# pedroegsilva/gofindthem

Hardware: AMD Instinct MI355X
Metric: ProcessText throughput: documents/s (and input GB/s), 10000-term dictionary + 1000 expressions, 1000000 docs of ~4 KB sharded over 1 GPU(s) (higher is better)
Workload: dtype u8; 1 GPU; BASELINE.json configs[2]: 10000 terms + 1000 AND/OR/NOT expressions, 1000000 docs x ~4 KB on this GPU (SURVEY.md 8(d) generator), case-insensitive finder, inputs resident in HBM; alphabet=lower, keywords=10000, docs_total=1000000, docs_per_gpu=1000000, text_bytes_per_gpu=4100690990, parallelism=docs sharded x1, cu_margin=0

## Files before the change

### gofindthem_amd/_lib.py

```python
import ctypes as C
import os

HERE = os.path.dirname(os.path.abspath(__file__))
LIB_PATH = os.environ.get("GFT_LIBRARY") or os.path.join(HERE, "libgft.so")

GFT_OK, GFT_E_INVALID, GFT_E_NOT_BUILT, GFT_E_HIP, GFT_E_UNSUPPORTED, GFT_E_PARSE, GFT_E_ENGINE = 0, -1, -2, -3, -4, -5, -6
GFT_E_NOMEM, GFT_E_INTERNAL, GFT_W_NO_RCCL = -7, -8, 1
GFT_POS_START, GFT_POS_END = 0, 1
GFT_JSON_OK, GFT_JSON_SYNTAX, GFT_JSON_DEPTH, GFT_JSON_PATH, GFT_JSON_KEY, GFT_JSON_DUP, GFT_JSON_TEXT = range(7)
GFT_FOLD_ASCII = 1
GFT_STATS_ACCUMULATE = 1
GFT_SCORE_DISTINCT = 1
GFT_SCAN_UNIQUE = 2
GFT_POS_RUNES = 4
OP_UNIT, OP_AND, OP_OR, OP_NOT, OP_INORD = 1, 2, 3, 4, 5
INORD_FLAG = 1 << 27


class GftMatches(C.Structure):
    _fields_ = [("n_docs", C.c_uint64), ("n_matches", C.c_uint64), ("match_off", C.c_void_p),
                ("term_id", C.c_void_p), ("pos", C.c_void_p)]


class GftSparse(C.Structure):
# ... 62 lines not shown
    "gft_finder_literal": (_i, [_vp, _i, _u32, C.POINTER(_vp), C.POINTER(_u32)]),
    "gft_finder_expression": (_i, [_vp, _u32, C.POINTER(_vp), C.POINTER(_u32), C.POINTER(_vp), C.POINTER(_u32),
                                   C.POINTER(_vp), C.POINTER(_u32)]),
    "gft_finder_force_build": (_i, [_vp]),
    "gft_finder_process_text": (_i, [_vp, C.c_char_p, _u64, _vp, _u32, C.POINTER(_u32)]),
    "gft_finder_process_texts": (_i, [_vp, _vp, _vp, _u64, _vp]),
    "gft_finder_last_regex_docs": (_u64, [_vp]),
    "gft_finder_process_device": (_i, [_vp, _vp, _vp, _u64, _vp]),
    "gft_finder_process_device_begin": (_i, [_vp, _vp, _vp, _u64, _vp]),
    "gft_finder_process_device_end": (_i, [_vp]),
    "gft_finder_debug_add_literal": (_i, [_vp, _i, C.c_char_p, _u32]),
    "gft_finder_debug_set_updated": (_i, [_vp, _i, _i]),
    "gft_finder_debug_get_updated": (_i, [_vp, C.POINTER(_i), C.POINTER(_i)]),
    "gft_group_create": (_i, [C.POINTER(_vp), _vp]),
    "gft_group_destroy": (None, [_vp]),
    "gft_group_last_error": (C.c_char_p, [_vp]),
    "gft_group_add_rule": (_i, [_vp, C.c_char_p, _u64, C.c_char_p, _u64]),
    "gft_group_state": (_i, [_vp, _vp, _u64, C.POINTER(_u64)]),
    "gft_group_process_jsons": (_i, [_vp, _vp, _vp, _u64, C.c_char_p, _u64, C.c_char_p, _u64, _i, _vp, _u64, C.POINTER(_u64)]),
    "gft_group_last_result": (_i, [_vp, _vp, _u64, C.POINTER(_u64)]),
    "gft_group_evaluate": (_i, [_vp, C.c_char_p, _u64, _vp, _u64, C.POINTER(_u64)]),
    "gft_group_last_batch": (_i, [_vp, C.POINTER(_u64), C.POINTER(_u64)]),
    "gft_group_set_schema": (_i, [_vp, _vp, _vp, _u32, C.c_char_p, _u64, C.c_char_p, _u64]),
    "gft_group_n_rule_exprs": (_u32, [_vp]),
    "gft_group_rule_expr": (_i, [_vp, _u32, C.POINTER(_vp), C.POINTER(_u32), C.POINTER(_vp), C.POINTER(_u32)]),
    "gft_group_process_records_device": (_i, [_vp, _vp, _vp, _vp, _vp, _u64, _u64, _vp]),
    "gft_group_process_records": (_i, [_vp, _vp, _vp, _vp, _vp, _u64, _u64, _vp]),
    "gft_debug_eval_rules": (_i, [_vp, _vp, _u32, _vp, _vp, _u64, _u64, _vp]),
    "gft_debug_eval_rules_device": (_i, [_vp, _vp, _u32, _vp, _vp, _u64, _u64, _vp]),
    "gft_group_tag_records_device": (_i, [_vp, _vp, _vp, _vp, _vp, _u64, _u64, _vp, _vp, _vp, _vp, _u64, C.POINTER(_u64)]),
    "gft_group_tag_records": (_i, [_vp, _vp, _vp, _vp, _vp, _u64, _u64, _vp, _vp, _vp, _vp, _u64, C.POINTER(_u64)]),
    "gft_group_tag_jsons_device": (_i, [_vp, _vp, _vp, _u64, _vp, _vp, _vp, _vp, _vp, _u64, C.POINTER(_u64)]),
    "gft_group_tag_jsons_schema": (_i, [_vp, _vp, _vp, _u64, _vp, _u64, C.POINTER(_u64)]),
    "gft_group_tag_jsons_auto": (_i, [_vp, _vp, _vp, _u64, C.c_char_p, _u64, C.c_char_p, _u64, _vp, _u64, C.POINTER(_u64)]),
    "gft_debug_tag_entries": (_i, [_vp, _vp, _u32, _vp, _vp, _u64, _u64, _vp, _vp, _vp, _vp, _u64, C.POINTER(_u64)]),
    "gft_debug_tag_entries_device": (_i, [_vp, _vp, _u32, _vp, _vp, _u64, _u64, _vp, _vp, _vp, _vp, _u64, C.POINTER(_u64)]),
    "gft_group_rules_json_device": (_i, [_vp, _vp, _u64, _vp, _vp, _u64, _vp, C.POINTER(_u64)]),
    "gft_debug_rules_json": (_i, [_vp, _vp, _u64, _vp, _vp, _u64, _vp, C.POINTER(_u64)]),
    "gft_group_tags_json_device": (_i, [_vp, _vp, _vp, _vp, _u64, _u64, _vp, _vp, _u64, _vp, C.POINTER(_u64)]),
    "gft_debug_tags_json": (_i, [_vp, _vp, _u32, _vp, _vp, _u64, _u64, _vp, _vp, _u64, _vp, C.POINTER(_u64)]),
    "gft_group_json_leaves_device": (_i, [_vp, _vp, _vp, _u64, _vp, _vp, _vp, _vp, _u64, _vp, _u64, _vp]),
    "gft_group_process_jsons_device": (_i, [_vp, _vp, _vp, _u64, _vp, _vp]),
    "gft_group_process_jsons_schema": (_i, [_vp, _vp, _vp, _u64, _vp, _u64, C.POINTER(_u64)]),
    "gft_group_json_last": (_i, [_vp, C.POINTER(_u64), C.POINTER(_u64)]),
    "gft_group_json_paths_device": (_i, [_vp, _vp, _vp, _u64, _vp, _u64, _vp, _u64, _vp, C.POINTER(_u64), C.POINTER(_u64)]),
    "gft_group_process_jsons_auto": (_i, [_vp, _vp, _vp, _u64, C.c_char_p, _u64, C.c_char_p, _u64, _vp, _u64, C.POINTER(_u64)]),
    "gft_group_json_auto_last": (_i, [_vp, C.POINTER(_u64), C.POINTER(_u64), C.POINTER(_u64)]),
    "gft_debug_emulate_json_paths": (_i, [_vp, _vp, _vp, _u64, _vp, _u64, _vp, _u64, _vp, C.POINTER(_u64), C.POINTER(_u64), _vp, _u64, C.POINTER(_u64)]),
    "gft_debug_json_paths_ref": (_i, [_vp, _vp, _vp, _u64, _vp, _u64, _vp, _u64, _vp, C.POINTER(_u64)]),
    "gft_debug_json_leaves_ref": (_i, [_vp, _vp, _vp, _u64, _vp, _vp, _vp, _vp, _u64, _vp, _u64, _vp]),
    "gft_debug_emulate_json_leaves": (_i, [_vp, _vp, _vp, _u64, _vp, _vp, _vp, _vp, _u64, _vp, _u64, _vp]),
    "gft_debug_json_schema_find": (C.c_int64, [_vp, C.c_int64, C.c_char_p, _u32, C.POINTER(C.c_int64)]),
    "gft_group_dsl_parse": (_i, [C.c_char_p, _u64, _vp, _u64, C.POINTER(_u64)]),
    "gft_group_dsl_tokens": (_i, [C.c_char_p, _u64, _vp, _u64, C.POINTER(_u64)]),
    "gft_dsl_parse": (_i, [C.c_char_p, _u64, _i, _vp, _u64, C.POINTER(_u64)]),
    "gft_regex_required_literals": (_i, [C.c_char_p, _u64, _vp, _u64, C.POINTER(_u64)]),
    "gft_dsl_tokens": (_i, [C.c_char_p, _u64, _vp, _u64, C.POINTER(_u64)]),
    "gft_to_lower": (_i, [C.c_char_p, _u64, _vp, _u64, C.POINTER(_u64)]),
    "gft_to_lower_device": (_i, [_vp, _vp, _vp, _u64, _vp, _u64, _vp, C.POINTER(_u64)]),
    "gft_debug_lower_rune": (_u32, [_u32]),
    "gft_debug_emulate_to_lower": (_i, [_vp, _vp, _u64, _vp, _u64, _vp, C.POINTER(_u64)]),
    "gft_finder_lowered_batches": (_i, [_vp, C.POINTER(_u64), C.POINTER(_u64)]),
    "gft_split_lines_device": (_i, [_vp, _vp, _u64, _u32, _vp, _u64, C.POINTER(_u64)]),
    "gft_debug_split_lines": (_i, [_vp, _u64, _u32, _vp, _u64, C.POINTER(_u64)]),
    "gft_debug_split_shape": (None, [C.POINTER(_u32), C.POINTER(_u32)]),
    "gft_finder_split_lines_device": (_i, [_vp, _vp, _u64, _u32, _vp, _u64, C.POINTER(_u64)]),
    "gft_select_docs_device": (_i, [_vp, _vp, _vp, _u64, _vp, _u32, _vp, _u32, _vp, _vp, _u64, _vp, _vp, _u64, C.POINTER(_u64), C.POINTER(_u64)]),
    "gft_debug_select_docs": (_i, [_vp, _vp, _u64, _vp, _u32, _vp, _u32, _vp, _vp, _u64, _vp, _vp, _u64, C.POINTER(_u64), C.POINTER(_u64)]),
    "gft_debug_select_shape": (None, [C.POINTER(_u32), C.POINTER(_u32), C.POINTER(_u32)]),
    "gft_context_docs_device": (_i, [_vp, _vp, _vp, _u64, _vp, _u32, _vp, _u32, _vp, _u64, _u64, _vp, _vp, _u64, _vp, _vp, _vp, _u64, _vp, _u64,
                                     C.POINTER(_u64), C.POINTER(_u64), C.POINTER(_u64), C.POINTER(_u64)]),
    "gft_debug_context_docs": (_i, [_vp, _vp, _u64, _vp, _u32, _vp, _u32, _vp, _u64, _u64, _vp, _vp, _u64, _vp, _vp, _vp, _u64, _vp, _u64,
                                    C.POINTER(_u64), C.POINTER(_u64), C.POINTER(_u64), C.POINTER(_u64)]),
    "gft_debug_context_shape": (None, [C.POINTER(_u32), C.POINTER(_u32), C.POINTER(_u32)]),
    "gft_finder_context_docs_device": (_i, [_vp, _vp, _vp, _u64, _vp, _vp, _u32, _vp, _u64, _u64, _vp, _vp, _u64, _vp, _vp, _vp, _u64, _vp, _u64,
                                            C.POINTER(_u64), C.POINTER(_u64), C.POINTER(_u64), C.POINTER(_u64)]),
    "gft_finder_select_docs_device": (_i, [_vp, _vp, _vp, _u64, _vp, _vp, _u32, _vp, _vp, _u64, _vp, _vp, _u64, C.POINTER(_u64), C.POINTER(_u64)]),
    "gft_route_docs_device": (_i, [_vp, _vp, _vp, _u64, _vp, _u32, _vp, _u32, _u32, _u32, _vp, _vp, _u64, _vp, _vp, _u64, _vp, _vp]),
    "gft_debug_route_docs": (_i, [_vp, _vp, _u64, _vp, _u32, _vp, _u32, _u32, _u32, _vp, _vp, _u64, _vp, _vp, _u64, _vp, _vp]),
    "gft_debug_route_shape": (None, [C.POINTER(_u32)]),
    "gft_finder_route_docs_device": (_i, [_vp, _vp, _vp, _u64, _vp, _vp, _u32, _u32, _u32, _vp, _vp, _u64, _vp, _vp, _u64, _vp, _vp]),
    "gft_hit_spans_device": (_i, [_vp, _vp, _vp, _u64, _u32, _vp, _vp, _vp, _vp, _vp, _vp, _vp, _u64, C.POINTER(_u64)]),
    "gft_redact_spans_device": (_i, [_vp, _vp, _vp, _u64, _vp, _vp, _vp, _u32]),
    "gft_debug_witness_terms": (_i, [_vp, _vp, _u32, _u32, _u32, _vp, _vp, _u64, C.POINTER(_u64)]),
    "gft_debug_hit_spans": (_i, [_vp, _vp, _vp, _u64, _vp, _u32, _vp, _vp, _vp, _u32, _vp, _vp, _vp, _vp, _vp, _vp, _u64, C.POINTER(_u64)]),
    "gft_debug_redact_spans": (_i, [_vp, _vp, _u64, _vp, _vp, _vp, _u32]),
    "gft_debug_spans_shape": (None, [C.POINTER(_u32), C.POINTER(_u32)]),
    "gft_finder_hit_spans_device": (_i, [_vp, _vp, _vp, _u64, _vp, _vp, _vp, _vp, _vp, _vp, _vp, _u64, C.POINTER(_u64), C.POINTER(_i)]),
    "gft_finder_hit_spans_source_device": (_i, [_vp, _vp, _vp, _u64, _vp, _vp, _vp, _vp, _vp, _vp, _vp, _u64, C.POINTER(_u64), C.POINTER(_i)]),
    "gft_map_spans_to_source_device": (_i, [_vp, _vp, _vp, _u64, _vp, _vp, _vp]),
    "gft_debug_map_spans_to_source": (_i, [_vp, _vp, _u64, _vp, _vp, _vp]),
    "gft_excerpt_spans_device": (_i, [_vp, _vp, _vp, _u64, _vp, _vp, _vp, _u32, _u32, _u32, _vp, _u64, _vp, _vp, _vp, _vp, _u64, _vp, _vp,
                                     C.POINTER(_u64), C.POINTER(_u64)]),
    "gft_debug_excerpt_spans": (_i, [_vp, _vp, _u64, _vp, _vp, _vp, _u32, _u32, _u32, _vp, _u64, _vp, _vp, _vp, _vp, _u64, _vp, _vp,
                                    C.POINTER(_u64), C.POINTER(_u64)]),
    "gft_debug_excerpt_shape": (None, [C.POINTER(_u32), C.POINTER(_u32)]),
    "gft_finder_excerpts_device": (_i, [_vp, _vp, _vp, _u64, _vp, _vp, _vp, _i, _i, _u32, _u32, _u32, _vp, _u64, _vp, _vp, _vp, _vp, _u64, _vp, _vp,
                                       C.POINTER(_u64), C.POINTER(_u64), C.POINTER(_i)]),
    "gft_excerpt_spans_snap_device": (_i, [_vp, _vp, _vp, _u64, _vp, _vp, _vp, _u32, _u32, _u32, _u32, _vp, _u64, _vp, _vp, _vp, _vp, _u64, _vp,
                                          _vp, C.POINTER(_u64), C.POINTER(_u64)]),
    "gft_debug_excerpt_spans_snap": (_i, [_vp, _vp, _u64, _vp, _vp, _vp, _u32, _u32, _u32, _u32, _vp, _u64, _vp, _vp, _vp, _vp, _u64, _vp, _vp,
                                         C.POINTER(_u64), C.POINTER(_u64)]),
    "gft_debug_excerpt_snap_edges": (_i, [_vp, _u64, _u64, _u64, _u32, _u32, C.POINTER(_u64), C.POINTER(_u64)]),
    "gft_finder_excerpts_snap_device": (_i, [_vp, _vp, _vp, _u64, _vp, _vp, _vp, _i, _i, _u32, _u32, _u32, _u32, _vp, _u64, _vp, _vp, _vp, _vp, _u64,
                                            _vp, _vp, C.POINTER(_u64), C.POINTER(_u64), C.POINTER(_i)]),
    "gft_mark_spans_device": (_i, [_vp, _vp, _vp, _u64, _vp, _vp, _vp, _vp, _u32, _vp, _u32, _u32, _vp, _u64, _vp, _vp, _vp, C.POINTER(_u64),
                                  C.POINTER(_u64)]),
    "gft_debug_mark_spans": (_i, [_vp, _vp, _u64, _vp, _vp, _vp, _vp, _u32, _vp, _u32, _u32, _vp, _u64, _vp, _vp, _vp, C.POINTER(_u64),
                                 C.POINTER(_u64)]),
    "gft_debug_mark_shape": (None, [C.POINTER(_u32), C.POINTER(_u32), C.POINTER(_u32), C.POINTER(_u32)]),
    "gft_finder_mark_device": (_i, [_vp, _vp, _vp, _u64, _vp, _vp, _vp, _i, _i, _vp, _u32, _vp, _u32, _u32, _vp, _u64, _vp, _vp, _vp,
                                   C.POINTER(_u64), C.POINTER(_u64), C.POINTER(_i)]),
    "gft_replace_spans_device": (_i, [_vp, _vp, _vp, _u64, _vp, _vp, _vp, _vp, _vp, _u32, _vp, _vp, _u32, _u32, _vp, _u64, _vp, _vp, _vp, _vp, _vp,
                                     _u64, C.POINTER(_u64), C.POINTER(_u64)]),
    "gft_debug_replace_spans": (_i, [_vp, _vp, _u64, _vp, _vp, _vp, _vp, _vp, _u32, _vp, _vp, _u32, _u32, _vp, _u64, _vp, _vp, _vp, _vp, _vp,
                                    _u64, C.POINTER(_u64), C.POINTER(_u64)]),
    "gft_debug_replace_shape": (None, [C.POINTER(_u32)] * 6),
    "gft_finder_replace_device": (_i, [_vp, _vp, _vp, _u64, _vp, _vp, _vp, _i, _i, _vp, _vp, _vp, _vp, _u32, _u32, _vp, _u64, _vp, _vp, _vp, _vp,
                                      _vp, _u64, C.POINTER(_u64), C.POINTER(_u64), C.POINTER(_i)]),
    "gft_term_stats_device": (_i, [_vp, _vp, _vp, _u64, _u32, _u32, _u64, _vp, _vp, _vp]),
    "gft_count_columns_device": (_i, [_vp, _vp, _u64, _u32, _vp, _u32, _vp]),
    "gft_batch_term_stats_device": (_i, [_vp, _vp, _vp, _u64, _u32, _vp, _vp, _u32, _u64, _vp, _vp, _vp, C.POINTER(_i)]),
    "gft_debug_term_stats": (_i, [_vp, _vp, _u64, _u32, _u32, _u64, _vp, _vp, _vp]),
    "gft_debug_count_columns": (_i, [_vp, _u64, _u32, _vp, _u32, _vp]),
    "gft_debug_stats_shape": (None, [C.POINTER(_u32)] * 8),
    "gft_finder_term_stats_device": (_i, [_vp, _vp, _vp, _u64, _vp, _vp, _u32, _u64, _vp, _vp, _vp, C.POINTER(_i)]),
    "gft_score_docs_device": (_i, [_vp, _vp, _vp, _u64, _u32, _vp, _u32, _vp, C.POINTER(_u64)]),
    "gft_top_docs_device": (_i, [_vp, _vp, _u64, _u32, _u64, _vp, _vp, C.POINTER(_u64)]),
    "gft_gather_docs_device": (_i, [_vp, _vp, _vp, _u64, _vp, _u64, _u64, _vp, _u64, _vp, C.POINTER(_u64)]),
    "gft_batch_top_docs_device": (_i, [_vp, _vp, _vp, _u64, _u32, _vp, _vp, _vp, _u32, _u32, _u64, _vp, _vp, _vp, C.POINTER(_u64), C.POINTER(_i)]),
    "gft_batch_top_docs_words_device": (_i, [_vp, _vp, _vp, _u64, _u32, _vp, _vp, _vp, _u32, _u32, _u64, _vp, _vp, _vp, C.POINTER(_u64),
                                            C.POINTER(_i)]),
    "gft_debug_score_docs": (_i, [_vp, _vp, _u64, _u32, _vp, _u32, _vp, C.POINTER(_u64)]),
    "gft_debug_top_docs": (_i, [_vp, _u64, _u32, _u64, _vp, _vp, C.POINTER(_u64)]),
    "gft_debug_gather_docs": (_i, [_vp, _vp, _u64, _vp, _u64, _u64, _vp, _u64, _vp, C.POINTER(_u64)]),
    "gft_debug_rank_shape": (None, [C.POINTER(_u32)] * 10),
    "gft_finder_top_docs_device": (_i, [_vp, _vp, _vp, _u64, _vp, _vp, _vp, _u32, _u32, _u64, _vp, _vp, _vp, C.POINTER(_u64), C.POINTER(_i)]),
    "gft_filter_word_matches_device": (_i, [_vp, _vp, _vp, _u64, _vp, _vp, _vp, _vp, _vp, _u32, _u32, _vp, _vp, _vp, _vp, _u64, C.POINTER(_u64)]),
    "gft_debug_filter_word_matches": (_i, [_vp, _vp, _u64, _vp, _vp, _vp, _vp, _vp, _u32, _u32, _vp, _vp, _vp, _vp, _u64, C.POINTER(_u64)]),
    "gft_debug_word_rune": (_u32, [_u32]),
    "gft_debug_words_shape": (None, [C.POINTER(_u32)] * 3),
    "gft_scan_words_device": (_i, [_vp, _vp, _vp, _u64, _u32, _vp]),
    "gft_process_words_device": (_i, [_vp, _vp, _vp, _u64, _u32, _vp]),
    "gft_process_words": (_i, [_vp, _vp, _vp, _u64, _u32, _vp]),
    "gft_hit_spans_words_device": (_i, [_vp, _vp, _vp, _u64, _u32, _vp, _vp, _vp, _vp, _vp, _vp, _vp, _u64, C.POINTER(_u64)]),
    "gft_batch_term_stats_words_device": (_i, [_vp, _vp, _vp, _u64, _u32, _vp, _vp, _u32, _u64, _vp, _vp, _vp, C.POINTER(_i)]),
    "gft_finder_set_whole_words": (_i, [_vp, _i]),
    "gft_finder_whole_words": (_i, [_vp]),
    "gft_debug_lowermap_shape": (None, [C.POINTER(_u32), C.POINTER(_u32), C.POINTER(_u32), C.POINTER(_u32)]),
    "gft_group_process_json_lines": (_i, [_vp, _vp, _u64, C.c_char_p, _u64, C.c_char_p, _u64, _vp, _u64, C.POINTER(_u64)]),
    "gft_debug_emulate_scan": (_i, [_vp, _vp, _u32, _vp, _u32, _u32, _u32, _u32, _vp, _vp, _u64, C.POINTER(_u64)]),
    "gft_debug_tables": (_i, [_vp, _vp, _u32, _vp, _u64, _u64, C.c_char_p, C.POINTER(C.c_char_p), _vp, _u64, C.POINTER(_u64), _vp, _u64]),
    "gft_debug_learned_unit": (_i, [_vp, C.POINTER(_u32), C.POINTER(_u32)]),
    "gft_debug_last_unit_route": (_i, [_vp, C.POINTER(C.c_char_p)]),
    "gft_debug_last_fold_bits": (_i, [_vp, C.POINTER(_u32)]),
    "gft_debug_scan_plan": (_i, [_vp, _vp, _u32, _u64, C.c_char_p, C.POINTER(C.c_char_p), _vp]),
    "gft_debug_pool_entries": (_i, [_vp, C.POINTER(_u64)]),
    "gft_debug_last_solve_pf": (_i, [_vp, C.POINTER(_u32), C.POINTER(_u32)]),
    "gft_debug_judge_batch": (_i, [_vp, _i, _u32, _u64, _u64, _u64, _u64, C.POINTER(_i), C.POINTER(_u64), _vp, _vp, _u64]),
    "gft_debug_learn": (_i, [C.c_char_p, _u32, _i, _u64, _u64, _u64, C.POINTER(_u32), C.POINTER(C.c_double)]),
    "gft_debug_eval_programs": (_i, [_vp, _vp, _u32, _u32, _vp, _vp, _vp]),
    "gft_debug_program_shape": (_i, [_vp, _vp, _u32, _u32, _vp, _u32]),
    "gft_debug_plan_solve": (_i, [_u32, _u32, _u32, _i, _u32, _u64, _u32, _u64, _i, _i, _u32, _vp]),
    "gft_debug_plan_solve_pf": (_i, [_u32, _u32, _u32, _i, _u32, _u32, _u64, _u32, _u64, _i, _i, _u32, _u32, _vp]),
    "gft_debug_host_solve": (_i, [_vp, _u64, _vp, _vp, _vp, _u32, C.POINTER(_i)]),
    "gft_profile_enable": (_i, [_vp, _i]),
    "gft_profile_read": (_i, [_vp, C.c_char_p, C.POINTER(C.c_double), C.POINTER(_u64)]),
    "gft_profile_reset": (_i, [_vp]),
}

EMIT_FN = C.CFUNCTYPE(None, _vp, _vp, _u32, C.c_int64)
BUILD_FN = C.CFUNCTYPE(_i, _vp, _vp, _vp, _u32, _i, _vp, _u32)
FIND_FN = C.CFUNCTYPE(_i, _vp, _vp, _u64, EMIT_FN, _vp, _vp, _u32)

_LIB = None


def _mapped_hip_runtimes():
    try:
        with open("/proc/self/maps") as f:
            return sorted({ln.split()[-1] for ln in f if "libamdhip64.so" in ln})
    except OSError:
        return []


def _hip_runtime_first():
    import sys
    if "torch" in sys.modules or os.environ.get("GFT_NO_TORCH_PRELOAD"):
        return
    import importlib.util
    if importlib.util.find_spec("torch") is not None:
        import torch


def _check_one_hip_runtime():
    libs = _mapped_hip_runtimes()
    if len(libs) > 1:
        import warnings
        warnings.warn("two HIP runtimes are mapped into this process (%s): device pointers of one are not valid in the "
                      "other -- import torch before gofindthem_amd loads libgft.so" % ", ".join(libs), RuntimeWarning)


def load():
    global _LIB
    if _LIB is None:
        if not os.path.exists(LIB_PATH):
            raise RuntimeError("libgft.so is not built (run `python -m gofindthem_amd.build`); "
                               "gofindthem_amd has no CPU fallback for the hot path")
        _hip_runtime_first()
        L = C.CDLL(LIB_PATH)
        _check_one_hip_runtime()
        for name, (res, args) in SYMBOLS.items():
            f = getattr(L, name)
            f.restype, f.argtypes = res, args
        _LIB = L
    return _LIB
```

### gofindthem_amd/csrc/batch_verdict.hpp

```cpp
#pragma once
#include <algorithm>
#include <cstddef>
#include <cstdint>

#include "table_set.hpp"

namespace gft {

constexpr size_t kCtlBytes = 64, kCtlWords = 7;
constexpr size_t kCtlBad = 0, kCtlCursor = 8, kCtlTotal = 16, kCtlNonascii = 24, kCtlUnits = 32;
constexpr size_t kCtlBatchClear = 32;
constexpr size_t kCtlRetryClear = 16;
constexpr size_t kCtlScanRead = 24;

struct CtlBlock {
    uint32_t bad = 0;
    uint64_t cursor = 0, total = 0;
    uint32_t nonascii_bits = 0;
    uint32_t miss_epoch = 0;
    uint64_t n_units = 0, text_lo = 0, text_hi = 0;
};
CtlBlock decode_ctl(const uint64_t words[kCtlWords]);

struct BatchVerdict {
    bool nonascii = false;
    uint32_t nonascii_bits = 0;
    uint64_t text_lo = 0, text_hi = 0;
    uint64_t n_units = 0, total = 0;
};

struct ScanLaunch {
    bool deferred = false;
    bool single = false;
    uint32_t epoch = 0;
    bool ordered = false;
    uint64_t n_docs = 0, unit_cap = 0, pool_cap = 0;
    uint64_t static_slabs = 0;
};

inline bool single_miss(const CtlBlock& c, const ScanLaunch& L) { return L.single && c.miss_epoch == L.epoch; }

struct Judgement {
    enum Kind { accept, again_general, again_grow, invalid } kind = accept;
    uint64_t pool_need = 0;
    const char* err = "";
    BatchVerdict verdict;
};
Judgement judge_deferred(const CtlBlock& c, const ScanLaunch& L);

struct Learned {
    int single_streak = 0;
    uint32_t unit_max = kScan2UnitMax;
    double scan4_density = 0.06;
    uint32_t unit_entries = 0;
};
constexpr int kSingleMissStreak = -8;
inline void count_streak(Learned& s, uint64_t n_units, uint64_t n_docs) {
    s.single_streak = n_units == n_docs ? s.single_streak + 1 : std::min(s.single_streak, 0);
}
void learn(Learned& s, ScanKernel kernel, uint32_t fifo_cap, bool ordered, uint64_t total, uint64_t text_lo, uint64_t text_hi);

}
```

### gofindthem_amd/csrc/gft_api.cpp

```cpp
#include "gft_engine.hpp"

#include <cstdio>
#include <cstdlib>

using namespace gft;
using namespace gft::api;

namespace {

long env_num(const char* name, long dflt) { const char* v = getenv(name); return v ? atol(v) : dflt; }

void refresh_options(gft_engine* e) {
    const auto num = env_num;
    e->opt_scan_dbg = (uint32_t)num("GFT_SCAN_DEBUG", 0);
    e->opt_scan_prio = num("GFT_SCAN_PRIO", 1) ? 1u : 0u;
    e->opt_scan_ordered = getenv("GFT_SCAN_ORDERED") ? 1u : 0u;
    e->opt_scan4_chunk = (uint32_t)num("GFT_SCAN4_CHUNK", 0);
    e->opt_scan4_round = (uint32_t)num("GFT_SCAN4_ROUND", 0);
    e->opt_solve.dbg = (uint32_t)num("GFT_SOLVE_DEBUG", 0);
    e->opt_solve.forced_group = (int)num("GFT_SOLVE_GROUP_DOCS", -1);
    e->opt_solve.prog_lds = num("GFT_SOLVE_PROG_LDS", 1) ? 1u : 0u;
    const long pf = num("GFT_SOLVE_PF_TERMS", 0);
    e->opt_solve.forced_pf = pf == 6 || pf == 12 ? (uint32_t)pf : 0u;
}

}

namespace gft::api {

ScanOptions scan_options() {
    const auto num = env_num;
    ScanOptions o;
    o.forced = parse_forced(getenv("GFT_SCAN_KERNEL"));
    o.scan5_groups = (uint32_t)num("GFT_SCAN5_GROUPS", 0);
    o.scan5_large = num("GFT_SCAN5_LARGE", 1) ? 1u : 0u;
    o.scan5_bloom_kb = (uint32_t)std::min<long>(std::max<long>(num("GFT_SCAN5_BLOOM_KB", 32), 0), 64);
    o.scan5_fifo = (uint32_t)std::min<long>(std::max<long>(num("GFT_SCAN5_FIFO", 0), 0), 4096) & ~63u;
    return o;
}

bool pend_settled(const gft_engine* e) {
    for (unsigned i = 0; i < e->pend_count; i++)
        if (!e->pend[(e->pend_head + i) % 2].done) return false;
    return true;
}

int check_ready(const gft_engine* e, unsigned need, const char* who) {
    if ((need & kNeedDevice) && e->device < 0) return fail(e, GFT_E_HIP, "no HIP device available");
    if ((need & kNeedBuilt) && !e->built) return fail(e, GFT_E_NOT_BUILT, "gft_build has not been called");
    if ((need & kNeedPrograms) && !e->have_programs) return fail(e, GFT_E_NOT_BUILT, "gft_set_programs has not been called");
    if ((need & kNeedSettled) && !pend_settled(e))
        return fail(e, GFT_E_INVALID, (who ? std::string(who) + ": " : std::string()) +
                                          "batches of gft_process_device_begin are in flight: gft_process_device_end (or _complete) first");
    return GFT_OK;
}

}

extern "C" {

int gft_engine_create(gft_engine** out, int device) try {
    if (!out) return GFT_E_INVALID;
    *out = nullptr;
    std::unique_ptr<gft_engine> owner(new gft_engine());
    gft_engine* e = owner.get();
    int count = 0;
    hipError_t h = hipGetDeviceCount(&count);
    if (h != hipSuccess || count == 0) {
        e->device = -1;
        e->err = std::string("no HIP device available: ") + (h != hipSuccess ? hipGetErrorString(h) : "device count is 0");
        *out = owner.release();
        return GFT_E_HIP;
    }
    if (device < 0) { if (hipGetDevice(&device) != hipSuccess) device = 0; }
    e->device = device;
    DeviceGuard g(device);
    hipDeviceProp_t prop;
    if (hipGetDeviceProperties(&prop, device) == hipSuccess) {
        e->n_cus_hw = prop.multiProcessorCount > 0 ? (unsigned)prop.multiProcessorCount : 256;
        if (const char* m = getenv("GFT_CU_MARGIN")) { const int v = atoi(m); if (v > 0) e->cu_margin = (unsigned)v; }
        e->n_cus = e->n_cus_hw > e->cu_margin ? e->n_cus_hw - e->cu_margin : 1;
        int optin = 0;
        if (hipDeviceGetAttribute(&optin, hipDeviceAttributeSharedMemPerBlockOptin, device) != hipSuccess) optin = 0;
        e->lds_max = std::max<size_t>(prop.sharedMemPerBlock, (size_t)std::max(optin, 0));
        if (std::string(prop.gcnArchName).find("gfx950") != std::string::npos) e->lds_max = std::max<size_t>(e->lds_max, 160 * 1024);
    }
    if (hipStreamCreateWithFlags(&e->stream, hipStreamDefault) == hipSuccess) e->own_stream = true;
    else e->stream = nullptr;
    refresh_options(e);
    *out = owner.release();
    return GFT_OK;
} GFT_CATCH(nullptr)

void gft_engine_destroy(gft_engine* e) {
    if (!e) return;
    if (e->device < 0) {
        destroy_multi(e);
        delete e;
        return;
    }
    DeviceGuard g(e->device);
    if (e->stream) (void)hipStreamSynchronize(e->stream);
    for (auto& kv : e->prof)
        for (auto& p : kv.second.ev) { e->prof_pool.push_back(p.first); e->prof_pool.push_back(p.second); }
    for (hipEvent_t ev : e->prof_pool) (void)hipEventDestroy(ev);
    for (int k = 0; k < 2; k++) {
        if (e->staging.pin[k]) (void)hipHostFree(e->staging.pin[k]);
        if (k == 0 && e->pin_rb) (void)hipHostFree(e->pin_rb);
        if (e->staging.pin_ev[k]) (void)hipEventDestroy(e->staging.pin_ev[k]);
        if (e->pend[k].rb) (void)hipHostFree(e->pend[k].rb);
        if (e->pend[k].ev) (void)hipEventDestroy(e->pend[k].ev);
    }
    if (e->d_excerpt.pin) (void)hipHostFree(e->d_excerpt.pin);
    destroy_multi(e);
    hipStream_t own = e->own_stream ? e->stream : nullptr;
    delete e;
    if (own) (void)hipStreamDestroy(own);
}

const char* gft_last_error(const gft_engine* e) { return e ? e->err.c_str() : "null engine"; }

int gft_set_stream(gft_engine* e, void* hip_stream) try {
    if (!e) return GFT_E_INVALID;
    GFT_LOCK(e);
    if (int rc = check_ready(e, kNeedDevice)) return rc;
    DeviceGuard g(e->device);
    if (e->own_stream && e->stream) { (void)hipStreamSynchronize(e->stream); (void)hipStreamDestroy(e->stream); }
    e->own_stream = false;
    e->stream = (hipStream_t)hip_stream;
    if (!hip_stream) {
        HIP_TRY(hipStreamCreateWithFlags(&e->stream, hipStreamDefault), "stream create");
        e->own_stream = true;
    }
    return GFT_OK;
} GFT_CATCH((e ? &e->err : nullptr))


int gft_set_cu_margin(gft_engine* e, uint32_t margin) try {
    if (!e) return GFT_E_INVALID;
    GFT_LOCK(e);
    if (int rc = check_ready(e, kNeedDevice)) return rc;
    if (e->pend_count) return fail(e, GFT_E_INVALID, "batches are in flight (gft_process_device_end first)");
    e->cu_margin = margin;
    e->n_cus = e->n_cus_hw > margin ? e->n_cus_hw - margin : 1;
    return GFT_OK;
} GFT_CATCH((e ? &e->err : nullptr))

}

namespace gft::api {

static int upload_scan3_short_tables(gft_engine* e, const Scan3Tables& s3) {
    const std::vector<uint8_t> none(16, 0), g1(s3.cls, s3.cls + 256), g2(s3.cls_fold, s3.cls_fold + 256);
    SyncOnExit drained(e);
    auto& d = e->d_tabs.s3;
    int rc;
    if ((rc = upload(e, d.short3, s3.short3.empty() ? none : s3.short3, "table upload"))) return rc;
    if ((rc = upload(e, d.srec, s3.srec, "table upload"))) return rc;
    if (!s3.short3_big.empty() && (rc = upload(e, d.short3_big, s3.short3_big, "table upload"))) return rc;
    if ((rc = upload(e, d.srec_big, s3.srec_big, "table upload"))) return rc;
    if ((rc = upload(e, d.cls, g1, "table upload"))) return rc;
    if ((rc = upload(e, d.cls_fold, g2, "table upload"))) return rc;
    return GFT_OK;
}

int install_tables(gft_engine* e, TableSet&& set, uint32_t flags) {
    const AcTables& tab = set.tab;
    const Scan2Tables& s2 = set.s2;
    const Scan3Tables& s3 = set.s3;
    ScanPlan plan;
// ... 258 lines not shown
```

### gofindthem_amd/csrc/gft_debug.cpp

```cpp
#include "gft_engine.hpp"

#include <unordered_set>

#include "host_solve.hpp"

using namespace gft;
using namespace gft::api;

extern "C" {

int gft_debug_emulate_scan(const uint8_t* terms_blob, const uint64_t* term_off, uint32_t n_terms, const uint8_t* text,
                           uint32_t len, uint32_t lo, uint32_t flags, uint32_t scan_flags, uint32_t* out_term,
                           uint32_t* out_pos, uint64_t cap, uint64_t* needed) try {
    if ((n_terms && (!terms_blob || !term_off)) || (len && !text) || lo > len || !needed) return GFT_E_INVALID;
    std::vector<std::string> terms;
    for (uint32_t i = 0; i < n_terms; i++) terms.emplace_back((const char*)terms_blob + term_off[i], (size_t)(term_off[i + 1] - term_off[i]));
    AcTables tab;
    build_ac_tables(std::move(terms), tab);
    Scan3Tables t;
    build_scan3_tables(tab, t);
    if (!t.supported) return GFT_E_UNSUPPORTED;
    std::vector<Scan3Hit> hits;
    scan3_emulate(t, text, len, lo, (scan_flags & GFT_FOLD_ASCII) != 0, (flags & GFT_POS_END) != 0, hits);
    *needed = hits.size();
// ... 13 lines not shown
    Scan2Tables s2;
    build_scan2_tables(tab, s2);
    if (!s2.long_ok) return GFT_E_UNSUPPORTED;
    Scan5Tables s5;
    build_scan5_tables(tab, s2, std::min<uint32_t>(groups && groups < s2.kp ? groups : s2.kp, 32u), s5);
    if (groups_used) *groups_used = s5.G;
    const bool fold = (scan_flags & GFT_FOLD_ASCII) != 0;
    const uint8_t* cls = fold ? s2.cls_fold : s2.cls;
    const uint8_t* grp = fold ? s5.grp_fold : s5.grp;
    const uint32_t kp = s2.kp, G = s5.G;
    auto cl = [&](int64_t i) { return i < 0 ? s2.pad_class : (uint32_t)cls[text[i]]; };
    auto gr = [&](int64_t i) { return i < 0 ? s5.pad_group : (uint32_t)grp[text[i]]; };
    std::unordered_set<uint32_t> keys;
    for (const Scan2Slot& sl : s2.slots) if (sl.key != kScan2EmptyKey) keys.insert(sl.key);
    std::vector<std::vector<uint32_t>> shorts;
    for (const auto& term : tab.terms)
        if (!term.empty() && term.size() < 4) {
            std::vector<uint32_t> v;
            for (unsigned char ch : term) v.push_back(tab.byte_class[ch]);
            shorts.push_back(v);
        }
    for (uint32_t i = 0; i < len; i++) {
        const uint32_t key = (uint32_t)((((uint64_t)cl((int64_t)i - 3) * kp + cl((int64_t)i - 2)) * kp + cl((int64_t)i - 1)) * kp + cl(i));
        bool f = keys.count(key) != 0;
        for (size_t k = 0; k < shorts.size() && !f; k++) {
            const auto& v = shorts[k];
            bool eq = true;
            for (size_t j = 0; j < v.size() && eq; j++) eq = cl((int64_t)i - (int64_t)(v.size() - 1 - j)) == v[j];
            f = eq;
        }
        out_exact[i] = f ? 1 : 0;
        out_dual[i] = 0;
    }
    for (int64_t j = (int64_t)(lane_start & 1u); j < (int64_t)len; j += 2) {
        const uint64_t ent = s5.filter[((size_t)gr(j - 2) * G + gr(j - 1)) * G + gr(j)];
        out_dual[j] = (uint8_t)(ent >> gr(j - 3) & 1);
        if (j + 1 < (int64_t)len) out_dual[j + 1] = (uint8_t)(ent >> (32 + gr(j + 1)) & 1);
    }
    if (lane_start & 1u) {
        const uint64_t ent = s5.filter[((size_t)gr(-3) * G + gr(-2)) * G + gr(-1)];
        if (len) out_dual[0] = (uint8_t)(ent >> (32 + gr(0)) & 1);
    }
    return GFT_OK;
} GFT_CATCH(nullptr)

int gft_debug_program_shape(const uint32_t* prog_words, const uint64_t* prog_off, uint32_t n_exprs, uint32_t n_slots, uint32_t* out_shape,
                            uint32_t shape_cap) try {
    if (!prog_words || !prog_off || !out_shape || n_slots > (1u << kDwFieldBits)) return GFT_E_INVALID;
    ProgramSet ps;
    std::string err;
    const int rc = compile_programs(prog_words, prog_off, n_exprs, n_slots, ps, err);
    if (rc) return rc;
    if (shape_cap < 3 + ps.blk_class.size()) return GFT_E_INVALID;
    out_shape[0] = ps.fprog_words; out_shape[1] = ps.n_rare_words > 0; out_shape[2] = ps.wide_pairs;
    std::copy(ps.blk_class.begin(), ps.blk_class.end(), out_shape + 3);
    return GFT_OK;
} GFT_CATCH(nullptr)

int gft_debug_eval_programs(const uint32_t* prog_words, const uint64_t* prog_off, uint32_t n_exprs, uint32_t n_slots,
                            const uint8_t* present, uint8_t* out_hit, uint32_t* out_depth) try {
    if (!prog_words || !prog_off || !out_hit || (n_slots && !present) || n_slots > (1u << kDwFieldBits)) return GFT_E_INVALID;
    ProgramSet ps;
    std::string err;
    const int rc = compile_programs(prog_words, prog_off, n_exprs, n_slots, ps, err);
    if (rc) return rc;
    std::vector<uint8_t> elsewhere(n_exprs, 0);
    for (uint32_t x : ps.host_only) elsewhere[x] = 1;
    for (uint32_t k = 0; k < ps.n_wide; k++) elsewhere[ps.wide_list[3 * k]] = 1;
    for (uint32_t i = 0; i < n_exprs; i++) {
        const uint32_t ex = ps.order[i], b = i / 64, lane = i % 64;
        if (elsewhere[ex]) return GFT_E_UNSUPPORTED;
        const uint32_t depth = ps.fdepth[ex];
        if (out_depth) out_depth[ex] = depth;
        bool acc = false;
        std::vector<bool> stack;
        size_t reached = 0;
        for (uint64_t pc = 0; pc < ps.fprog_off[ex + 1] - ps.fprog_off[ex]; pc++) {
            const uint32_t w = ps.fprog_t[ps.fblk_off[b] + ((pc / 4) * 64 + lane) * 4 + pc % 4];
            if (w & kDwRare) {
                if (!(w & kDwNeg)) return GFT_E_UNSUPPORTED;
                acc = !acc;
                continue;
            }
            const bool v = (present[(w & kDwFieldMask) >> kDwFieldShift] != 0) != ((w & kDwNeg) != 0);
            if ((w & kDwPop) && stack.empty()) return GFT_E_INVALID;
            const bool x = (w & kDwPop) ? (bool)stack.back() : v;
            const bool A = (w & kDwSel) ? x : (w & kDwOnes) != 0, B = (w & kDwOr) ? x : false;
            const bool before = acc;
            acc = (acc && A) || B;
            if (w & kDwPop) stack.pop_back();
            if (w & kDwPush) stack.push_back(before);
            if (stack.size() > depth) return GFT_E_INVALID;
            reached = std::max(reached, stack.size());
        }
        if (!stack.empty()) return GFT_E_INVALID;
        if (reached > (ps.blk_class[b] == 0 ? 0u : ps.blk_class[b] == 1 ? kSolveRegStack : kMaxBoolDepth)) return GFT_E_INTERNAL;
        out_hit[ex] = acc ? 1 : 0;
    }
    return GFT_OK;
} GFT_CATCH(nullptr)

static int debug_tables_and_plan(const uint8_t* terms_blob, const uint64_t* term_off, uint32_t n_terms, const uint8_t* blob, uint64_t blob_len,
                                 uint64_t lds_max, const char* forced_kernel, TableSet& set, uint32_t& flags, ScanPlan& plan, std::string& err) {
    if (blob) {
        if (int rc = read_tables(blob, blob_len, set, flags, err)) return rc;
    } else {
        std::vector<std::string> terms;
        for (uint32_t i = 0; i < n_terms; i++) terms.emplace_back((const char*)terms_blob + term_off[i], (size_t)(term_off[i + 1] - term_off[i]));
        compile_tables(std::move(terms), set);
    }
    ScanOptions opt = scan_options();
    if (forced_kernel) opt.forced = parse_forced(forced_kernel);
    return plan_scan(set, opt, lds_max, kExtraKernels, plan, err);
}

int gft_debug_tables(const uint8_t* terms_blob, const uint64_t* term_off, uint32_t n_terms, const uint8_t* blob, uint64_t blob_len,
                     uint64_t lds_max, const char* forced_kernel, const char** kernel, uint8_t* out, uint64_t cap, uint64_t* needed,
                     char* err_out, uint64_t err_cap) try {
    if (!kernel || !needed || (!blob && n_terms && (!terms_blob || !term_off))) return GFT_E_INVALID;
    *kernel = "";
    *needed = 0;
    std::string err;
    auto done = [&](int rc) {
        if (err_out && err_cap) { const size_t n = std::min<size_t>(err.size(), err_cap - 1); memcpy(err_out, err.data(), n); err_out[n] = 0; }
        return rc;
    };
    TableSet set;
    uint32_t flags = 0;
    int rc;
    ScanPlan plan;
    if ((rc = debug_tables_and_plan(terms_blob, term_off, n_terms, blob, blob_len, lds_max, forced_kernel, set, flags, plan, err))) return done(rc);
    *kernel = kScanKernelName[(int)plan.kernel];
    if (plan.kernel == ScanKernel::scan5) {
        Scan5Tables s5;
        std::vector<uint32_t> bloom;
        derive_scan5(set, plan, s5, bloom);
    }
    std::vector<uint8_t> b;
    write_tables(set, flags, b);
    *needed = b.size();
    if (!out) return done(GFT_OK);
    if (cap < b.size()) return done(GFT_E_INVALID);
    memcpy(out, b.data(), b.size());
    return done(GFT_OK);
} GFT_CATCH(nullptr)

int gft_debug_learned_unit(const gft_engine* e, uint32_t* unit_max, uint32_t* fifo_cap) {
    if (!e || !unit_max) return GFT_E_INVALID;
    *unit_max = e->learned.unit_max;
    if (fifo_cap) *fifo_cap = e->plan.kernel == ScanKernel::scan5 ? e->plan.s5plan.fifo_cap : kScan2FifoCap;
    return GFT_OK;
}

int gft_debug_last_unit_route(const gft_engine* e, const char** name) {
    if (!e || !name) return GFT_E_INVALID;
    *name = e->last_unit_route;
    return GFT_OK;
}

int gft_debug_last_fold_bits(const gft_engine* e, uint32_t* bits) {
    if (!e || !bits) return GFT_E_INVALID;
    *bits = e->reported.nonascii_bits;
    return GFT_OK;
}

int gft_debug_scan_plan(const uint8_t* terms_blob, const uint64_t* term_off, uint32_t n_terms, uint64_t lds_max, const char* forced_kernel,
                        const char** kernel, uint32_t* plan_out) try {
    if (!kernel || !plan_out || (n_terms && (!terms_blob || !term_off))) return GFT_E_INVALID;
    *kernel = "";
    TableSet set;
    uint32_t flags = 0;
    ScanPlan plan;
    std::string err;
    if (int rc = debug_tables_and_plan(terms_blob, term_off, n_terms, nullptr, 0, lds_max, forced_kernel, set, flags, plan, err)) return rc;
    *kernel = kScanKernelName[(int)plan.kernel];
    const bool s5 = plan.kernel == ScanKernel::scan5;
    plan_out[0] = set.tab.max_term_len;
    plan_out[1] = s5 ? plan.s5_term_bits : 0u;
    plan_out[2] = s5 ? plan.s5_pos_bias : 0u;
    plan_out[3] = s5 ? plan.s5plan.fifo_cap : kScan2FifoCap;
    return GFT_OK;
} GFT_CATCH(nullptr)

int gft_debug_pool_entries(const gft_engine* e, uint64_t* entries) {
    if (!e || !entries) return GFT_E_INVALID;
    *entries = e->pool.total;
    return GFT_OK;
}

int gft_debug_last_solve_pf(const gft_engine* e, uint32_t* pf_terms, uint32_t* unit_entries) {
    if (!e || !pf_terms) return GFT_E_INVALID;
    *pf_terms = e->last_pf_terms;
    if (unit_entries) *unit_entries = e->learned.unit_entries;
    return GFT_OK;
}

int gft_debug_host_solve(const uint32_t* words, uint64_t len, const uint32_t* slots, const uint64_t* list_off,
                         const int64_t* positions, uint32_t n_lists, int* out) try {
    if (!words || !out || (n_lists && (!slots || !list_off))) return GFT_E_INVALID;
    uint32_t n_slots = 0;
    for (uint64_t i = 0; i < len; i++)
        if ((words[i] >> 28) == GFT_OP_UNIT) n_slots = std::max(n_slots, (words[i] & GFT_SLOT_MASK) + 1);
    ProgramTraits tr;
    std::string err;
    const int rc = check_program(words, len, n_slots, 0, tr, err);
    if (rc) return rc;
    SlotLists m;
    for (uint32_t k = 0; k < n_lists; k++) {
        std::vector<int64_t>& v = m[slots[k]];
        for (uint64_t i = list_off[k]; i < list_off[k + 1]; i++) v.push_back(positions[i]);
    }
    *out = host_solve(words, len, m) ? 1 : 0;
    return GFT_OK;
} GFT_CATCH(nullptr)

}
```

### gofindthem_amd/csrc/gft_engine.hpp

```cpp
#pragma once
#include "../../include/gft.h"

#include <hip/hip_runtime.h>

#include <algorithm>
#include <cstring>
#include <map>
#include <memory>
#include <mutex>
#include <string>
#include <utility>
#include <vector>

#include "batch_verdict.hpp"
#include "copy_pool.hpp"
#include "gft_guard.hpp"
#include "gft_kernels.hpp"
#include "program_set.hpp"
#include "solve_plan.hpp"
#include "table_set.hpp"

namespace gft::api {

struct DevBuf {
    void* p = nullptr;
    size_t cap = 0;
    DevBuf() = default;
    DevBuf(const DevBuf&) = delete;
    DevBuf& operator=(const DevBuf&) = delete;
    DevBuf(DevBuf&& o) noexcept : p(o.p), cap(o.cap) { o.p = nullptr; o.cap = 0; }
    DevBuf& operator=(DevBuf&& o) noexcept {
        if (this != &o) { release(); p = o.p; cap = o.cap; o.p = nullptr; o.cap = 0; }
        return *this;
    }
    ~DevBuf() { release(); }
    hipError_t ensure(size_t bytes) {
        if (bytes <= cap) return hipSuccess;
        if (p) { hipError_t e = hipFree(p); p = nullptr; cap = 0; if (e != hipSuccess) return e; }
        size_t want = bytes + bytes / 8 + 256;
        hipError_t e = hipMalloc(&p, want);
        if (e == hipSuccess) cap = want;
        return e;
    }
    void release() { if (p) (void)hipFree(p); p = nullptr; cap = 0; }
    template <class T> T* as() const { return reinterpret_cast<T*>(p); }
};

struct ProfCat {
    std::vector<std::pair<hipEvent_t, hipEvent_t>> ev;
};

struct PoolState {
    uint64_t n_units = 0, total = 0;
    uint64_t valid_docs = ~0ull;
    bool csr_valid = false;
};

}

struct gft_engine {
    using DevBuf = gft::api::DevBuf;
    int device = 0;
    hipStream_t stream = nullptr;
    struct Staging {
        void* pin[2] = {nullptr, nullptr};
        hipEvent_t pin_ev[2] = {nullptr, nullptr};
        std::unique_ptr<gft::CopyPool> copy_pool;
    } staging;
    uint64_t* pin_rb = nullptr;
    bool own_stream = false;
    unsigned n_cus = 256;
    unsigned n_cus_hw = 256, cu_margin = 0;
    size_t lds_max = 65536;
    mutable std::string err;

    gft::TableSet tables;
    gft::ScanPlan plan;
    gft::Scan5Tables s5;
    bool built = false;
    uint32_t build_flags = 0;
    struct TableBufs {
        struct { DevBuf byte_class, delta, out_term, out_link, term_len; } dfa;
        struct { DevBuf filter, slots, more, cls, cls_fold, term_blob, term_off, short3, shorts_packed, short3_big, fpt; } s2;
        struct { DevBuf filter, short3, srec, short3_big, srec_big, bloom, slots, more, cls, cls_fold, term_blob, term_off; } s3;
        struct { DevBuf grp, grp_fold, filter, bloom; } s5;
    } d_tabs;
    DevBuf d_ctl, d_dbg;
    gft::Learned learned;
    gft::BatchVerdict reported;
    gft::api::PoolState pool;
    uint32_t opt_scan_dbg = 0;
    uint32_t opt_scan_prio = 1;
    uint32_t opt_scan_ordered = 0;
    uint32_t opt_scan4_round = 0;
    uint32_t opt_scan4_chunk = 0;
    gft::SolveOptions opt_solve;
    mutable std::recursive_mutex mu;
    std::vector<gft_engine*> peers;
    std::vector<uint64_t> shard_cut;
    bool in_multi = false;
    std::vector<void*> comms;
    bool rccl_self = false;
    void* rccl_lib = nullptr;

    bool have_programs = false;
    uint32_t n_exprs = 0, n_extra = 0;
    gft::ProgramSet progs;
    struct ProgramBufs {
        DevBuf prog, prog_off;
        DevBuf fprog, fprog_off, groups;
        DevBuf order, blk_class, wave_blk;
        DevBuf fprog_t, fblk_off;
        DevBuf wide_list;
    } d_progs;
    DevBuf d_patch;
    DevBuf d_wide_slot, d_wide_theta;
    DevBuf d_solve_dbg;
    uint32_t ctl_epoch = 1;
    uint32_t solve_unit_entries = 0;
    uint32_t last_pf_terms = 0;
    const char* last_unit_route = "";
    struct Pending {
        bool done = false;
        int rc = 0;
        const uint8_t* d_text = nullptr; const uint64_t* d_doc_off = nullptr; uint64_t n_docs = 0; uint32_t flags = 0;
        uint32_t* d_bitmap = nullptr;
        gft::ScanLaunch launch;
        uint64_t* rb = nullptr; hipEvent_t ev = nullptr;
        gft::BatchVerdict verdict;
    };
    Pending pend[2];
    unsigned pend_head = 0, pend_count = 0;
    DevBuf d_pscratch;

    DevBuf d_unit_cnt, d_unit_base, d_units, d_partial, d_pool_term, d_pool_pos, d_unit_start,
        d_unit_count, d_unit_out, d_term, d_pos, d_match_off;
    uint64_t pool_cap = 0;
    DevBuf d_text, d_doc_off, d_bitmap, d_xoff, d_xslot, d_xpos;
    struct UniqueBufs { DevBuf first, cnt, off, term; } d_uq;
    struct RuneBufs { DevBuf cnt, base, starts, prefix; } d_rn;
    std::vector<uint64_t> h_match_off;
    std::vector<uint32_t> h_term, h_pos;
    bool have_labels = false;
    std::vector<uint32_t> h_labels;
    DevBuf d_labels;
    struct SparseBufs {
        DevBuf cnt, partial, row_off, idx, label;
        std::vector<uint64_t> h_row_off;
        std::vector<uint32_t> h_expr_idx, h_label, h_bitmap;
    } sparse;
    struct LowerBufs {
        bool table_up = false;
        DevBuf page, delta, doc_units, unit_base, units, partial, unit_cnt, unit_out, ctl, text, off;
    } d_lw;

    struct SplitBufs { DevBuf sums, carry, cnt, base, partial; } d_split;

    struct SelectBufs { DevBuf want, len, sel, pos, rank, partial, ctl, c_off, c_src; } d_select;

    struct ContextBufs { DevBuf want, sel, len, keep, word_sel, word_fence, sum, carry, part, pos, rank, grank, partial, ctl, c_off, c_src; } d_context;

    struct RouteBufs { DevBuf masks, member, len, cnt, tile_bytes, base, partial, ctl, ent_len, c_off, c_src; } d_route;

    struct SpanBufs {
        bool wit_ready = false;
        DevBuf wit_off, wit_expr, want, keep, rank, partial, dst, ctl;
    } d_spans;

    struct LowerMapBufs { DevBuf tab, off, mapped, ctl; } d_lmap;

    struct ExcerptBufs {
        DevBuf ws, we, sdoc, smin, head, share, tmin, carry, rank, pos, partial, ctl, c_off, c_src;
        uint64_t* pin = nullptr;
    } d_excerpt;

    struct MarkBufs { DevBuf q, marks; } d_mark;

    struct ReplaceBufs { DevBuf rid, pl, ppos, key_rep, rep_off, tab, at, delta, len, roff; } d_replace;

    struct StatsBufs { DevBuf ctl, rows; } d_stats;

    struct KeptBufs { DevBuf off, start, term; } d_kept;

    struct RankBufs {
        DevBuf ctl, weights, rows, hist, tile_gt, tile_eq, gt_pos, eq_pos, partial, cand_score, cand_idx, len, c_off, c_src, score;
    } d_rank;

    struct WordBufs {
        bool table_up = false;
        DevBuf tab_row, tab_bits, ctl, keep, rank, partial, off, pos, term, span_off, span_start, span_len, span_term;
    } d_words;

    struct RuleBufs {
        uint64_t serial = 0;
        uint32_t n_fields = 0, n_tags = 0, n_exprs = 0, n_rules = 0, n_units = 0, max_depth = 0, field_words = 0;
        DevBuf expr_tag, masks, units, prog, prog_off, leaf_bitmap, tag_rows, flags, stage[6];
        DevBuf valid;
    } d_rules;

    struct TagBufs {
        DevBuf cnt, leaf_ent_off, partial, flags, row_off, ent_field, ent_expr;
    } d_tags;

    struct ResultBufs {
        uint64_t serial = 0;
        uint32_t n_exprs = 0;
        DevBuf rule_first, name_off, name_len, expr_off, expr_len, blob, cnt, scan, partial, flags, hole_len, out_off, text;
    } d_result;

    struct TagDocBufs {
        uint64_t slot_serial = 0, field_serial = 0;
        uint32_t n_exprs = 0, SW = 0, n_tags = 0, n_fields = 0;
        DevBuf src_off, src_expr, slot_off, slot_len, tag_word, tag_words, tag_off, tag_len, slot_blob;
        DevBuf field_rank, field_off, field_len, valid, field_blob;
        DevBuf slot_rows, leaf_field, rec_off, cnt, scan, partial, flags, hole_len, out_off, text;
        bool staged = false;
        uint64_t staged_records = 0, staged_leaves = 0;
    } d_tagdoc;

    struct JsonBufs {
        uint64_t serial = 0;
        uint32_t n_nodes = 0, table_mask = 0, max_key_len = 0;
        DevBuf nodes, keys, table, cnt_leaves, cnt_text, text_off, partial, flags, rec_off, leaf_field, leaf_off, text, blob, doc_off, status, rows;
        DevBuf paths;
    } d_json;

    int profiling = 0;
    std::vector<hipEvent_t> prof_pool;
    std::map<std::string, gft::api::ProfCat> prof;
};

#define GFT_LOCK(e) std::lock_guard<std::recursive_mutex> _gft_lock((e)->mu)

#define HIP_TRY(expr, what)                                             \
    do {                                                                \
        hipError_t _h = (expr);                                         \
        if (_h != hipSuccess) return gft::api::fail_hip(e, _h, what);   \
    } while (0)

namespace gft::api {

inline int fail(const gft_engine* e, int code, const std::string& msg) {
    e->err = msg;
    return code;
}
inline int fail_hip(const gft_engine* e, hipError_t h, const char* what) {
    e->err = std::string(what) + ": " + hipGetErrorString(h);
// ... 98 lines not shown
```

### gofindthem_amd/csrc/gft_kernels.hip

```cpp
#include <hip/hip_runtime.h>

#include "gft_kernels.hpp"
#include "gft_wave_dev.hpp"

namespace gft {

namespace {

constexpr uint32_t kLane = 64;

__device__ __forceinline__ uint32_t wave_incl_scan_shfl(uint32_t v) {
    const uint32_t l = lane_id();
#pragma unroll
    for (int s = 1; s < 64; s <<= 1) {
        uint32_t o = __shfl_up(v, s, 64);
        if ((int)l >= s) v += o;
    }
    return v;
}

__global__ void __launch_bounds__(256) k_unit_count(const uint64_t* __restrict__ doc_off, uint64_t n_docs,
                                                    uint32_t unit_max, uint32_t* __restrict__ cnt,
                                                    uint32_t* __restrict__ bad) {
    uint64_t d = (uint64_t)blockIdx.x * blockDim.x + threadIdx.x;
    if (d >= n_docs) return;
    uint64_t n = doc_off[d + 1] - doc_off[d];
    if (n > 0xFFFFFFFFull) { atomicOr(bad, 1u); n = 0; }
    cnt[d] = n <= unit_max ? 1u : (uint32_t)((n + unit_max - 1) / unit_max);
}

__global__ void k_pack_ctl(const uint64_t* __restrict__ unit_base, const uint64_t* __restrict__ doc_off, uint64_t n_docs,
                           uint64_t* __restrict__ out) {
    out[0] = unit_base[n_docs];
    out[1] = doc_off[0];
    out[2] = doc_off[n_docs];
}

__global__ void __launch_bounds__(256) k_unit_fill(const uint64_t* __restrict__ doc_off, uint64_t n_docs,
                                                   const uint64_t* __restrict__ unit_base, Unit* __restrict__ units,
                                                   uint64_t max_units, uint32_t unit_max) {
    uint64_t d = (uint64_t)blockIdx.x * blockDim.x + threadIdx.x;
    if (d >= n_docs) return;
    uint64_t n = doc_off[d + 1] - doc_off[d];
    if (n > 0xFFFFFFFFull) n = 0;
    uint64_t b = unit_base[d];
    uint32_t k = (uint32_t)(unit_base[d + 1] - b);
    if (k == 0) return;
    for (uint32_t i = 0; i < k; i++)
        if (b + i < max_units) units[b + i] = unit_slice((uint32_t)d, n, k, i, unit_max);
}

__global__ void __launch_bounds__(256) k_units_single(const uint64_t* __restrict__ doc_off, uint64_t n_docs, uint32_t unit_max,
                                                      Unit* __restrict__ units, uint64_t* __restrict__ unit_base,
                                                      uint32_t* __restrict__ ctl32, uint32_t epoch) {
    const uint64_t d = (uint64_t)blockIdx.x * blockDim.x + threadIdx.x;
    if (d == 0) {
        uint64_t* ctl64 = reinterpret_cast<uint64_t*>(ctl32);
        unit_base[n_docs] = n_docs;
        ctl32[1] = 0; ctl64[1] = 0; ctl64[2] = 0; ctl32[6] = 0;
        ctl64[4] = n_docs; ctl64[5] = doc_off[0]; ctl64[6] = doc_off[n_docs];
    }
    if (d >= n_docs) return;
    uint64_t n = doc_off[d + 1] - doc_off[d];
    if (n > 0xFFFFFFFFull) { atomicMax(ctl32, epoch); n = 0; }
    if (n > unit_max) { atomicMax(ctl32 + 7, epoch); n = unit_max; }
    units[d] = Unit{(uint32_t)d, 0u, (uint32_t)n};
    unit_base[d] = d;
}

__global__ void __launch_bounds__(256) k_patch_words(uint32_t* __restrict__ words, const uint64_t* __restrict__ idx,
                                                     const uint32_t* __restrict__ clr, const uint32_t* __restrict__ set, uint64_t n) {
    const uint64_t i = (uint64_t)blockIdx.x * blockDim.x + threadIdx.x;
    if (i >= n) return;
    if (clr[i]) atomicAnd(&words[idx[i]], ~clr[i]);
    if (set[i]) atomicOr(&words[idx[i]], set[i]);
}

__global__ void __launch_bounds__(256) k_clamp_u64(uint64_t* __restrict__ v, uint64_t n, uint64_t cap) {
    const uint64_t i = (uint64_t)blockIdx.x * blockDim.x + threadIdx.x;
    if (i < n && v[i] > cap) v[i] = cap;
}

constexpr uint32_t kScanItems = 16, kScanBlock = 256, kScanTile = kScanItems * kScanBlock;

__device__ __forceinline__ uint64_t block_excl_scan_u64(uint64_t v, uint64_t* total) {
    __shared__ uint64_t wsum[kScanBlock / 64];
    const uint32_t l = lane_id(), w = threadIdx.x >> 6;
    uint64_t incl = v;
#pragma unroll
    for (int s = 1; s < 64; s <<= 1) {
        uint64_t o = __shfl_up(incl, s, 64);
        if ((int)l >= s) incl += o;
    }
    if (l == 63) wsum[w] = incl;
    __syncthreads();
    uint64_t off = 0, tot = 0;
#pragma unroll
    for (uint32_t i = 0; i < kScanBlock / 64; i++) {
        if (i < w) off += wsum[i];
        tot += wsum[i];
    }
    __syncthreads();
    *total = tot;
    return off + incl - v;
}

__global__ void __launch_bounds__(kScanBlock) k_scan_partials(const uint32_t* __restrict__ in, uint64_t n,
                                                              uint64_t* __restrict__ partial) {
    uint64_t base = (uint64_t)blockIdx.x * kScanTile + (uint64_t)threadIdx.x * kScanItems;
    uint64_t s = 0;
#pragma unroll
    for (uint32_t i = 0; i < kScanItems; i++)
        if (base + i < n) s += in[base + i];
    uint64_t tot;
    block_excl_scan_u64(s, &tot);
    if (threadIdx.x == 0) partial[blockIdx.x] = tot;
}

__global__ void __launch_bounds__(kScanBlock) k_scan_spine(uint64_t* __restrict__ partial, uint64_t n_part) {
    uint64_t carry = 0;
    for (uint64_t b = 0; b < n_part; b += kScanBlock) {
        uint64_t i = b + threadIdx.x;
        uint64_t v = i < n_part ? partial[i] : 0, tot;
        uint64_t ex = block_excl_scan_u64(v, &tot);
        if (i < n_part) partial[i] = carry + ex;
        carry += tot;
    }
    if (threadIdx.x == 0) partial[n_part] = carry;
}

__global__ void __launch_bounds__(kScanBlock) k_scan_final(const uint32_t* __restrict__ in, uint64_t n,
                                                           const uint64_t* __restrict__ partial, uint64_t n_part,
                                                           uint64_t* __restrict__ out) {
    uint64_t base = (uint64_t)blockIdx.x * kScanTile + (uint64_t)threadIdx.x * kScanItems;
    uint32_t v[kScanItems];
    uint64_t s = 0;
#pragma unroll
    for (uint32_t i = 0; i < kScanItems; i++) {
        v[i] = base + i < n ? in[base + i] : 0;
        s += v[i];
    }
    uint64_t tot;
    uint64_t ex = block_excl_scan_u64(s, &tot) + partial[blockIdx.x];
#pragma unroll
    for (uint32_t i = 0; i < kScanItems; i++) {
        if (base + i < n) out[base + i] = ex;
        ex += v[i];
    }
    if (blockIdx.x == 0 && threadIdx.x == 0) out[n] = partial[n_part];
}

template <bool WRITE>
__device__ __forceinline__ uint32_t walk_chunk(const ScanParams& P, const uint8_t* __restrict__ buf,
                                               const uint8_t* __restrict__ cls_lds,
                                               const uint32_t* __restrict__ delta_lds, uint32_t seg_lo,
                                               uint32_t walk_from, uint32_t my_lo, uint32_t my_hi, uint64_t out_idx) {
    uint32_t state = 0, cnt = 0;
    const uint32_t ncls = P.n_classes;
    for (uint32_t p = walk_from; p < my_hi; p++) {
        const uint32_t c = cls_lds[buf[p - seg_lo]];
        const uint32_t e = state < P.n_lds_states ? delta_lds[state * ncls + c] : P.delta[(size_t)state * ncls + c];
        state = e & 0x7FFFFFFFu;
        if ((e >> 31) && p >= my_lo) {
            uint32_t s = state;
            do {
                const uint32_t t = P.out_term[s];
                if (t != 0xFFFFFFFFu) {
                    if (WRITE) {
                        P.pool_term[out_idx + cnt] = t;
                        P.pool_pos[out_idx + cnt] = P.pos_end ? p : p + 1 - P.term_len[t];
                    }
                    cnt++;
                }
                s = P.out_link[s];
            } while (s != 0);
        }
    }
    return cnt;
}

__global__ void __launch_bounds__(kScanBlockThreads) k_scan_units(const ScanParams P) {
    extern __shared__ __align__(16) uint8_t smem[];
    uint8_t* cls_lds = smem;
    uint32_t* delta_lds = reinterpret_cast<uint32_t*>(smem + 256);
    const uint32_t tier_words = P.n_lds_states * P.n_classes;
    uint8_t* text_lds = smem + 256 + (((size_t)tier_words * 4 + 15) & ~(size_t)15);

    for (uint32_t i = threadIdx.x; i < 256; i += blockDim.x) cls_lds[i] = P.byte_class[i];
    for (uint32_t i = threadIdx.x; i < tier_words; i += blockDim.x) delta_lds[i] = P.delta[i];
    __syncthreads();

    const uint32_t lane = lane_id(), wave = threadIdx.x >> 6, wpb = blockDim.x >> 6;
    uint8_t* buf = text_lds + (size_t)wave * kTextBuf;
    const uint32_t warm = P.max_term_len > 0 ? P.max_term_len - 1 : 0;
    bool told_nonascii = false;

    for (uint64_t u = (uint64_t)blockIdx.x * wpb + wave; u < P.n_units; u += (uint64_t)gridDim.x * wpb) {
        const Unit un = P.units[u];
        const uint64_t dstart = P.doc_off[un.doc];
        const uint32_t seg_lo = un.lo > warm ? un.lo - warm : 0;
        const uint32_t nbytes = un.hi - seg_lo;
        const uint8_t* src = P.text + dstart + seg_lo;
        uint32_t hib = 0;
        for (uint32_t i = lane; i < nbytes; i += kLane) {
            uint8_t b = src[i];
            hib |= b;
            if (P.fold && b >= 'A' && b <= 'Z') b += 32;
            buf[i] = b;
        }
        if (P.fold && P.nonascii && !told_nonascii && __any((hib & 0x80u) != 0)) { told_nonascii = true; if (lane == 0) atomicOr(P.nonascii, 1u); }
        __builtin_amdgcn_wave_barrier();
        __builtin_amdgcn_fence(__ATOMIC_ACQ_REL, "wavefront");
// ... 440 lines not shown
```

### gofindthem_amd/csrc/gft_kernels.hpp

```cpp
#pragma once
#include <hip/hip_runtime.h>
#include <stdint.h>

#include "solve_plan.hpp"

namespace gft {

constexpr uint32_t kScanBlockThreads = 512;
constexpr uint32_t kTextBuf = 8448;
constexpr uint32_t kSolveBlockThreads = 1024;
constexpr uint32_t kMaxPairs = 64;
constexpr uint32_t kMaxPairDepth = 32;
constexpr uint32_t kMaxBoolDepth = 128;
constexpr uint32_t kMaxPairsWide = 8192;
constexpr uint32_t kMaxPairDepthWide = 64;

#define GFT_K_INORD_FLAG (1u << 27)
#define GFT_K_SLOT_MASK ((1u << 27) - 1u)

struct Unit { uint32_t doc, lo, hi; };
__host__ __device__ inline Unit unit_slice(uint32_t doc, uint64_t n, uint64_t k, uint64_t i, uint32_t unit_max) {
    uint64_t per = (n + k - 1) / k;
    if (per > unit_max) per = unit_max;
    const uint64_t lo = i * per < n ? i * per : n, hi = lo + per < n ? lo + per : n;
// ... 71 lines not shown
    const uint32_t* unit_count;
    const uint32_t* term;
    const uint32_t* pos;
    const uint64_t* x_off;
    const uint32_t* x_slot;
    const uint32_t* x_pos;
    uint64_t n_docs;
    const uint32_t* fprog;
    const uint64_t* fprog_off;
    const uint32_t* gprog;
    const uint32_t* groups;
    const uint32_t* order;
    const Unit* units;
    uint32_t has_rare;
    uint32_t pos_back;
    const uint32_t* blk_class;
    const uint32_t* wave_blk;
    const uint32_t* fprog_t;
    const uint32_t* fblk_off;
    uint32_t n_exprs, n_slots, tile_words;
    uint32_t fprog_words;
    uint32_t dbg;
    unsigned long long* dbg_out;
    uint64_t* p_scratch;
    uint32_t* wide_slot;
    long long* wide_theta;
    uint32_t wide_cap;
    const uint32_t* wide_list;
    uint32_t n_wide;
    uint32_t* bitmap;
};

#if defined(__HIPCC__)
#define GFT_HD __host__ __device__
#else
#define GFT_HD
#endif

constexpr uint32_t kScan2Threads = 1024;
constexpr uint32_t kScan2StageCap = 6;
constexpr uint32_t kScan2FifoCap = 256;
constexpr uint32_t kScan2CandCapMin = 512;
constexpr uint32_t kScan2Slab = 4096;
constexpr uint32_t kScan2UnitMax = 8192;
constexpr uint32_t kGoldDev = 0x9E3779B1u;

constexpr uint32_t kScan2EmptyKey = 0xFFFFFFFFu;
constexpr uint32_t kScan2Multi = 0x80000000u;
constexpr uint32_t kScan2InlineLen = 24;
constexpr uint32_t kScan2MaxOff = 4;
constexpr uint32_t kScan2LenMask = 0x00FFFFFFu;
struct __attribute__((aligned(32))) Scan2Slot {
    uint32_t key;
    uint32_t info;
    uint32_t len;
    uint32_t front[5];
};
struct Scan2Short {
    uint32_t n;
    uint32_t term[3];
    uint32_t len[3];
    uint32_t pad;
};
constexpr uint32_t kScan2Short3Max = 32768;
constexpr uint32_t kScan2FptSize = 20480;
constexpr uint32_t kScan2FptLdsItems = 11000;
constexpr uint32_t kScan2FptAmbiguous = 0xFF;
template <uint32_t C>
GFT_HD inline uint32_t scan2_mul24c(uint32_t a) {
#if defined(__HIP_DEVICE_COMPILE__)
    uint32_t d;
    asm("v_mul_u32_u24 %0, %1, %2" : "=v"(d) : "n"(C), "v"(a));
    return d;
#else
    return (uint32_t)((uint64_t)(a & 0xFFFFFFu) * (uint64_t)(C & 0xFFFFFFu));
#endif
}
GFT_HD inline uint32_t scan2_slot_hash(uint32_t x, int which, uint32_t shift, uint32_t seed) {
    const uint32_t xf = (x ^ (x >> 20)) + seed;
    return (which ? scan2_mul24c<0x85EBCBu>(xf) : scan2_mul24c<0x9E3779u>(xf)) >> shift;
}
GFT_HD inline uint32_t scan2_pair_slot(uint32_t x, int which, uint32_t shift, uint32_t seed) {
    const uint32_t xf = (x ^ (x >> 20)) + seed;
    return ((scan2_mul24c<0x9E3779u>(xf) >> shift) & ~1u) | (uint32_t)which;
}
GFT_HD inline uint32_t scan2_fpt_index(uint32_t h, uint32_t fpt_lg) {
    return fpt_lg ? h >> (32 - fpt_lg) : scan2_mul24c<kScan2FptSize>(h >> 16) >> 16;
}
GFT_HD inline uint32_t scan2_fpt_xcell(uint32_t x, uint32_t fpt_lg) { return scan2_fpt_index(scan2_mul24c<0x3779B1u>(x), fpt_lg); }
GFT_HD inline uint32_t scan2_fpt_gcell(uint32_t x, uint32_t b1n, int which, uint32_t fpt_lg) {
    return scan2_fpt_index(which ? scan2_mul24c<0xB2AE35u>(x) + scan2_mul24c<0x9E4F2Du>(b1n)
                                 : scan2_mul24c<0xC2B2AFu>(x) + scan2_mul24c<0x27D4EBu>(b1n), fpt_lg);
}
GFT_HD inline uint32_t scan2_fpt_xmix(uint32_t x) { return scan2_mul24c<0xD4EB2Fu>(x); }
GFT_HD inline uint32_t scan2_fpt_xbyte(uint32_t xmix) { return 1u + (xmix >> 25); }
GFT_HD inline bool scan2_fpt_pass(uint32_t cx, uint32_t cg0, uint32_t cg1, uint32_t xmix, uint32_t tw) {
    (void)tw;
    const uint32_t tag = scan2_fpt_xbyte(xmix);
    const bool amb = (cx == kScan2FptAmbiguous) | (cg0 == kScan2FptAmbiguous) | (cg1 == kScan2FptAmbiguous);
    return (cx == tag) | (cg0 == tag) | (cg1 == tag) | amb;
}

struct Scan2Params {
    const uint8_t* text;
    const uint64_t* doc_off;
    const Unit* units;
    uint64_t n_units;
    const uint32_t* filter;
    uint32_t filter_words, hashed, hash_shift;
    const uint8_t* short3;
    uint32_t short3_bytes;
    const uint32_t* shorts_packed;
    uint32_t shorts_words;
    const uint32_t* short3_big;
    uint32_t cand_cap;
    const uint8_t* fpt;
    uint32_t fpt_lg;
    const Scan2Slot* slots;
    uint32_t slot_shift, slot_seed;
    const Scan2Slot* more;
    const uint8_t* cls;
    const uint8_t* term_blob;
    const uint32_t* term_off;
    uint32_t kp, pad_class, fold, pos_end;
    uint64_t* cursor;
    uint64_t pool_cap;
    uint32_t* pool_term;
    uint32_t* pool_pos;
    uint64_t* unit_start;
    uint32_t* unit_count;
    uint64_t* n_matches;
    uint32_t slab;
    uint32_t ordered;
    uint64_t text_bytes;
    uint32_t prio;
    uint32_t want_pos;
    uint32_t dbg;
    uint32_t* nonascii;
    uint64_t* dbg_counters;
    uint32_t chunk_units;
    uint32_t bound_q16, bound_add;
    uint32_t round_c;
    const uint8_t* s5_grp;
    uint32_t s5_G, s5_pad_g;
    const uint64_t* s5_filter;
    uint32_t s5_dual;
    uint32_t s5_fifo_cap;
    const uint8_t* s5_sgrp;
    uint32_t s5_sG;
    const uint32_t* s5_srec_big;
    uint32_t s5_term_bits, s5_pos_bias;
    const uint32_t* s5_bloom;
    uint32_t s5_bloom_lg;
};
GFT_HD inline uint32_t scan5_bloom_g(uint32_t x, uint32_t b1n, uint32_t lg) {
    return (scan2_mul24c<0xC2B2AFu>(x ^ (x >> 20)) + scan2_mul24c<0x27D4EBu>(b1n + 1)) >> (32 - lg);
}
GFT_HD inline uint32_t scan5_bloom_x(uint32_t x, uint32_t lg) { return scan2_mul24c<0x3779B1u>(x ^ (x >> 20)) >> (32 - lg); }
bool scan2_plan(uint32_t filter_words, uint32_t short3_bytes, uint32_t shorts_words, uint32_t fpt_lds_bytes, size_t lds_max,
                uint32_t* waves, uint32_t* cand_cap);
hipError_t launch_scan2(const Scan2Params& P, uint32_t waves, unsigned n_cus, hipStream_t st);
constexpr uint32_t kScan4ChunkUnits = 8;
constexpr uint32_t kScan4UnitMax = 8176;
bool scan4_plan(uint32_t filter_words, uint32_t short3_bytes, uint32_t shorts_words, uint32_t fpt_lds_bytes, size_t lds_max, bool want_pos,
                uint32_t* waves, uint32_t* fifo_cap);
hipError_t launch_scan4(const Scan2Params& P, uint32_t waves, unsigned n_cus, hipStream_t st);
constexpr uint32_t kScan5Waves = 16;
constexpr uint32_t kScan5MaxGroups = 27;
constexpr uint32_t kScan5SurvX = 64;
constexpr uint32_t kScan5SeenWords = 8;
constexpr uint32_t kScan5CandCapMin = 384;
struct Scan5Plan { uint32_t G, dual_entries, cand_cap, fifo_cap; };
bool scan5_plan(uint32_t kp, uint32_t short3_bytes, uint32_t shorts_words, uint32_t fpt_lds_bytes, size_t lds_max, uint32_t fifo_cap, Scan5Plan* out);
hipError_t launch_scan5(const Scan2Params& P, unsigned n_cus, hipStream_t st);


constexpr uint32_t kScan3Groups = 27;
constexpr uint32_t kScan3Threads = 1024;
constexpr uint32_t kScan3UnitMax = 8192;
constexpr uint32_t kScan3RecWords = 6;
constexpr uint32_t kScan3RecLds = 254;
constexpr uint32_t kScan3BloomLdsLg = 13;
constexpr uint32_t kScan3SurvCap = 128;
constexpr uint32_t kScan3MinRoom = 512;
constexpr uint32_t kScan3CandCapMin = 256;
constexpr uint32_t kScan3BloomMul1 = 0x9E3779B1u, kScan3BloomMul2 = 0x85EBCA6Bu;
GFT_HD inline uint32_t scan3_bloom_cell(uint32_t key5, uint32_t lg) { return (key5 * kScan3BloomMul1) >> (32 - lg); }
GFT_HD inline uint32_t scan3_bloom_bits(uint32_t key5) {
    const uint32_t h = key5 * kScan3BloomMul2;
    return 1u << (h >> 27) | 1u << ((h >> 22) & 31);
}

struct Scan3Params {
    const uint8_t* text;
    const uint64_t* doc_off;
    const Unit* units;
    uint64_t n_units;
    uint64_t text_bytes;
    const uint8_t* cls;
    const uint32_t* filter;
    uint32_t filter_words;
    const uint8_t* short3;
    uint32_t short3_bytes;
    const uint32_t* srec;
    uint32_t srec_words;
    const uint32_t* short3_big;
    const uint32_t* srec_big;
    const uint32_t* bloom;
    uint32_t bloom_lg, bloom_lds;
    const Scan2Slot* slots;
    uint32_t slot_shift, slot_seed;
    const Scan2Slot* more;
    const uint8_t* term_blob;
    const uint32_t* term_off;
    uint32_t G, fold, pos_end, want_pos, grouped, prio;
    uint32_t cand_cap;
    uint32_t dbg;
    uint32_t* nonascii;
    uint64_t* cursor;
    uint64_t pool_cap;
    uint32_t* pool_term;
    uint32_t* pool_pos;
    uint64_t* unit_start;
    uint32_t* unit_count;
    uint64_t* n_matches;
    uint32_t slab;
};
bool scan3_plan(uint32_t filter_words, uint32_t short3_bytes, uint32_t srec_words, uint32_t bloom_lds_bytes, size_t lds_max,
                uint32_t* waves, uint32_t* cand_cap);
hipError_t launch_scan3(const Scan3Params& P, uint32_t waves, unsigned n_cus, hipStream_t st);

hipError_t launch_unit_count(const uint64_t* d_doc_off, uint64_t n_docs, uint32_t unit_max, uint32_t* d_cnt,
                             uint32_t* d_bad, hipStream_t st);
hipError_t launch_pack_ctl(const uint64_t* d_unit_base, const uint64_t* d_doc_off, uint64_t n_docs, uint64_t* d_out, hipStream_t st);
hipError_t launch_unit_fill(const uint64_t* d_doc_off, uint64_t n_docs, const uint64_t* d_unit_base, Unit* d_units,
                            uint32_t unit_max, hipStream_t st, uint64_t max_units = ~0ull);
hipError_t launch_units_single(const uint64_t* d_doc_off, uint64_t n_docs, uint32_t unit_max, Unit* d_units, uint64_t* d_unit_base,
                               uint32_t* d_ctl32, uint32_t epoch, hipStream_t st);
hipError_t launch_patch_words(uint32_t* d_words, const uint64_t* d_idx, const uint32_t* d_clr, const uint32_t* d_set, uint64_t n, hipStream_t st);
hipError_t launch_clamp_u64(uint64_t* d_v, uint64_t n, uint64_t cap, hipStream_t st);
uint64_t scan_partials_needed(uint64_t n);
hipError_t launch_exclusive_scan(const uint32_t* d_in, uint64_t n, uint64_t* d_out, uint64_t* d_partial,
                                 hipStream_t st);
hipError_t launch_compact_count(const uint32_t* d_bitmap, uint64_t n_docs, uint32_t n_exprs, uint32_t* d_cnt, unsigned n_cus,
                                hipStream_t st);
hipError_t launch_compact_fill(const uint32_t* d_bitmap, uint64_t n_docs, uint32_t n_exprs, const uint64_t* d_row_off,
                               uint32_t* d_expr_idx, uint32_t* d_label, const uint32_t* d_expr_label, uint64_t cap, unsigned n_cus,
                               hipStream_t st);
size_t scan_units_lds_bytes(uint32_t n_lds_states, uint32_t n_classes);
hipError_t launch_scan_units(const ScanParams& P, unsigned n_cus, hipStream_t st);
hipError_t launch_gather(const uint64_t* d_unit_start, const uint32_t* d_unit_count, const uint64_t* d_unit_out,
                         uint64_t n_units, const uint32_t* d_pool_term, const uint32_t* d_pool_pos, uint32_t* d_term,
                         uint32_t* d_pos, const uint64_t* d_unit_base, uint64_t n_docs, uint64_t* d_match_off,
                         unsigned n_cus, hipStream_t st, const Unit* d_units_to_sort = nullptr,
                         const uint32_t* d_term_len = nullptr, uint32_t pos_end = 0);
hipError_t launch_fold_safe(const uint8_t* d_text, uint64_t lo, uint64_t hi, const uint64_t* d_doc_off, uint64_t n_docs, uint32_t* d_flag, hipStream_t st);
hipError_t launch_unique_terms(bool write, const uint64_t* d_match_off, const uint32_t* d_term, uint64_t n_docs, uint32_t n_terms,
                               uint32_t* d_first, unsigned grid, uint32_t* d_cnt, const uint64_t* d_out_off, uint32_t* d_out_term,
                               hipStream_t st);
hipError_t launch_rune_doc_blocks(const uint64_t* d_doc_off, uint64_t n_docs, uint32_t* d_cnt, hipStream_t st);
hipError_t launch_rune_block_starts(const uint8_t* d_text, const uint64_t* d_doc_off, const uint64_t* d_blk_base, uint64_t n_docs,
                                    uint64_t n_blocks, uint32_t* d_starts, hipStream_t st);
hipError_t launch_pos_to_rune(const uint8_t* d_text, const uint64_t* d_doc_off, const uint64_t* d_blk_base, const uint64_t* d_blk_prefix,
                              const uint64_t* d_match_off, uint64_t n_docs, uint64_t n_matches, uint32_t* d_pos, hipStream_t st);
hipError_t launch_solve(const SolveParams& S, const SolvePlan& plan, hipStream_t st);

}
```

### gofindthem_amd/csrc/gft_pipeline.cpp

```cpp
#include "gft_engine.hpp"

#include <cstdio>

#include "host_solve.hpp"

#ifndef GFT_EXTRA_KERNELS
namespace gft {
bool scan2_plan(uint32_t, uint32_t, uint32_t, uint32_t, size_t, uint32_t*, uint32_t*) { return false; }
hipError_t launch_scan2(const Scan2Params&, uint32_t, unsigned, hipStream_t) { return hipErrorNotSupported; }
bool scan4_plan(uint32_t, uint32_t, uint32_t, uint32_t, size_t, bool, uint32_t*, uint32_t*) { return false; }
hipError_t launch_scan4(const Scan2Params&, uint32_t, unsigned, hipStream_t) { return hipErrorNotSupported; }
}
namespace gft::api { const bool kExtraKernels = false; }
#else
namespace gft::api { const bool kExtraKernels = true; }
#endif

namespace gft::api {

static int ensure_pool(gft_engine* e, uint64_t entries) {
    if (entries <= e->pool_cap) return GFT_OK;
    HIP_TRY(e->d_pool_term.ensure(entries * 4), "pool alloc");
    HIP_TRY(e->d_pool_pos.ensure(entries * 4), "pool alloc");
    e->pool_cap = std::min(e->d_pool_term.cap, e->d_pool_pos.cap) / 4;
    return GFT_OK;
}

static int csr_from_pool(gft_engine* e, uint64_t n_docs) {
    hipStream_t st = e->stream;
    const uint64_t n_units = e->pool.n_units, total = e->pool.total;
    HIP_TRY(e->d_term.ensure(std::max<uint64_t>(total, 1) * 4), "result alloc");
    HIP_TRY(e->d_pos.ensure(std::max<uint64_t>(total, 1) * 4), "result alloc");
    HIP_TRY(e->d_unit_out.ensure((n_units + 1) * 8), "unit alloc");
    HIP_TRY(e->d_partial.ensure(scan_partials_needed(std::max(n_units, n_docs)) * 8), "unit alloc");
    ProfScope ps(e, "aux");
    HIP_TRY(launch_exclusive_scan(e->d_unit_count.as<uint32_t>(), n_units, e->d_unit_out.as<uint64_t>(),
                                  e->d_partial.as<uint64_t>(), st), "unit_out scan");
    const bool sort_units = counts_slabs(e->plan.kernel);
    HIP_TRY(launch_gather(e->d_unit_start.as<uint64_t>(), e->d_unit_count.as<uint32_t>(),
                          e->d_unit_out.as<uint64_t>(), n_units, e->d_pool_term.as<uint32_t>(),
                          e->d_pool_pos.as<uint32_t>(), e->d_term.as<uint32_t>(), e->d_pos.as<uint32_t>(),
                          e->d_unit_base.as<uint64_t>(), n_docs, e->d_match_off.as<uint64_t>(), e->n_cus, st,
                          sort_units ? e->d_units.as<Unit>() : nullptr,
                          e->d_tabs.dfa.term_len.as<uint32_t>(), (e->build_flags & GFT_POS_END) ? 1u : 0u),
            "gather");
    e->pool.csr_valid = true;
    return GFT_OK;
}

struct ScanBatch {
    const uint8_t* d_text; const uint64_t* d_doc_off;
    uint64_t n_docs, n_units, text_hi;
    uint32_t flags, unit_max;
    bool need_csr;
};

template <class T>
T* ctl_at(const gft_engine* e, size_t byte_off) { return reinterpret_cast<T*>(e->d_ctl.as<uint8_t>() + byte_off); }

template <class Params>
void fill_common(const gft_engine* e, const ScanBatch& b, Params& P) {
    P.text = b.d_text; P.doc_off = b.d_doc_off; P.units = e->d_units.as<Unit>(); P.n_units = b.n_units;
    P.pos_end = (e->build_flags & GFT_POS_END) ? 1 : 0;
    P.fold = (b.flags & GFT_FOLD_ASCII) ? 1 : 0;
    P.nonascii = ctl_at<uint32_t>(e, kCtlNonascii);
    P.cursor = ctl_at<uint64_t>(e, kCtlCursor); P.pool_cap = e->pool_cap;
    P.pool_term = e->d_pool_term.as<uint32_t>(); P.pool_pos = e->d_pool_pos.as<uint32_t>();
    P.unit_start = e->d_unit_start.as<uint64_t>(); P.unit_count = e->d_unit_count.as<uint32_t>();
}
template <class Params>
void fill_window(const gft_engine* e, const ScanBatch& b, Params& P) {
    fill_common(e, b, P);
    P.text_bytes = b.text_hi;
    P.n_matches = ctl_at<uint64_t>(e, kCtlTotal);
    P.want_pos = (b.need_csr || e->progs.n_inord_groups > 0) ? 1 : 0;
    P.prio = e->opt_scan_prio;
    P.dbg = e->opt_scan_dbg;
}

static uint64_t grid_waves(const gft_engine* e, uint64_t work) {
    const uint64_t wpw = e->plan.scan_waves;
    return std::min<uint64_t>(std::max<uint64_t>((work + wpw - 1) / wpw, 1), e->n_cus) * wpw;
}
constexpr uint64_t slab_floor(ScanKernel k) { return k == ScanKernel::scan3 ? 2 * kScan3MinRoom : 64; }
static uint32_t slab_size(const gft_engine* e) {
    const uint64_t n_waves = (uint64_t)e->n_cus * e->plan.scan_waves;
    return (uint32_t)std::min<uint64_t>(kScan2Slab, std::max<uint64_t>(slab_floor(e->plan.kernel), e->pool_cap / (2 * n_waves)));
}

static ScanParams dfa_params(const gft_engine* e, const ScanBatch& b) {
    ScanParams P;
    fill_common(e, b, P);
    const AcTables& tab = e->tables.tab;
    const auto& d = e->d_tabs.dfa;
    P.byte_class = d.byte_class.as<uint8_t>(); P.delta = d.delta.as<uint32_t>();
    P.out_term = d.out_term.as<uint32_t>(); P.out_link = d.out_link.as<uint32_t>();
    P.term_len = d.term_len.as<uint32_t>();
    P.n_classes = tab.n_classes; P.n_states = tab.n_states; P.n_lds_states = e->plan.n_lds_states;
    P.max_term_len = tab.max_term_len;
    return P;
}

static Scan3Params scan3_params(const gft_engine* e, const ScanBatch& b) {
    Scan3Params P;
    fill_window(e, b, P);
    const Scan3Tables& s3 = e->tables.s3;
    const auto& d = e->d_tabs.s3;
    P.cls = P.fold ? d.cls_fold.as<uint8_t>() : d.cls.as<uint8_t>();
    P.filter = d.filter.as<uint32_t>(); P.filter_words = (uint32_t)s3.filter.size();
    P.short3 = d.short3.as<uint8_t>(); P.short3_bytes = (uint32_t)s3.short3.size();
    P.srec = d.srec.as<uint32_t>(); P.srec_words = (uint32_t)s3.srec.size();
    P.short3_big = s3.short3_big.empty() ? nullptr : d.short3_big.as<uint32_t>();
    P.srec_big = d.srec_big.as<uint32_t>();
    P.bloom = d.bloom.as<uint32_t>(); P.bloom_lg = s3.bloom_lg; P.bloom_lds = s3.bloom_lg <= kScan3BloomLdsLg ? 1 : 0;
    P.slots = d.slots.as<Scan2Slot>(); P.slot_shift = s3.slot_shift; P.slot_seed = s3.slot_seed;
    P.more = d.more.as<Scan2Slot>();
    P.term_blob = d.term_blob.as<uint8_t>(); P.term_off = d.term_off.as<uint32_t>();
    P.G = s3.G; P.grouped = s3.grouped ? 1 : 0;
    P.cand_cap = e->plan.scan3_cand_cap;
    P.slab = slab_size(e);
    return P;
}

static Scan2Params scan2_params(const gft_engine* e, const ScanBatch& b) {
    Scan2Params P;
    fill_window(e, b, P);
    const Scan2Tables& s2 = e->tables.s2;
    const Scan3Tables& s3 = e->tables.s3;
    const gft_engine::TableBufs& d = e->d_tabs;
    P.filter = d.s2.filter.as<uint32_t>(); P.filter_words = (uint32_t)s2.filter.size();
    P.hashed = s2.hashed ? 1 : 0; P.hash_shift = s2.hash_shift;
    P.short3 = d.s2.short3.as<uint8_t>(); P.short3_bytes = (uint32_t)s2.short3.size();
    P.fpt = d.s2.fpt.as<uint8_t>(); P.fpt_lg = s2.fpt_lg;
    P.shorts_packed = d.s2.shorts_packed.as<uint32_t>(); P.shorts_words = (uint32_t)std::min<size_t>(s2.shorts_packed.size(), 255 * 3);
    P.short3_big = s2.short3_big.empty() ? nullptr : d.s2.short3_big.as<uint32_t>();
    P.cand_cap = e->plan.scan2_cand_cap;
    P.slots = d.s2.slots.as<Scan2Slot>(); P.slot_shift = s2.slot_shift; P.slot_seed = s2.slot_seed;
    P.more = d.s2.more.as<Scan2Slot>();
    P.cls = P.fold ? d.s2.cls_fold.as<uint8_t>() : d.s2.cls.as<uint8_t>();
    P.term_blob = d.s2.term_blob.as<uint8_t>(); P.term_off = d.s2.term_off.as<uint32_t>();
    P.kp = s2.kp; P.pad_class = s2.pad_class;
    P.ordered = (b.need_csr && e->opt_scan_ordered) ? 1 : 0;
    P.dbg_counters = (P.dbg & (2 | 64)) ? e->d_dbg.as<uint64_t>() : nullptr;
    P.slab = slab_size(e);
    if (e->plan.kernel == ScanKernel::scan4) {
        const uint64_t n_waves = (uint64_t)e->n_cus * e->plan.scan_waves;
        P.chunk_units = (uint32_t)std::min<uint64_t>(kScan4ChunkUnits, std::max<uint64_t>(1, b.n_docs / (n_waves * 4)));
        if (e->opt_scan4_chunk) P.chunk_units = std::min<uint32_t>(e->opt_scan4_chunk, kScan4ChunkUnits);
        P.cand_cap = e->plan.scan4_fifo[P.want_pos ? 1 : 0];
        P.bound_q16 = (uint32_t)std::min<double>(e->learned.scan4_density * 1.6 * 65536.0 + 1.0, 4.0e9);
        P.bound_add = 48;
        P.round_c = e->opt_scan4_round ? std::min<uint32_t>(64, std::max<uint32_t>(16, e->opt_scan4_round & ~15u)) : 64;
        const uint64_t chunk_need = (uint64_t)P.chunk_units * (((uint64_t)b.unit_max * P.bound_q16 >> 16) + P.bound_add);
        P.slab = (uint32_t)std::min<uint64_t>(std::max<uint64_t>(kScan2Slab, 4 * chunk_need), std::max<uint64_t>(chunk_need, e->pool_cap / (2 * n_waves)));
    } else if (e->plan.kernel == ScanKernel::scan5) {
        P.s5_filter = d.s5.filter.as<uint64_t>(); P.s5_dual = (uint32_t)e->s5.filter.size();
        P.s5_grp = P.fold ? d.s5.grp_fold.as<uint8_t>() : d.s5.grp.as<uint8_t>();
        P.s5_G = e->s5.G; P.s5_pad_g = e->s5.pad_group;
        P.s5_fifo_cap = e->plan.s5plan.fifo_cap; P.cand_cap = e->plan.s5plan.cand_cap;
        P.s5_sG = 0; P.s5_sgrp = nullptr; P.s5_srec_big = nullptr;
        if (e->plan.s5_short_groups) {
            P.short3 = d.s3.short3.as<uint8_t>(); P.short3_bytes = (uint32_t)s3.short3.size();
            P.shorts_packed = d.s3.srec.as<uint32_t>(); P.shorts_words = (uint32_t)s3.srec.size();
            P.short3_big = s3.short3_big.empty() ? nullptr : d.s3.short3_big.as<uint32_t>();
            P.s5_srec_big = d.s3.srec_big.as<uint32_t>();
            P.s5_sgrp = P.fold ? d.s3.cls_fold.as<uint8_t>() : d.s3.cls.as<uint8_t>();
            P.s5_sG = s3.G;
        }
        P.s5_term_bits = e->plan.s5_term_bits; P.s5_pos_bias = e->plan.s5_pos_bias;
        P.s5_bloom = e->plan.s5_bloom_lg ? d.s5.bloom.as<uint32_t>() : nullptr; P.s5_bloom_lg = e->plan.s5_bloom_lg;
    }
    return P;
}

static int enqueue_scan(gft_engine* e, const ScanBatch& b, ScanLaunch& L) {
    hipStream_t st = e->stream;
    const ScanKernel k = e->plan.kernel;
    ScanParams Pd; Scan3Params P3; Scan2Params P2;
    uint64_t work = b.n_units, slab = 0;
    L.ordered = false;
    if (k == ScanKernel::dfa) Pd = dfa_params(e, b);
    else if (k == ScanKernel::scan3) { P3 = scan3_params(e, b); slab = P3.slab; }
    else {
        if (e->opt_scan_dbg & (2 | 64)) {
            HIP_TRY(e->d_dbg.ensure(128), "debug alloc");
            HIP_TRY(hipMemsetAsync(e->d_dbg.p, 0, 128, st), "memset");
        }
        P2 = scan2_params(e, b); slab = P2.slab;
        L.ordered = P2.ordered != 0;
        if (k == ScanKernel::scan4) work = (b.n_units + P2.chunk_units - 1) / P2.chunk_units;
    }
    L.static_slabs = counts_slabs(k) ? grid_waves(e, work) * slab : 0;
    {
        ProfScope ps(e, "scan");
        HIP_TRY(k == ScanKernel::dfa     ? launch_scan_units(Pd, e->n_cus, st)
                : k == ScanKernel::scan2 ? launch_scan2(P2, e->plan.scan_waves, e->n_cus, st)
                : k == ScanKernel::scan3 ? launch_scan3(P3, e->plan.scan_waves, e->n_cus, st)
                : k == ScanKernel::scan4 ? launch_scan4(P2, e->plan.scan_waves, e->n_cus, st)
                                         : launch_scan5(P2, e->n_cus, st), "scan kernel launch");
    }
    if (on_scan2_tables(k) && (e->opt_scan_dbg & 64)) {
        const uint64_t n_units = b.n_units;
        uint64_t t[16];
        HIP_TRY(hipMemcpyAsync(t, e->d_dbg.p, sizeof t, hipMemcpyDeviceToHost, st), "debug read-back");
        HIP_TRY(hipStreamSynchronize(st), "debug read-back");
        if (k == ScanKernel::scan5) fprintf(stderr, "[gft scan debug] scan5 (G=%u, list %u):\n", e->s5.G, e->plan.s5plan.cand_cap);
        if (k == ScanKernel::scan4)
            fprintf(stderr, "[gft scan debug] scan4 wave cycles per unit: chunk set-up %.0f, filter %.0f, queue push %.0f, stage A issue %.0f, stage A %.0f, stage B %.0f, flush %.0f, unit records %.0f\n",
                    (double)t[4] / n_units, (double)t[5] / n_units, (double)t[6] / n_units, (double)t[7] / n_units, (double)t[8] / n_units,
                    (double)t[9] / n_units, (double)t[10] / n_units, (double)t[11] / n_units);
        else
            fprintf(stderr, "[gft scan debug] wave cycles per unit: first bytes %.0f, filter %.0f, list %.0f, stage A %.0f (scan5: trips %.0f + stage-B issue and short-term trips %.0f), stage B %.0f, flush %.0f, unit record %.0f\n",
                (double)t[4] / n_units, (double)t[5] / n_units, (double)t[6] / n_units, (double)(t[7] + t[10]) / n_units, (double)t[10] / n_units, (double)t[7] / n_units,
                (double)t[8] / n_units, (double)t[9] / n_units, (double)t[11] / n_units);
        double sum = 0;
        for (int ph = 4; ph < 12; ph++) sum += (double)t[ph];
        if (t[13]) fprintf(stderr, "[gft scan debug] %llu waves: mean %.0f cycles in all, the slowest %.0f (+%.1f %%)\n", (unsigned long long)t[13],
                           sum / (double)t[13], (double)t[12], 100.0 * ((double)t[12] * (double)t[13] / sum - 1.0));
    }
    return GFT_OK;
}

static void learn_from_batch(gft_engine* e, const ScanLaunch& L, const BatchVerdict& v) {
    const ScanKernel k = e->plan.kernel;
    learn(e->learned, k, k == ScanKernel::scan5 ? e->plan.s5plan.fifo_cap : kScan2FifoCap, L.ordered, v.total, v.text_lo, v.text_hi);
    e->learned.unit_entries = v.n_units ? (uint32_t)std::min<uint64_t>((v.total + v.n_units - 1) / v.n_units, 0xFFFFFFFFu) : 0u;
}

enum class UnitRoute {
    host,
    single,
    deferred,
    counted,
};
constexpr const char* kUnitRouteName[] = {"host", "single", "deferred", "counted"};
constexpr uint64_t kHostUnitDocs = 1024;

struct UnitTable {
    gft_engine* e;
    uint64_t n_units = 0, text_lo = 0, text_hi = 0;
    std::vector<uint64_t> h_base;
    std::vector<Unit> h_units;
    bool drain = false;
    explicit UnitTable(gft_engine* e_) : e(e_) {}
    ~UnitTable() { if (drain && e->stream) (void)hipStreamSynchronize(e->stream); }
};

static int build_unit_table(gft_engine* e, UnitRoute route, const uint64_t* d_doc_off, const uint64_t* h_doc_off, uint64_t n_docs,
                            uint32_t unit_max, uint64_t cap_units, ScanLaunch& L, UnitTable& t) {
    hipStream_t st = e->stream;
    HIP_TRY(e->d_ctl.ensure(kCtlBytes), "control alloc");
    HIP_TRY(e->d_unit_cnt.ensure(n_docs * 4), "unit alloc");
    HIP_TRY(e->d_unit_base.ensure((n_docs + 1) * 8), "unit alloc");
    HIP_TRY(e->d_partial.ensure(scan_partials_needed(n_docs) * 8), "unit alloc");
    if (route != UnitRoute::single) HIP_TRY(hipMemsetAsync(e->d_ctl.p, 0, kCtlBatchClear, st), "memset");
    auto room = [&]() -> int {
        HIP_TRY(e->d_units.ensure(t.n_units * sizeof(Unit)), "unit alloc");
        HIP_TRY(e->d_unit_start.ensure(t.n_units * 8), "unit alloc");
        HIP_TRY(e->d_unit_count.ensure(t.n_units * 4), "unit alloc");
        HIP_TRY(e->d_unit_out.ensure((t.n_units + 1) * 8), "unit alloc");
        HIP_TRY(e->d_partial.ensure(scan_partials_needed(std::max(t.n_units, n_docs)) * 8), "unit alloc");
        return GFT_OK;
    };
    auto count = [&]() -> int {
        ProfScope ps(e, "aux");
        HIP_TRY(launch_unit_count(d_doc_off, n_docs, unit_max, e->d_unit_cnt.as<uint32_t>(), ctl_at<uint32_t>(e, kCtlBad), st), "unit_count");
        HIP_TRY(launch_exclusive_scan(e->d_unit_cnt.as<uint32_t>(), n_docs, e->d_unit_base.as<uint64_t>(),
                                      e->d_partial.as<uint64_t>(), st), "unit scan");
        HIP_TRY(launch_pack_ctl(e->d_unit_base.as<uint64_t>(), d_doc_off, n_docs, ctl_at<uint64_t>(e, kCtlUnits), st), "unit scan");
        return GFT_OK;
    };
    int rc;
    switch (route) {
    case UnitRoute::host: {
        t.drain = true;
        t.h_base.assign(n_docs + 1, 0);
        for (uint64_t d = 0; d < n_docs; d++) {
            if (h_doc_off[d + 1] < h_doc_off[d]) return fail(e, GFT_E_INVALID, "doc_off is not ascending");
            const uint64_t n = h_doc_off[d + 1] - h_doc_off[d];
            if (n > 0xFFFFFFFFull) return fail(e, GFT_E_UNSUPPORTED, "a document is longer than 4 GiB - 1 bytes (positions are 32-bit)");
            const uint64_t k = n <= unit_max ? 1 : (n + unit_max - 1) / unit_max;
            t.h_base[d + 1] = t.h_base[d] + k;
            for (uint64_t i = 0; i < k; i++) t.h_units.push_back(unit_slice((uint32_t)d, n, k, i, unit_max));
        }
        t.n_units = t.h_base[n_docs]; t.text_lo = h_doc_off[0]; t.text_hi = h_doc_off[n_docs];
        HIP_TRY(hipMemcpyAsync(e->d_unit_base.p, t.h_base.data(), (n_docs + 1) * 8, hipMemcpyHostToDevice, st), "unit upload");
        if ((rc = room())) return rc;
        ProfScope ps(e, "aux");
        if (t.n_units) HIP_TRY(hipMemcpyAsync(e->d_units.p, t.h_units.data(), t.n_units * sizeof(Unit), hipMemcpyHostToDevice, st), "unit upload");
        return GFT_OK;
    }
    case UnitRoute::single: {
        {
            ProfScope ps(e, "aux");
            HIP_TRY(launch_units_single(d_doc_off, n_docs, unit_max, e->d_units.as<Unit>(), e->d_unit_base.as<uint64_t>(),
                                        ctl_at<uint32_t>(e, kCtlBad), e->ctl_epoch, st), "unit table");
        }
        t.n_units = n_docs; t.text_lo = 0; t.text_hi = ~0ull;
        L.deferred = L.single = true; L.epoch = e->ctl_epoch;
        L.unit_cap = L.n_docs = n_docs;
        if ((rc = room())) return rc;
        ProfScope ps(e, "aux");
        return GFT_OK;
    }
    case UnitRoute::deferred: {
        if ((rc = count())) return rc;
        L.deferred = true;
        t.n_units = cap_units; t.text_lo = 0; t.text_hi = ~0ull;
        L.unit_cap = cap_units; L.n_docs = n_docs;
        if ((rc = room())) return rc;
        ProfScope ps(e, "aux");
        HIP_TRY(hipMemsetAsync(e->d_units.p, 0, t.n_units * sizeof(Unit), st), "memset");
        HIP_TRY(launch_unit_fill(d_doc_off, n_docs, e->d_unit_base.as<uint64_t>(), e->d_units.as<Unit>(), unit_max, st, t.n_units), "unit_fill");
        HIP_TRY(launch_clamp_u64(e->d_unit_base.as<uint64_t>(), n_docs + 1, t.n_units, st), "unit clamp");
        return GFT_OK;
    }
    case UnitRoute::counted: {
        if ((rc = count())) return rc;
        uint64_t raw[kCtlWords] = {};
        HIP_TRY(hipMemcpyAsync(raw, e->d_ctl.p, sizeof raw, hipMemcpyDeviceToHost, st), "readback");
        HIP_TRY(hipStreamSynchronize(st), "sync");
        const CtlBlock c = decode_ctl(raw);
        t.n_units = c.n_units; t.text_lo = c.text_lo; t.text_hi = c.text_hi;
        count_streak(e->learned, t.n_units, n_docs);
        if (t.text_hi < t.text_lo) return fail(e, GFT_E_INVALID, "doc_off is not ascending");
        if (c.bad) return fail(e, GFT_E_INVALID, "doc_off is not ascending, or a document is longer than 4 GiB - 1 bytes (positions are 32-bit)");
        if ((rc = room())) return rc;
        ProfScope ps(e, "aux");
        HIP_TRY(launch_unit_fill(d_doc_off, n_docs, e->d_unit_base.as<uint64_t>(), e->d_units.as<Unit>(), unit_max, st), "unit_fill");
        return GFT_OK;
    }
    }
    return GFT_E_INTERNAL;
}

int scan_pipeline(gft_engine* e, const uint8_t* d_text, const uint64_t* d_doc_off, uint64_t n_docs, uint32_t flags,
                  bool need_csr, BatchVerdict& v, const uint64_t* h_doc_off, ScanLaunch* defer) {
    hipStream_t st = e->stream;
    v = BatchVerdict();
    ScanLaunch L;
    if (defer) *defer = L;
    e->pool = PoolState();
    e->solve_unit_entries = e->learned.unit_entries;
// ... 303 lines not shown
```

### gofindthem_amd/csrc/gft_scan5.hip

```cpp
#include <hip/hip_runtime.h>

#include <cstdlib>
#include <type_traits>

#include "gft_kernels.hpp"
#include "gft_wave_dev.hpp"

namespace gft {


namespace {

#include "gft_scan2_dev.hpp"
#include "gft_foldsafe_dev.hpp"

constexpr int kWays5 = 2;

struct Ctx5 {
    uint32_t* fifo;
    uint32_t fifo_cap;
    uint32_t nf;
    uint32_t npend;
    bool lost;
    bool direct;
    uint64_t dbase;
    uint32_t term_bits, pos_base;
};
typedef __attribute__((address_space(3))) uint32_t lds_w32;
__device__ __forceinline__ lds_w32* scan5_seen(const Ctx5& o) { return (lds_w32*)(o.fifo + o.fifo_cap + kScan5SurvX); }

template <bool POS>
__device__ __forceinline__ void out_append(Ctx5& o, bool em, uint32_t term, uint32_t pos) {
    const uint64_t mask = __ballot(em);
    if (em) {
        const uint32_t idx = o.nf + wave_rank(mask);
        if (!o.direct) {
            if (idx < o.fifo_cap - o.npend) o.fifo[idx] = POS ? term | (pos - o.pos_base) << o.term_bits : term;
        } else {
            KARG(pool_term)[o.dbase + idx] = term;
            if (POS) KARG(pool_pos)[o.dbase + idx] = pos;
        }
    }
    o.nf += (uint32_t)__popcll(mask);
    if (!o.direct && o.nf + o.npend > o.fifo_cap) o.lost = true;
}

template <bool POS>
__device__ __forceinline__ void short_trip(const Ctx& c, Ctx5& o, uint32_t ubase, uint32_t n) {
    const uint32_t lane = lane_id();
    const bool on = lane < n;
    const uint32_t job = o.fifo[o.fifo_cap - 1 - (o.npend - n) - (on ? lane : 0)];
    o.npend -= n;
    const uint32_t p = ubase + (job & 0xFFFFu);
    uint32_t sid = on ? job >> 16 : 0;
    if (!POS && sid && p >= 3) {
        const uint32_t bit = 1u << (sid & 31);
        if (__hip_atomic_fetch_or(scan5_seen(o) + (sid >> 5), bit, __ATOMIC_RELAXED, __HIP_MEMORY_SCOPE_WAVEFRONT) & bit) sid = 0;
    }
    uint32_t r[3] = {0, 0, 0};
    if (sid) {
        const uint32_t* src = c.lrec + 3 * sid;
        r[0] = src[0]; r[1] = src[1]; r[2] = src[2];
    }
#pragma unroll
    for (uint32_t j = 0; j < 3; j++) {
        if (j && !__any(r[j] != 0)) break;
        const uint32_t L = r[j] >> 28;
        out_append<POS>(o, r[j] != 0 && L <= p + 1, r[j] & 0x0FFFFFFFu, POS ? (c.P.pos_end ? p : p + 1 - L) : 0u);
    }
}
template <bool POS>
__device__ __forceinline__ void park_short(const Ctx& c, Ctx5& o, uint32_t ubase, uint32_t rel, uint32_t sid, uint32_t x3) {
    if (!__any(sid != 0)) return;
    if (__builtin_expect(__any(sid == 255) && KARG(short3_big) != nullptr, 0)) {
        uint32_t r[3] = {0, 0, 0};
        const uint32_t p = ubase + rel;
        if (sid) short_record(c, sid, x3, r);
#pragma unroll
        for (uint32_t j = 0; j < 3; j++) {
            const uint32_t L = r[j] >> 28;
            out_append<POS>(o, r[j] != 0 && L <= p + 1, r[j] & 0x0FFFFFFFu, POS ? (c.P.pos_end ? p : p + 1 - L) : 0u);
        }
        return;
    }
    const uint64_t m = __ballot(sid != 0);
    const uint32_t n = (uint32_t)__popcll(m);
    if (o.npend + n > o.fifo_cap / 2) {
        wave_lds_fence();
        while (o.npend) short_trip<POS>(c, o, ubase, o.npend < 64 ? o.npend : 64);
        wave_lds_fence();
    }
    if (!o.direct && o.nf + o.npend + n > o.fifo_cap) o.lost = true;
    if (sid) o.fifo[o.fifo_cap - 1 - o.npend - wave_rank(m)] = rel | sid << 16;
    o.npend += n;
}

template <bool POS>
__device__ __forceinline__ void short_trip_g(const Ctx& c, Ctx5& o, lds_u8* lsg, uint32_t ubase, uint32_t n) {
    const Scan2Params& P = c.P;
    const uint32_t lane = lane_id();
    const bool on = lane < n;
    const uint32_t job = o.fifo[o.fifo_cap - 1 - (o.npend - n) - (on ? lane : 0)];
    o.npend -= n;
    const uint32_t p = ubase + (job & 0xFFFFu);
    uint32_t sid = on ? job >> 16 : 0;
    const Text8 t8 = cand_load(c, p);
    const uint32_t W = P.fold ? fold4(t8.w) : t8.w;
    if (__builtin_expect(__any(sid == 255), 0)) {
        const uint32_t G = P.s5_sG;
        const uint32_t x3 = (lsg[(t8.w >> 8) & 0xFF] * G + lsg[(t8.w >> 16) & 0xFF]) * G + lsg[t8.w >> 24];
        const bool b = sid == 255;
        uint32_t cnt = 0;
        const uint32_t* g = nullptr;
        if (b) { g = KARG(s5_srec_big) + KARG(short3_big)[x3]; cnt = g[0]; }
        for (uint32_t j = 0; __any(j < cnt); j++) {
            uint32_t w0 = 0, w1 = 0;
            if (j < cnt) { w0 = g[1 + 2 * j]; w1 = g[2 + 2 * j]; }
            const uint32_t L = w0 >> 28;
            const bool ok = w0 != 0 && L <= p + 1 && ((W ^ w1) >> ((32 - 8 * L) & 31)) == 0;
            out_append<POS>(o, ok, w0 & 0x0FFFFFFFu, POS ? (P.pos_end ? p : p + 1 - L) : 0u);
        }
        if (b) sid = 0;
    }
    if (!__any(sid != 0)) return;
    const uint32_t* r = c.lrec + sid * kScan3RecWords;
#pragma unroll
    for (uint32_t j = 0; j < 3; j++) {
        const uint32_t w0 = sid ? r[2 * j] : 0;
        if (j && !__any(w0 != 0)) break;
        const uint32_t L = w0 >> 28;
        const bool ok = w0 != 0 && L <= p + 1 && ((W ^ r[2 * j + 1]) >> ((32 - 8 * L) & 31)) == 0;
        out_append<POS>(o, ok, w0 & 0x0FFFFFFFu, POS ? (P.pos_end ? p : p + 1 - L) : 0u);
    }
}
template <bool POS>
__device__ __forceinline__ void park_short_g(const Ctx& c, Ctx5& o, lds_u8* lsg, uint32_t ubase, uint32_t rel, uint32_t sid) {
    if (!__any(sid != 0)) return;
    const uint64_t m = __ballot(sid != 0);
    const uint32_t n = (uint32_t)__popcll(m);
    if (o.npend + n > o.fifo_cap / 2) {
        wave_lds_fence();
        while (o.npend) short_trip_g<POS>(c, o, lsg, ubase, o.npend < 64 ? o.npend : 64);
        wave_lds_fence();
    }
    if (!o.direct && o.nf + o.npend + n > o.fifo_cap) o.lost = true;
    if (sid) o.fifo[o.fifo_cap - 1 - o.npend - wave_rank(m)] = rel | sid << 16;
    o.npend += n;
}

template <bool POS>
__device__ __forceinline__ void finish_long5(const Ctx& c, Ctx5& o, bool on, uint32_t rel, const Cand& k, const Slot& s0, const Slot& s1,
                                             Front t, uint32_t tl, Deferred& d) {
    const Scan2Params& P = c.P;
    Slot e;
    const bool have = slot_pick(k.x, s0, s1, e) && on;
    if (!__any(have)) return;
    const bool multi = have && (e.a.y & kScan2Multi);
    uint32_t folded = 0;
    {
        const bool act = have && !multi;
        const uint32_t kmax = wave_kmax(act ? e.a.z & kScan2LenMask : 0);
        if (P.fold) front_fold_upto(t, folded, kmax);
        const bool ok = act && entry_ok(c, k.p, t, tl, e, kmax);
        out_append<POS>(o, ok, e.a.y, POS ? match_pos(P, k.p, e.a.z) : 0u);
    }
    if (!__any(multi)) return;
    const uint32_t n_ent = multi ? e.a.z : 0, more_at = e.a.y & ~kScan2Multi;
    const uint32_t tot = lane_value(wave_incl_scan(n_ent), 63);
    if (tot <= d.cap - d.n) {
        for (uint32_t j = 0; __any(j < n_ent); j++) {
            const uint64_t m = __ballot(j < n_ent);
            if (j < n_ent)
                d.list[d.n + wave_rank(m)] = make_uint2(rel, more_at + j);
            d.n += (uint32_t)__popcll(m);
        }
        return;
    }
    Slot cur = e;
    if (multi) cur = slot_load(&KARG(more)[more_at]);
    for (uint32_t j = 0; __any(j < n_ent); j++) {
        const bool act = j < n_ent;
        Slot nxt = cur;
        if (j + 1 < n_ent) nxt = slot_load(&KARG(more)[more_at + j + 1]);
        const uint32_t kmax = wave_kmax(act ? cur.a.z & kScan2LenMask : 0);
        if (P.fold) front_fold_upto(t, folded, kmax);
        const bool ok = act && entry_ok(c, k.p, t, tl, cur, kmax);
        out_append<POS>(o, ok, cur.a.y, POS ? match_pos(P, k.p, cur.a.z) : 0u);
        cur = nxt;
    }
}


template <bool POS>
__device__ __forceinline__ void drain_deferred5(const Ctx& c, Ctx5& o, uint32_t ubase, Deferred& d) {
    const Scan2Params& P = c.P;
    const uint32_t lane = lane_id();
    wave_lds_fence();
    const Scan2Slot* more = KARG(more);
    for (uint32_t i0 = 0; i0 < d.n; i0 += 64) {
        const bool on = i0 + lane < d.n;
        const uint2 it = d.list[on ? i0 + lane : 0];
        const uint32_t p = ubase + it.x;
        const Slot e = slot_load(&more[it.y]);
        const Text8 t8 = cand_load(c, p);
        Front t = front_load(c, p, t8.tw);
        const uint32_t tl = tail_load(c, p);
        const uint32_t kmax = wave_kmax(on ? e.a.z & kScan2LenMask : 0);
        uint32_t folded = 0;
        if (P.fold) front_fold_upto(t, folded, kmax);
        const bool ok = on && entry_ok(c, p, t, tl, e, kmax);
        out_append<POS>(o, ok, e.a.y, POS ? match_pos(P, p, e.a.z) : 0u);
    }
    d.n = 0;
    __builtin_amdgcn_wave_barrier();
}

template <bool FPT_LDS, bool DBG, bool SG, bool POS>
__global__ void __launch_bounds__(kScan2Threads) k_scan5(const Scan2Params P) {
    extern __shared__ __align__(16) uint8_t smem[];
    uint8_t* grp = smem;
    uint8_t* cls = smem + 256;
    uint8_t* sgrp = smem + 512;
    uint64_t* dual = reinterpret_cast<uint64_t*>(smem + 768);
    uint8_t* short3 = reinterpret_cast<uint8_t*>(dual + P.s5_dual);
    uint8_t* fpt = short3 + P.short3_bytes;
    const uint32_t bloom_lg = FPT_LDS ? 0u : __builtin_amdgcn_readfirstlane(P.s5_bloom_lg);
    const uint32_t bloom_bytes = bloom_lg ? (1u << bloom_lg) / 8 : 0u;
    uint32_t* lrec = reinterpret_cast<uint32_t*>(fpt + (FPT_LDS ? kScan2FptSize : bloom_bytes));
    uint32_t* wg_next = reinterpret_cast<uint32_t*>(smem + (((size_t)(reinterpret_cast<uint8_t*>(lrec) - smem) + P.shorts_words * 4 + 15) & ~(size_t)15));
    uint8_t* wave_lds_all = reinterpret_cast<uint8_t*>(wg_next) + 16;

    for (uint32_t i = threadIdx.x; i < 256; i += blockDim.x) { grp[i] = P.s5_grp[i]; cls[i] = P.cls[i]; sgrp[i] = SG ? P.s5_sgrp[i] : 0; }
    for (uint32_t i = threadIdx.x; i < P.s5_dual; i += blockDim.x) dual[i] = P.s5_filter[i];
    for (uint32_t i = threadIdx.x; i < P.short3_bytes / 4; i += blockDim.x)
        reinterpret_cast<uint32_t*>(short3)[i] = reinterpret_cast<const uint32_t*>(P.short3)[i];
    for (uint32_t i = threadIdx.x; FPT_LDS && i < kScan2FptSize / 4; i += blockDim.x)
        reinterpret_cast<uint32_t*>(fpt)[i] = reinterpret_cast<const uint32_t*>(P.fpt)[i];
    for (uint32_t i = threadIdx.x; !FPT_LDS && i < bloom_bytes / 4; i += blockDim.x) reinterpret_cast<uint32_t*>(fpt)[i] = P.s5_bloom[i];
    for (uint32_t i = threadIdx.x; i < P.shorts_words; i += blockDim.x) lrec[i] = P.shorts_packed[i];
    if (threadIdx.x == 0) { wg_next[0] = kScan5Waves; wg_next[1] = wg_next[2] = wg_next[3] = 0; }
    __syncthreads();
    if (DBG && (P.dbg & 128)) return;

    const uint32_t lane = lane_id(), wave = __builtin_amdgcn_readfirstlane(threadIdx.x >> 6);
    uint8_t* wave_lds = wave_lds_all + (size_t)wave * (P.s5_fifo_cap * 4 + kScan5SurvX * 4 + kScan5SeenWords * 4 + ((P.cand_cap * 2 + 15) & ~15u));
    uint32_t* fifo = reinterpret_cast<uint32_t*>(wave_lds);
    uint32_t* survx = fifo + P.s5_fifo_cap;
    uint16_t* cand = reinterpret_cast<uint16_t*>(survx + kScan5SurvX + kScan5SeenWords);
    const uint32_t G = __builtin_amdgcn_readfirstlane(P.s5_G);
    const uint32_t kp = __builtin_amdgcn_readfirstlane(P.kp), kp2 = __builtin_amdgcn_readfirstlane(kp * kp);
    lds_u8* lgrp = (lds_u8*)0;
    typedef uint32_t u32x2 __attribute__((ext_vector_type(2)));
    typedef __attribute__((address_space(3))) const u32x2 lds_u64;
    lds_u64* ldual = (lds_u64*)768;
    lds_u8* lsg = (lds_u8*)512;
    if ((uint32_t)(uintptr_t)(lds_u8*)smem != 0) __builtin_trap();

    unsigned long long tl[8] = {0, 0, 0, 0, 0, 0, 0, 0}, tprev = DBG ? clock64() : 0;
    auto mark = [&](int ph) {
        if (DBG && (P.dbg & 64)) { const unsigned long long now = clock64(); tl[ph] += now - tprev; tprev = now; }
    };
    auto static_slabs = [&]() { return (uint64_t)gridDim.x * kScan5Waves * KARG(slab); };
    uint64_t slab_next = ((uint64_t)blockIdx.x * kScan5Waves + wave) * KARG(slab);
    uint32_t wave_matches = 0;
    bool told_nonascii = !(P.fold && P.nonascii);
    uint32_t slab_left = KARG(slab);

    constexpr uint32_t wg_waves = kScan5Waves;
    const uint32_t round_units = gridDim.x * wg_waves, wg_first = blockIdx.x * wg_waves;
    auto unit_of = [&](uint32_t item) -> uint64_t { return (uint64_t)(item / wg_waves) * round_units + (wg_first + item % wg_waves); };
    uint64_t u = unit_of(wave), nu = 0;
    Unit un_n;
    uint64_t abs_n, end_n;
    auto request_unit = [&](uint64_t k) {
        un_n = P.units[k < P.n_units ? k : P.n_units - 1];
        abs_n = P.doc_off[un_n.doc]; end_n = P.doc_off[un_n.doc + 1];
    };
    auto units_arrived = [&]() { asm volatile("" : : "v"(un_n.doc), "v"(un_n.lo), "v"(un_n.hi), "v"(abs_n), "v"(end_n)); };
    request_unit(u);
    units_arrived();
    const uint8_t* text_n = KARG(text);
    for (; u < P.n_units; u = nu) {
        const Unit un{(uint32_t)__builtin_amdgcn_readfirstlane(un_n.doc), (uint32_t)__builtin_amdgcn_readfirstlane(un_n.lo),
                      (uint32_t)__builtin_amdgcn_readfirstlane(un_n.hi)};
        const uint64_t doc_abs = (uint64_t)(uint32_t)__builtin_amdgcn_readfirstlane((uint32_t)(abs_n >> 32)) << 32 |
                                 (uint32_t)__builtin_amdgcn_readfirstlane((uint32_t)abs_n);
        const uint64_t end_v = end_n;
        const Ctx c{P, cls, nullptr, P.short3_bytes ? short3 : nullptr, fpt, lrec, text_n + doc_abs, doc_abs, kp2,
                    doc_abs < 7, doc_abs < 23, un.lo, un.hi, doc_abs + un.hi + 4 > KARG(text_bytes), DBG ? P.dbg : 0u};
        const uint32_t nborder = un.lo < kScan2MaxOff ? un.lo : kScan2MaxOff;
        const uint32_t ubase = un.lo - kScan2MaxOff;
        const uint32_t own = un.hi - un.lo;
        const uint32_t C = ((own + 63) / 64 + 3) & ~3u;
        const uint32_t my_lo = un.lo + lane * C;
        const uint32_t my_hi = my_lo + C < un.hi ? my_lo + C : un.hi;
        const uint32_t nvalid = my_lo < un.hi ? my_hi - my_lo : 0;
        Ctx5 o{fifo, P.s5_fifo_cap, 0, 0, false, false, 0, POS ? P.s5_term_bits : 0u, POS ? un.lo - P.s5_pos_bias : 0u};

        const uint8_t* src = c.dbase + my_lo;
        uint32_t hist = 0;
        U128u nxt{0, 0, 0, 0};
        if (nvalid) {
            if (doc_abs + my_lo >= 4) hist = load_u32_unaligned(src - 4);
            else for (uint32_t i = 1; i <= 3 && i <= doc_abs + my_lo; i++) hist |= (uint32_t)src[-(int)i] << (32 - 8 * i);
            nxt = *reinterpret_cast<const U128u*>(src);
        }
        {
            uint32_t item = 0;
            if (lane == 0) item = __hip_atomic_fetch_add(wg_next, 1u, __ATOMIC_RELAXED, __HIP_MEMORY_SCOPE_WORKGROUP);
            nu = unit_of((uint32_t)__builtin_amdgcn_readfirstlane(item));
        }
        mark(7);
        request_unit(nu);

        uint32_t m0 = 0, m1 = 0, m2 = 0, m3 = 0;
        if (own) {
            uint32_t h1 = P.s5_pad_g, h2 = P.s5_pad_g, h3 = P.s5_pad_g, pq = 0;
            (void)h2;
            if (nvalid) {
                if (my_lo >= 1) h1 = lgrp[hist >> 24];
                if (my_lo >= 2) h2 = lgrp[(hist >> 16) & 0xFF];
                if (my_lo >= 3) h3 = lgrp[(hist >> 8) & 0xFF];
            }
            pq = mad24s(h2, G, h1);
            mark(0);
            uint32_t acc = 0, njobs = 0, hib = 0;
            const uint32_t ndw = C >> 2;
            const uint32_t npieces = (ndw + 3) >> 2;
            for (uint32_t q = 0; q < npieces; q++) {
                const uint32_t w[4] = {nxt.x, nxt.y, nxt.z, nxt.w};
                if (q * 16 < nvalid) hib |= (w[0] | w[1]) | (w[2] | w[3]);
                if constexpr (SG) {
                    if (!told_nonascii)
                        fold_job_push(q * 16 < nvalid && (((w[0] | w[1]) | (w[2] | w[3])) & 0x80808080u) != 0, lane * C + q * 16, cand, P.cand_cap, njobs);
                }
                if (q + 1 < npieces && (q + 1) * 16 < nvalid) nxt = *reinterpret_cast<const U128u*>(src + (q + 1) * 16);
                const uint32_t nd = ndw - 4 * q;
                auto dword = [&](uint32_t wd) {
                    const uint32_t c0 = lgrp[wd & 0xFF], c1 = lgrp[(wd >> 8) & 0xFF], c2 = lgrp[(wd >> 16) & 0xFF], c3 = lgrp[wd >> 24];
                    const uint32_t xa = mad24s(pq, G, c0);
                    const uint32_t xb = mad24s(mad24s(c0, G, c1), G, c2);
                    const u32x2 fa = ldual[xa], fb = ldual[xb];
                    acc = __builtin_amdgcn_alignbit(fa.x >> h3, acc, 1);
                    acc = __builtin_amdgcn_alignbit(fa.y >> c1, acc, 1);
                    acc = __builtin_amdgcn_alignbit(fb.x >> h1, acc, 1);
                    acc = __builtin_amdgcn_alignbit(fb.y >> c3, acc, 1);
                    pq = mad24s(c2, G, c3);
                    h3 = c1; h2 = c2; h1 = c3;
                };
                if (nd >= 4) {
                    uint32_t cc[19];
                    cc[0] = h3; cc[1] = h2; cc[2] = h1;
#pragma unroll
                    for (int i = 0; i < 16; i++) cc[3 + i] = lgrp[(w[i >> 2] >> (8 * (i & 3))) & 0xFF];
                    uint32_t xk[8];
                    xk[0] = mad24s(pq, G, cc[3]);
#pragma unroll
                    for (int t = 1; t < 8; t++) xk[t] = mad24s(mad24s(cc[1 + 2 * t], G, cc[2 + 2 * t]), G, cc[3 + 2 * t]);
                    u32x2 fk[8];
#pragma unroll
                    for (int t = 0; t < 8; t++) fk[t] = ldual[xk[t]];
#pragma unroll
                    for (int t = 0; t < 8; t++) {
                        acc = __builtin_amdgcn_alignbit(fk[t].x >> cc[2 * t], acc, 1);
                        acc = __builtin_amdgcn_alignbit(fk[t].y >> cc[4 + 2 * t], acc, 1);
                    }
                    pq = mad24s(cc[17], G, cc[18]);
                    h3 = cc[16]; h2 = cc[17]; h1 = cc[18];
                } else {
                    dword(w[0]);
                    if (nd >= 2) dword(w[1]);
                    if (nd >= 3) dword(w[2]);
                }
                if ((q & 1) && nd >= 4) {
                    if ((q >> 1) == 0) m0 = acc; else if ((q >> 1) == 1) m1 = acc; else if ((q >> 1) == 2) m2 = acc; else m3 = acc;
                }
            }
            if (ndw & 7) {
                const uint32_t v = acc >> (32 - 4 * (ndw & 7));
                const uint32_t k = ndw >> 3;
                if (k == 0) m0 = v; else if (k == 1) m1 = v; else if (k == 2) m2 = v; else m3 = v;
            }
            if (!SG && !told_nonascii && __any((hib & 0x80808080u) != 0)) {
                for (uint32_t q = 0; q < npieces; q++)
                    fold_job_push((hib & 0x80808080u) != 0 && q * 16 < nvalid, lane * C + q * 16, cand, P.cand_cap, njobs);
            }
            if (njobs && !told_nonascii) {
                uint32_t bits = 1u;
                if (njobs <= P.cand_cap) {
                    FOLD_JOB_VARS(fj_);
                    bits = fold_jobs_begin(KARG(text), end_v, doc_abs + un.lo, own, un.lo == 0, cand, njobs, FOLD_JOB_PASS(fj_)) || fold_jobs_finish(FOLD_JOB_PASS(fj_)) ? 2u : 0u;
                }
                if (bits) { told_nonascii = true; if (lane == 0) atomicOr(KARG(nonascii), bits); }
            }
            m0 = nvalid >= 32 ? m0 : (nvalid ? m0 & ((1u << nvalid) - 1) : 0);
            m1 = nvalid >= 64 ? m1 : (nvalid > 32 ? m1 & ((1u << (nvalid - 32)) - 1) : 0);
            m2 = nvalid >= 96 ? m2 : (nvalid > 64 ? m2 & ((1u << (nvalid - 64)) - 1) : 0);
            m3 = nvalid >= 128 ? m3 : (nvalid > 96 ? m3 & ((1u << (nvalid - 96)) - 1) : 0);
        }
        mark(1);
        units_arrived();

        if (DBG && P.dbg) {
            if (P.dbg & 2) {
                uint32_t f = __popc(m0) + __popc(m1) + __popc(m2) + __popc(m3);
                for (int s = 32; s; s >>= 1) f += __shfl_xor(f, s, 64);
                if (lane == 0) atomicAdd(reinterpret_cast<unsigned long long*>(KARG(dbg_counters)), (unsigned long long)f);
            }
            if (P.dbg & 1) m0 = m1 = m2 = m3 = 0;
        }

        const uint32_t f = __popc(m0) + __popc(m1) + __popc(m2) + __popc(m3) + (lane == 0 ? nborder : 0);
        const uint32_t fincl = wave_incl_scan(f);
        const uint32_t ftotal = lane_value(fincl, 63);
        for (uint32_t walk = 0; walk < 2 && ftotal; walk++) {
            o.nf = 0; o.npend = 0; o.lost = false;
            if (lane < kScan5SeenWords) scan5_seen(o)[lane] = 0;
            for (uint32_t l0 = 0; l0 < 64;) {
                const uint32_t before = l0 ? lane_value_at(fincl, l0 - 1) : 0;
                const bool fits = lane >= l0 && fincl - before <= P.cand_cap;
                const uint64_t fm = __ballot(fits) >> l0;
                const uint32_t nl = fm == ~0ull >> l0 ? 64 - l0 : (uint32_t)__builtin_ctzll(~fm);
                const uint32_t l1 = l0 + nl;
                const uint32_t ptotal = lane_value_at(fincl, l1 - 1) - before;
                if (lane >= l0 && lane < l1) {
                    uint32_t wpos = fincl - f - before;
                    if (lane == 0)
                        for (uint32_t i = 0; i < nborder; i++) cand[wpos++] = (uint16_t)(kScan2MaxOff - nborder + i);
                    uint32_t mm[4] = {m0, m1, m2, m3};
                    const uint32_t rel = lane * C + kScan2MaxOff;
#pragma unroll
                    for (int k = 0; k < 4; k++) {
                        uint32_t mk = mm[k];
                        while (mk) {
                            const uint32_t i = __builtin_ctz(mk);
                            mk &= mk - 1;
                            cand[wpos++] = (uint16_t)(rel + 32 * k + i);
                        }
                    }
                }
                wave_lds_fence();
                mark(2);
                uint32_t ns = 0;
                bool n_on[kWays5];
                uint32_t n_rel[kWays5];
                Text8 n_tx[kWays5];
                auto fetch = [&](uint32_t i0) {
#pragma unroll
                    for (int q = 0; q < kWays5; q++) {
                        const uint32_t i = i0 + 64 * q + lane;
                        n_on[q] = i < ptotal;
                        n_rel[q] = cand[n_on[q] ? i : 0];
                    }
#pragma unroll
                    for (int q = 0; q < kWays5; q++) n_tx[q] = cand_load(c, ubase + n_rel[q]);
                };
                fetch(0);
                for (uint32_t i0 = 0; i0 < ptotal; i0 += 64 * kWays5) {
                    bool on[kWays5];
                    uint32_t rel[kWays5];
                    Text8 tx[kWays5];
                    Cand k[kWays5];
#pragma unroll
                    for (int q = 0; q < kWays5; q++) { on[q] = n_on[q]; rel[q] = n_rel[q]; tx[q] = n_tx[q]; }
                    if (i0 + 64 * kWays5 < ptotal) fetch(i0 + 64 * kWays5);
#pragma unroll
                    for (int q = 0; q < kWays5; q++) {
                        cand_keys<!SG>(c, ubase + rel[q], tx[q], k[q]);
                        if (SG && P.short3_bytes) {
                            const uint32_t wq = tx[q].w, sG = P.s5_sG;
                            k[q].sid = short3[mad24s(mad24s(lsg[(wq >> 8) & 0xFF], sG, lsg[(wq >> 16) & 0xFF]), sG, lsg[wq >> 24])];
                        }
                    }
#pragma unroll
                    for (int q = 0; q < kWays5; q++) {
                        if (FPT_LDS || !bloom_lg) cand_decide<FPT_LDS>(c, k[q]);
                        else {
                            const uint32_t* bl = reinterpret_cast<const uint32_t*>(fpt);
                            const uint32_t hg = scan5_bloom_g(k[q].x, (k[q].tw >> 24) & 0xDFu, bloom_lg), hx = scan5_bloom_x(k[q].x, bloom_lg);
                            const uint32_t wg = bl[hg >> 5], wx = bl[hx >> 5];
                            k[q].go_long = false;
                            if (((wg >> (hg & 31)) | (wx >> (hx & 31))) & 1u) cand_decide<false>(c, k[q]);
                        }
                    }
#pragma unroll
                    for (int q = 0; q < kWays5; q++)
                        if (i0 + 64 * q < ptotal)
                        {
                            const uint32_t sidq = on[q] && rel[q] >= kScan2MaxOff ? k[q].sid : 0;
                            if (SG) park_short_g<POS>(c, o, lsg, ubase, rel[q], sidq); else park_short<POS>(c, o, ubase, rel[q], sidq, k[q].x3);
                        }
                    const uint64_t below = (1ull << lane) - 1;
#pragma unroll
                    for (int q = 0; q < kWays5; q++) {
                        const bool keep = on[q] && k[q].go_long;
                        const uint64_t sb = __ballot(keep);
                        if (keep) {
                            const uint32_t at = ns + (uint32_t)__popcll(sb & below);
                            cand[at] = (uint16_t)rel[q];
                            if (at < kScan5SurvX) survx[at] = k[q].x;
                        }
                        ns += (uint32_t)__popcll(sb);
                    }
                }
                wave_lds_fence();
                mark(6);
                static_assert(kScan5SurvX >= 64, "the first stage-B trip takes its keys from survx");
                const bool b_on = lane < ns;
                const uint32_t b_rel = ns ? cand[b_on ? lane : 0] : 0;
                Cand b_k;
                b_k.p = ubase + b_rel; b_k.x3 = 0; b_k.sid = 0; b_k.go_long = true; b_k.x = 0; b_k.tw = 0;
                Slot b_s0{}, b_s1{};
                Text8 b_t8{0, 0};
                Front b_fr{};
                uint32_t b_tl = 0;
                if (ns) {
                    b_k.x = survx[b_on ? lane : 0];
                    b_s0 = slot_load(&P.slots[scan2_pair_slot(b_k.x, 0, P.slot_shift, P.slot_seed)]);
                    b_s1 = slot_load(&P.slots[scan2_pair_slot(b_k.x, 1, P.slot_shift, P.slot_seed)]);
                    if (!c.near24 && !c.near_end) {
                        const U128u v1 = *reinterpret_cast<const U128u*>(c.dbase + (int64_t)b_k.p - 23);
                        const U128u v2 = *reinterpret_cast<const U128u*>(c.dbase + (int64_t)b_k.p - 7);
                        b_fr.f[4] = v1.x; b_fr.f[3] = v1.y; b_fr.f[2] = v1.z; b_fr.f[1] = v1.w;
                        b_t8.tw = v2.x; b_t8.w = v2.y;
                        b_tl = v2.z;
                    } else {
                        b_t8 = cand_load(c, b_k.p);
                        b_fr = front_load(c, b_k.p, 0);
                        b_tl = tail_load(c, b_k.p);
                    }
                }
                while (o.npend) { if (SG) short_trip_g<POS>(c, o, lsg, ubase, o.npend < 64 ? o.npend : 64); else short_trip<POS>(c, o, ubase, o.npend < 64 ? o.npend : 64); }
                if (DBG && (P.dbg & 2)) { if (lane == 0) atomicAdd(reinterpret_cast<unsigned long long*>(KARG(dbg_counters) + 2), (unsigned long long)ns); }
                mark(3);
                Deferred dfr;
                dfr.list = reinterpret_cast<uint2*>(reinterpret_cast<uint8_t*>(cand) + ((ns * 2 + 7) & ~7u));
                dfr.cap = (P.cand_cap * 2 - ((ns * 2 + 7) & ~7u)) / 8;
                dfr.n = 0;
                if (ns) {
                    b_k.tw = b_t8.tw;
                    b_fr.f[0] = b_t8.tw;
                    finish_long5<POS>(c, o, b_on, b_rel, b_k, b_s0, b_s1, b_fr, b_tl, dfr);
                }
                for (uint32_t i0 = 64; i0 < ns; i0 += 64) {
                    const bool on = i0 + lane < ns;
                    const uint32_t rel = cand[on ? i0 + lane : 0];
                    const uint32_t p = ubase + rel;
                    Cand k;
                    k.p = p; k.x3 = 0; k.sid = 0; k.go_long = true;
                    if (i0 + 64 <= kScan5SurvX) {
                        k.x = survx[on ? i0 + lane : 0];
                        const Slot s0 = slot_load(&P.slots[scan2_pair_slot(k.x, 0, P.slot_shift, P.slot_seed)]);
                        const Slot s1 = slot_load(&P.slots[scan2_pair_slot(k.x, 1, P.slot_shift, P.slot_seed)]);
                        const Text8 t8 = cand_load(c, p);
                        const Front fr = front_load(c, p, t8.tw);
                        const uint32_t tl5 = tail_load(c, p);
                        k.tw = t8.tw;
                        finish_long5<POS>(c, o, on, rel, k, s0, s1, fr, tl5, dfr);
                    } else {
                        const Text8 t8 = cand_load(c, p);
                        const Front fr = front_load(c, p, t8.tw);
                        const uint32_t tl5 = tail_load(c, p);
                        cand_keys<false>(c, p, t8, k);
                        const Slot s0 = slot_load(&P.slots[scan2_pair_slot(k.x, 0, P.slot_shift, P.slot_seed)]);
                        const Slot s1 = slot_load(&P.slots[scan2_pair_slot(k.x, 1, P.slot_shift, P.slot_seed)]);
                        finish_long5<POS>(c, o, on, rel, k, s0, s1, fr, tl5, dfr);
                    }
                }
                if (dfr.n) drain_deferred5<POS>(c, o, ubase, dfr);
                wave_lds_fence();
                l0 = l1;
                mark(4);
            }
            if (o.direct || !o.lost) break;
            {
                const uint32_t nh = o.nf;
                if (nh > slab_left) {
                    const uint32_t want = nh > KARG(slab) ? nh : KARG(slab);
                    uint64_t nb = 0;
                    if (lane == 0) nb = atomicAdd(reinterpret_cast<unsigned long long*>(KARG(cursor)), (unsigned long long)want);
                    slab_next = static_slabs() + __shfl(nb, 0, 64);
                    slab_left = want;
                }
                o.dbase = slab_next;
                o.direct = true;
                if (slab_next + nh > KARG(pool_cap)) break;
            }
        }
        text_n = KARG(text);
        if (ftotal) {
            const uint32_t nh = o.nf;
            if (!o.direct && nh > slab_left) {
                const uint32_t want = nh > KARG(slab) ? nh : KARG(slab);
                uint64_t nb = 0;
                if (lane == 0) nb = atomicAdd(reinterpret_cast<unsigned long long*>(KARG(cursor)), (unsigned long long)want);
                slab_next = static_slabs() + __shfl(nb, 0, 64);
                slab_left = want;
            }
            const uint64_t base = slab_next;
            slab_next += nh;
            slab_left -= nh;
            wave_matches += nh;
            const bool room = base + nh <= KARG(pool_cap);
            if (lane == 0) { KARG(unit_start)[u] = base; KARG(unit_count)[u] = room ? nh : 0u; }
            if (room && !o.direct) {
                const uint32_t tmask = POS ? (1u << o.term_bits) - 1u : 0u;
                for (uint32_t i = lane; i < nh; i += 64) {
                    const uint32_t e = fifo[i];
                    if constexpr (POS) {
                        __builtin_nontemporal_store(e & tmask, &KARG(pool_term)[base + i]);
                        __builtin_nontemporal_store(o.pos_base + (e >> o.term_bits), &KARG(pool_pos)[base + i]);
                    } else {
                        __builtin_nontemporal_store(e, &KARG(pool_term)[base + i]);
                    }
                }
            }
            __builtin_amdgcn_wave_barrier();
            mark(5);
        } else if (lane == 0) {
            KARG(unit_start)[u] = slab_next; KARG(unit_count)[u] = 0;
        }
    }
    if (lane == 0) {
        if (wave_matches)
            __hip_atomic_fetch_add(reinterpret_cast<unsigned long long*>(wg_next + 2), (unsigned long long)wave_matches, __ATOMIC_RELAXED,
                                   __HIP_MEMORY_SCOPE_WORKGROUP);
        const uint32_t done = __hip_atomic_fetch_add(wg_next + 1, 1u, __ATOMIC_ACQ_REL, __HIP_MEMORY_SCOPE_WORKGROUP) & 0x7FFFFFFFu;
        if (done + 1 == kScan5Waves) {
            const unsigned long long all = __hip_atomic_load(reinterpret_cast<unsigned long long*>(wg_next + 2), __ATOMIC_RELAXED,
                                                             __HIP_MEMORY_SCOPE_WORKGROUP);
            if (all) atomicAdd(reinterpret_cast<unsigned long long*>(KARG(n_matches)), all);
        }
    }
    if (DBG && (P.dbg & 64) && lane == 0 && KARG(dbg_counters)) {
        unsigned long long all = 0;
        for (int ph = 0; ph < 8; ph++) { atomicAdd(reinterpret_cast<unsigned long long*>(KARG(dbg_counters) + 4 + ph), tl[ph]); all += tl[ph]; }
        atomicMax(reinterpret_cast<unsigned long long*>(KARG(dbg_counters) + 12), all);
        atomicAdd(reinterpret_cast<unsigned long long*>(KARG(dbg_counters) + 13), 1ull);
    }
}

}

static size_t scan5_fixed_lds(uint32_t dual_entries, uint32_t short3_bytes, uint32_t shorts_words, uint32_t fpt_lds_bytes) {
    return ((768 + (size_t)dual_entries * 8 + short3_bytes + fpt_lds_bytes + (size_t)shorts_words * 4 + 15) & ~(size_t)15) + 16;
}
static size_t scan5_wave_lds(uint32_t fifo_cap, uint32_t cand_cap) {
    return (size_t)fifo_cap * 4 + kScan5SurvX * 4 + kScan5SeenWords * 4 + (((size_t)cand_cap * 2 + 15) & ~(size_t)15);
}

bool scan5_plan(uint32_t kp, uint32_t short3_bytes, uint32_t shorts_words, uint32_t fpt_lds_bytes, size_t lds_max, uint32_t fifo_cap, Scan5Plan* out) {
    const uint32_t g_hi = kp < kScan5MaxGroups ? kp : kScan5MaxGroups;
    const uint32_t g_lo = g_hi > 8 + 12 ? g_hi - 8 : (g_hi < 12 ? g_hi : 12);
    for (uint32_t G = g_hi; G >= g_lo; G--) {
        const uint32_t ent = G * G * G;
        const size_t fixed = scan5_fixed_lds(ent, short3_bytes, shorts_words, fpt_lds_bytes);
        const size_t need = fixed + (size_t)kScan5Waves * scan5_wave_lds(fifo_cap, kScan5CandCapMin);
        if (need > lds_max) continue;
        const size_t spare = ((lds_max - need) / kScan5Waves / 2) & ~(size_t)7;
        out->G = G; out->dual_entries = ent;
        out->cand_cap = (uint32_t)std::min<size_t>(kScan5CandCapMin + spare, 2048);
        out->fifo_cap = fifo_cap;
        return true;
    }
    return false;
}

hipError_t launch_scan5(const Scan2Params& P, unsigned n_cus, hipStream_t st) {
    if (!P.n_units) return hipSuccess;
    const bool fl = P.fpt_lg == 0;
    const size_t lds = scan5_fixed_lds(P.s5_dual, P.short3_bytes, P.shorts_words, fl ? kScan2FptSize : P.s5_bloom_lg ? (1u << P.s5_bloom_lg) / 8 : 0) +
                       (size_t)kScan5Waves * scan5_wave_lds(P.s5_fifo_cap, P.cand_cap);
    using Kern = void (*)(const Scan2Params);
    const auto pick = [&](auto pos) -> Kern {
        constexpr bool POS = decltype(pos)::value;
#ifdef GFT_S5_SG_CLOCKS
        if (P.s5_sG && P.dbg && fl) return k_scan5<true, true, true, POS>;
#endif
        if (P.s5_sG) return fl ? k_scan5<true, false, true, POS> : k_scan5<false, false, true, POS>;
        if (P.dbg) return fl ? k_scan5<true, true, false, POS> : k_scan5<false, true, false, POS>;
        return fl ? k_scan5<true, false, false, POS> : k_scan5<false, false, false, POS>;
    };
    const Kern fn = P.want_pos ? pick(std::true_type{}) : pick(std::false_type{});
    hipError_t e = hipFuncSetAttribute(reinterpret_cast<const void*>(fn), hipFuncAttributeMaxDynamicSharedMemorySize, (int)lds);
    if (e != hipSuccess) return e;
    uint64_t g = (P.n_units + kScan5Waves - 1) / kScan5Waves;
    const unsigned grid = (unsigned)(g < n_cus ? (g ? g : 1) : n_cus);
    fn<<<dim3(grid), dim3(kScan5Waves * 64), lds, st>>>(P);
    return hipGetLastError();
}

}
```

### include/gft.h

```cpp
#ifndef GFT_H
#define GFT_H

#include <stdint.h>

#ifdef __cplusplus
extern "C" {
#endif

typedef enum gft_status {
    GFT_OK = 0,
    GFT_E_INVALID = -1,
    GFT_E_NOT_BUILT = -2,
    GFT_E_HIP = -3,
    GFT_E_UNSUPPORTED = -4,
    GFT_E_PARSE = -5,
    GFT_E_ENGINE = -6,
    GFT_E_NOMEM = -7,
    GFT_E_INTERNAL = -8,
    GFT_W_NO_RCCL = 1
} gft_status;

#define GFT_POS_START 0u
#define GFT_POS_END 1u
#define GFT_FOLD_ASCII 1u
// ... 343 lines not shown
                                    int* lowered);
int gft_finder_mark_device(gft_finder* f, const uint8_t* d_text_blob, const uint64_t* d_doc_off, uint64_t n_docs, const uint64_t* d_span_off,
                           const uint32_t* d_span_start, const uint32_t* d_span_len, int spans_lowered, int source, const uint8_t* open,
                           uint32_t open_len, const uint8_t* close, uint32_t close_len, uint32_t flags, uint8_t* d_out, uint64_t cap_bytes,
                           uint64_t* d_out_off, uint32_t* d_span_new, uint64_t* d_doc_run_off, uint64_t* n_runs, uint64_t* total_bytes,
                           int* lowered);
int gft_finder_replace_device(gft_finder* f, const uint8_t* d_text_blob, const uint64_t* d_doc_off, uint64_t n_docs, const uint64_t* d_span_off,
                              const uint32_t* d_span_start, const uint32_t* d_span_len, int spans_lowered, int source,
                              const uint32_t* d_span_term, const uint32_t* term_rep, const uint8_t* rep_bytes, const uint64_t* rep_off,
                              uint32_t n_reps, uint32_t flags, uint8_t* d_out, uint64_t cap_bytes, uint64_t* d_out_off, uint64_t* d_doc_run_off,
                              uint32_t* d_run_new, uint32_t* d_run_len, uint32_t* d_run_rep, uint64_t cap_runs, uint64_t* n_runs,
                              uint64_t* total_bytes, int* lowered);
int gft_finder_term_stats_device(gft_finder* f, const uint8_t* d_text_blob, const uint64_t* d_doc_off, uint64_t n_docs,
                                 const uint32_t* d_hit_bitmap, const uint32_t* want, uint32_t flags, uint64_t doc_base, uint64_t* d_occ,
                                 uint64_t* d_docs, uint64_t* d_first, int* lowered);
int gft_finder_top_docs_device(gft_finder* f, const uint8_t* d_text_blob, const uint64_t* d_doc_off, uint64_t n_docs,
                               const uint32_t* d_hit_bitmap, const uint32_t* want, const uint32_t* weights, uint32_t flags, uint32_t k,
                               uint64_t doc_base, uint64_t* d_score, uint64_t* d_top_idx, uint64_t* d_top_score, uint64_t* n_top, int* lowered);
int gft_finder_process_device_begin(gft_finder* f, const uint8_t* d_text_blob, const uint64_t* d_doc_off, uint64_t n_docs,
                                    uint32_t* d_hit_bitmap);
int gft_finder_process_device_end(gft_finder* f);
int gft_finder_set_whole_words(gft_finder* f, int on);
int gft_finder_whole_words(const gft_finder* f);
int gft_finder_lowered_batches(const gft_finder* f, uint64_t* on_device, uint64_t* on_host);
int gft_finder_compact_device(gft_finder* f, const uint32_t* d_hit_bitmap, uint64_t n_docs, uint64_t* d_row_off,
                              uint32_t* d_expr_idx, uint32_t* d_tag_id, uint64_t cap, uint64_t* total);
int gft_finder_debug_add_literal(gft_finder* f, int which, const uint8_t* lit, uint32_t len);
int gft_finder_debug_set_updated(gft_finder* f, int updated_sub, int updated_rgx);
int gft_finder_debug_get_updated(const gft_finder* f, int* updated_sub, int* updated_rgx);

typedef struct gft_group gft_group;
int gft_group_create(gft_group** out, gft_finder* finder);
void gft_group_destroy(gft_group* g);
const char* gft_group_last_error(const gft_group* g);
int gft_group_add_rule(gft_group* g, const uint8_t* name, uint64_t name_len, const uint8_t* expr, uint64_t expr_len);
int gft_group_state(const gft_group* g, char* out, uint64_t cap, uint64_t* needed);
int gft_group_process_jsons(gft_group* g, const uint8_t* json_blob, const uint64_t* doc_off, uint64_t n_docs,
                            const uint8_t* include_json, uint64_t include_len, const uint8_t* exclude_json,
                            uint64_t exclude_len, int what, char* out, uint64_t cap, uint64_t* needed);
int gft_group_last_result(const gft_group* g, char* out, uint64_t cap, uint64_t* needed);
int gft_group_evaluate(gft_group* g, const uint8_t* tagmap_json, uint64_t len, char* out, uint64_t cap, uint64_t* needed);
int gft_group_last_batch(const gft_group* g, uint64_t* leaves, uint64_t* bytes);
int gft_group_set_schema(gft_group* g, const uint8_t* paths_blob, const uint64_t* path_off, uint32_t n_fields,
                         const uint8_t* include_json, uint64_t include_len, const uint8_t* exclude_json, uint64_t exclude_len);
uint32_t gft_group_n_rule_exprs(gft_group* g);
int gft_group_rule_expr(gft_group* g, uint32_t i, const uint8_t** name, uint32_t* name_len, const uint8_t** expr, uint32_t* expr_len);
int gft_group_process_records_device(gft_group* g, const uint8_t* d_text_blob, const uint64_t* d_leaf_off, const uint32_t* d_leaf_field,
                                     const uint64_t* d_rec_off, uint64_t n_records, uint64_t n_leaves, uint32_t* d_rule_bitmap);
int gft_group_process_records(gft_group* g, const uint8_t* text_blob, const uint64_t* leaf_off, const uint32_t* leaf_field,
                              const uint64_t* rec_off, uint64_t n_records, uint64_t n_leaves, uint32_t* rule_bitmap);
int gft_debug_eval_rules(gft_group* g, const uint32_t* hit_bitmap, uint32_t n_exprs, const uint32_t* leaf_field, const uint64_t* rec_off,
                         uint64_t n_records, uint64_t n_leaves, uint32_t* rule_bitmap);
int gft_debug_eval_rules_device(gft_group* g, const uint32_t* d_hit_bitmap, uint32_t n_exprs, const uint32_t* d_leaf_field,
                                const uint64_t* d_rec_off, uint64_t n_records, uint64_t n_leaves, uint32_t* d_rule_bitmap);
int gft_group_tag_records_device(gft_group* g, const uint8_t* d_text_blob, const uint64_t* d_leaf_off, const uint32_t* d_leaf_field,
                                 const uint64_t* d_rec_off, uint64_t n_records, uint64_t n_leaves, uint64_t* d_row_off, uint32_t* d_ent_field,
                                 uint32_t* d_ent_expr, uint32_t* d_ent_tag, uint64_t cap, uint64_t* total);
int gft_group_tag_records(gft_group* g, const uint8_t* text_blob, const uint64_t* leaf_off, const uint32_t* leaf_field, const uint64_t* rec_off,
                          uint64_t n_records, uint64_t n_leaves, uint64_t* row_off, uint32_t* ent_field, uint32_t* ent_expr, uint32_t* ent_tag,
                          uint64_t cap, uint64_t* total);
int gft_group_tag_jsons_device(gft_group* g, const uint8_t* d_json_blob, const uint64_t* d_doc_off, uint64_t n_docs, uint8_t* d_status,
                               uint64_t* d_row_off, uint32_t* d_ent_field, uint32_t* d_ent_expr, uint32_t* d_ent_tag, uint64_t cap,
                               uint64_t* total);
int gft_group_tag_jsons_schema(gft_group* g, const uint8_t* json_blob, const uint64_t* doc_off, uint64_t n_docs, char* out, uint64_t cap,
                               uint64_t* needed);
int gft_group_tag_jsons_auto(gft_group* g, const uint8_t* json_blob, const uint64_t* doc_off, uint64_t n_docs, const uint8_t* include_json,
                             uint64_t include_len, const uint8_t* exclude_json, uint64_t exclude_len, char* out, uint64_t cap,
                             uint64_t* needed);
int gft_debug_tag_entries(gft_group* g, const uint32_t* hit_bitmap, uint32_t n_exprs, const uint32_t* leaf_field, const uint64_t* rec_off,
                          uint64_t n_records, uint64_t n_leaves, uint64_t* row_off, uint32_t* ent_field, uint32_t* ent_expr, uint32_t* ent_tag,
                          uint64_t cap, uint64_t* total);
int gft_debug_tag_entries_device(gft_group* g, const uint32_t* d_hit_bitmap, uint32_t n_exprs, const uint32_t* d_leaf_field,
                                 const uint64_t* d_rec_off, uint64_t n_records, uint64_t n_leaves, uint64_t* d_row_off, uint32_t* d_ent_field,
                                 uint32_t* d_ent_expr, uint32_t* d_ent_tag, uint64_t cap, uint64_t* total);
enum gft_json_status {
    GFT_JSON_OK = 0,
    GFT_JSON_SYNTAX = 1,
    GFT_JSON_DEPTH = 2,
    GFT_JSON_PATH = 3,
    GFT_JSON_KEY = 4,
    GFT_JSON_DUP = 5,
    GFT_JSON_TEXT = 6
};
int gft_group_json_leaves_device(gft_group* g, const uint8_t* d_json_blob, const uint64_t* d_doc_off, uint64_t n_docs, uint8_t* d_status,
                                 uint64_t* d_rec_off, uint32_t* d_leaf_field, uint64_t* d_leaf_off, uint64_t leaf_cap, uint8_t* d_text,
                                 uint64_t text_cap, uint64_t* totals);
int gft_group_process_jsons_device(gft_group* g, const uint8_t* d_json_blob, const uint64_t* d_doc_off, uint64_t n_docs, uint8_t* d_status,
                                   uint32_t* d_rule_bitmap);
int gft_group_process_jsons_schema(gft_group* g, const uint8_t* json_blob, const uint64_t* doc_off, uint64_t n_docs, char* out, uint64_t cap,
                                   uint64_t* needed);
int gft_group_json_last(const gft_group* g, uint64_t* n_device, uint64_t* n_host);
int gft_group_rules_json_device(gft_group* g, const uint32_t* d_rule_bitmap, uint64_t n_docs, const uint64_t* d_hole_len, uint8_t* d_out,
                                uint64_t cap, uint64_t* d_out_off, uint64_t* total);
int gft_debug_rules_json(gft_group* g, const uint32_t* rule_bitmap, uint64_t n_docs, const uint64_t* hole_len, uint8_t* out, uint64_t cap,
                         uint64_t* out_off, uint64_t* total);
#define GFT_TAGS_JSON_MAX_LEAVES 1024
int gft_group_tags_json_device(gft_group* g, const uint32_t* d_hit_bitmap, const uint32_t* d_leaf_field, const uint64_t* d_rec_off,
                               uint64_t n_records, uint64_t n_leaves, const uint64_t* d_hole_len, uint8_t* d_out, uint64_t cap,
                               uint64_t* d_out_off, uint64_t* total);
int gft_debug_tags_json(gft_group* g, const uint32_t* hit_bitmap, uint32_t n_exprs, const uint32_t* leaf_field, const uint64_t* rec_off,
                        uint64_t n_records, uint64_t n_leaves, const uint64_t* hole_len, uint8_t* out, uint64_t cap, uint64_t* out_off,
                        uint64_t* total);
int gft_group_json_paths_device(gft_group* g, const uint8_t* d_json_blob, const uint64_t* d_doc_off, uint64_t n_docs, uint8_t* paths_blob,
                                uint64_t blob_cap, uint64_t* path_off, uint64_t path_cap, uint64_t* needed, uint64_t* n_paths, uint64_t* dropped);
int gft_group_process_jsons_auto(gft_group* g, const uint8_t* json_blob, const uint64_t* doc_off, uint64_t n_docs, const uint8_t* include_json,
                                 uint64_t include_len, const uint8_t* exclude_json, uint64_t exclude_len, char* out, uint64_t cap,
                                 uint64_t* needed);
int gft_group_process_json_lines(gft_group* g, const uint8_t* blob, uint64_t len, const uint8_t* include_json, uint64_t include_len,
                                 const uint8_t* exclude_json, uint64_t exclude_len, char* out, uint64_t cap, uint64_t* needed);
int gft_group_json_auto_last(const gft_group* g, uint64_t* n_paths, uint64_t* dropped, uint64_t* recompiled);
int gft_debug_emulate_json_paths(gft_group* g, const uint8_t* json_blob, const uint64_t* doc_off, uint64_t n_docs, uint8_t* paths_blob,
                                 uint64_t blob_cap, uint64_t* path_off, uint64_t path_cap, uint64_t* needed, uint64_t* n_paths, uint64_t* dropped,
                                 uint64_t* hashes, uint64_t hash_cap, uint64_t* n_hashes);
int gft_debug_json_paths_ref(gft_group* g, const uint8_t* json_blob, const uint64_t* doc_off, uint64_t n_docs, uint8_t* paths_blob, uint64_t blob_cap,
                             uint64_t* path_off, uint64_t path_cap, uint64_t* needed, uint64_t* n_paths);
int gft_debug_json_leaves_ref(gft_group* g, const uint8_t* json_blob, const uint64_t* doc_off, uint64_t n_docs, uint8_t* status, uint64_t* rec_off,
                              uint32_t* leaf_field, uint64_t* leaf_off, uint64_t leaf_cap, uint8_t* text, uint64_t text_cap, uint64_t* totals);
int gft_debug_emulate_json_leaves(gft_group* g, const uint8_t* json_blob, const uint64_t* doc_off, uint64_t n_docs, uint8_t* status,
                                  uint64_t* rec_off, uint32_t* leaf_field, uint64_t* leaf_off, uint64_t leaf_cap, uint8_t* text, uint64_t text_cap,
                                  uint64_t* totals);
int64_t gft_debug_json_schema_find(gft_group* g, int64_t parent, const uint8_t* key, uint32_t key_len, int64_t* field);
int gft_group_dsl_parse(const uint8_t* expr, uint64_t len, char* out, uint64_t cap, uint64_t* needed);
int gft_group_dsl_tokens(const uint8_t* expr, uint64_t len, char* out, uint64_t cap, uint64_t* needed);

int gft_dsl_parse(const uint8_t* expr, uint64_t len, int case_sensitive, char* out, uint64_t cap, uint64_t* needed);
int gft_dsl_tokens(const uint8_t* expr, uint64_t len, char* out, uint64_t cap, uint64_t* needed);
int gft_regex_required_literals(const uint8_t* pattern, uint64_t len, char* out, uint64_t cap, uint64_t* needed);
int gft_to_lower(const uint8_t* in, uint64_t len, uint8_t* out, uint64_t cap, uint64_t* needed);

int gft_profile_enable(gft_engine* e, int on);
int gft_profile_read(gft_engine* e, const char* name, double* total_ms, uint64_t* launches);
int gft_profile_reset(gft_engine* e);

int gft_engine_create_multi(gft_engine** out, const int* devices, int n_devices);
int gft_n_devices(const gft_engine* e);
const char* gft_gather_mode(const gft_engine* e);
gft_engine* gft_device_engine(gft_engine* e, int i);
int gft_split_docs(const gft_engine* e, const uint64_t* doc_off, uint64_t n_docs, uint64_t* cut);
int gft_process_device_multi(gft_engine* e, const uint8_t* const* d_text, const uint64_t* const* d_doc_off, const uint64_t* n_docs,
                             uint32_t flags, uint32_t* d_bitmap_root);

int gft_debug_emulate_scan(const uint8_t* terms_blob, const uint64_t* term_off, uint32_t n_terms, const uint8_t* text,
                           uint32_t len, uint32_t lo, uint32_t flags, uint32_t scan_flags, uint32_t* out_term,
                           uint32_t* out_pos, uint64_t cap, uint64_t* needed);

int gft_debug_scan5_filter(const uint8_t* terms_blob, const uint64_t* term_off, uint32_t n_terms, const uint8_t* text, uint32_t len,
                           uint32_t lane_start, uint32_t scan_flags, uint32_t groups, uint8_t* out_exact, uint8_t* out_dual,
                           uint32_t* groups_used);

int gft_debug_tables(const uint8_t* terms_blob, const uint64_t* term_off, uint32_t n_terms, const uint8_t* blob, uint64_t blob_len,
                     uint64_t lds_max, const char* forced_kernel, const char** kernel, uint8_t* out, uint64_t cap, uint64_t* needed,
                     char* err, uint64_t err_cap);
int gft_debug_learned_unit(const gft_engine* e, uint32_t* unit_max, uint32_t* fifo_cap);
int gft_debug_last_unit_route(const gft_engine* e, const char** name);
int gft_debug_last_fold_bits(const gft_engine* e, uint32_t* bits);
int gft_debug_scan_plan(const uint8_t* terms_blob, const uint64_t* term_off, uint32_t n_terms, uint64_t lds_max, const char* forced_kernel,
                        const char** kernel, uint32_t* plan);
int gft_debug_pool_entries(const gft_engine* e, uint64_t* entries);
int gft_debug_last_solve_pf(const gft_engine* e, uint32_t* pf_terms, uint32_t* unit_entries);

int gft_debug_judge_batch(const uint64_t* ctl_words, int single, uint32_t epoch, uint64_t n_docs, uint64_t unit_cap, uint64_t pool_cap,
                          uint64_t static_slabs, int* kind, uint64_t* pool_need, uint64_t* verdict, char* err, uint64_t err_cap);
int gft_debug_learn(const char* kernel, uint32_t fifo_cap, int ordered, uint64_t total, uint64_t text_lo, uint64_t text_hi,
                    uint32_t* unit_max, double* scan4_density);

int gft_debug_eval_programs(const uint32_t* prog_words, const uint64_t* prog_off, uint32_t n_exprs, uint32_t n_slots,
                            const uint8_t* present, uint8_t* out_hit, uint32_t* out_depth);
int gft_debug_program_shape(const uint32_t* prog_words, const uint64_t* prog_off, uint32_t n_exprs, uint32_t n_slots, uint32_t* out_shape,
                            uint32_t shape_cap);

int gft_debug_plan_solve(uint32_t n_slots, uint32_t n_exprs, uint32_t fprog_words, int has_rare, uint32_t wide_pairs,
                         uint64_t lds_max, uint32_t n_cus, uint64_t n_docs, int forced_group, int prog_lds, uint32_t dbg,
                         uint64_t* plan);

int gft_debug_plan_solve_pf(uint32_t n_slots, uint32_t n_exprs, uint32_t fprog_words, int has_rare, uint32_t wide_pairs,
                            uint32_t unit_entries, uint64_t lds_max, uint32_t n_cus, uint64_t n_docs, int forced_group, int prog_lds,
                            uint32_t dbg, uint32_t forced_pf, uint64_t* plan);

int gft_debug_host_solve(const uint32_t* words, uint64_t len, const uint32_t* slots, const uint64_t* list_off,
                         const int64_t* positions, uint32_t n_lists, int* out);

#ifdef __cplusplus
}
#endif
#endif
```

Baseline: 306.0 million docs/s.

## Add specialized fast path to scan5 with bail-out to general path

Splits the k_scan5 per-unit body into a compile-time FAST variant that assumes no document edges, ASCII-only text, no deep multi-entry chains, no big short records and no FIFO overflow. The FAST variant drops the boundary checks, the second walk and the direct-write mode, and returns a bail reason when any assumption fails. On a bail the unit is reprocessed with the original general path. Bail counts are recorded in an enlarged control block and exposed through a debug API. The trade-off is larger code and register pressure from instantiating both paths, plus repeated work on units that bail.

Result: no change. 305.1 million docs/s (-0.3%).

```diff
diff --git a/gofindthem_amd/_lib.py b/gofindthem_amd/_lib.py
--- a/gofindthem_amd/_lib.py
+++ b/gofindthem_amd/_lib.py
@@ -238,6 +238,7 @@
     "gft_debug_emulate_scan": (_i, [_vp, _vp, _u32, _vp, _u32, _u32, _u32, _u32, _vp, _vp, _u64, C.POINTER(_u64)]),
     "gft_debug_tables": (_i, [_vp, _vp, _u32, _vp, _u64, _u64, C.c_char_p, C.POINTER(C.c_char_p), _vp, _u64, C.POINTER(_u64), _vp, _u64]),
     "gft_debug_learned_unit": (_i, [_vp, C.POINTER(_u32), C.POINTER(_u32)]),
+    "gft_debug_scan5_bails": (_i, [_vp, C.POINTER(_u32)]),
     "gft_debug_last_unit_route": (_i, [_vp, C.POINTER(C.c_char_p)]),
     "gft_debug_last_fold_bits": (_i, [_vp, C.POINTER(_u32)]),
     "gft_debug_scan_plan": (_i, [_vp, _vp, _u32, _u64, C.c_char_p, C.POINTER(C.c_char_p), _vp]),
diff --git a/gofindthem_amd/csrc/batch_verdict.hpp b/gofindthem_amd/csrc/batch_verdict.hpp
--- a/gofindthem_amd/csrc/batch_verdict.hpp
+++ b/gofindthem_amd/csrc/batch_verdict.hpp
@@ -7,10 +7,11 @@
 
 namespace gft {
 
-constexpr size_t kCtlBytes = 64, kCtlWords = 7;
+constexpr size_t kCtlBytes = 96, kCtlWords = 7;
 constexpr size_t kCtlBad = 0, kCtlCursor = 8, kCtlTotal = 16, kCtlNonascii = 24, kCtlUnits = 32;
 constexpr size_t kCtlBatchClear = 32;
 constexpr size_t kCtlRetryClear = 16;
+constexpr size_t kCtlScan5Bail = 64, kCtlScan5BailBytes = 24;
 constexpr size_t kCtlScanRead = 24;
 
 struct CtlBlock {
diff --git a/gofindthem_amd/csrc/gft_api.cpp b/gofindthem_amd/csrc/gft_api.cpp
--- a/gofindthem_amd/csrc/gft_api.cpp
+++ b/gofindthem_amd/csrc/gft_api.cpp
@@ -16,6 +16,7 @@
     e->opt_scan_prio = num("GFT_SCAN_PRIO", 1) ? 1u : 0u;
     e->opt_scan_ordered = getenv("GFT_SCAN_ORDERED") ? 1u : 0u;
     e->opt_scan4_chunk = (uint32_t)num("GFT_SCAN4_CHUNK", 0);
+    e->opt_scan5_fast = num("GFT_SCAN5_FAST", 1) ? 1u : 0u;
     e->opt_scan4_round = (uint32_t)num("GFT_SCAN4_ROUND", 0);
     e->opt_solve.dbg = (uint32_t)num("GFT_SOLVE_DEBUG", 0);
     e->opt_solve.forced_group = (int)num("GFT_SOLVE_GROUP_DOCS", -1);
diff --git a/gofindthem_amd/csrc/gft_debug.cpp b/gofindthem_amd/csrc/gft_debug.cpp
--- a/gofindthem_amd/csrc/gft_debug.cpp
+++ b/gofindthem_amd/csrc/gft_debug.cpp
@@ -189,6 +189,15 @@
     return GFT_OK;
 }
 
+int gft_debug_scan5_bails(const gft_engine* e, uint32_t* counts) {
+    if (!e || !counts) return GFT_E_INVALID;
+    for (uint32_t r = 0; r < kScan5BailReasons; r++) counts[r] = 0;
+    if (e->plan.kernel != ScanKernel::scan5 || !e->d_ctl.p) return GFT_OK;
+    if (e->stream && hipStreamSynchronize(e->stream) != hipSuccess) return GFT_E_HIP;
+    if (hipMemcpy(counts, e->d_ctl.as<uint8_t>() + kCtlScan5Bail, kScan5BailReasons * 4, hipMemcpyDeviceToHost) != hipSuccess) return GFT_E_HIP;
+    return GFT_OK;
+}
+
 int gft_debug_last_unit_route(const gft_engine* e, const char** name) {
     if (!e || !name) return GFT_E_INVALID;
     *name = e->last_unit_route;
diff --git a/gofindthem_amd/csrc/gft_engine.hpp b/gofindthem_amd/csrc/gft_engine.hpp
--- a/gofindthem_amd/csrc/gft_engine.hpp
+++ b/gofindthem_amd/csrc/gft_engine.hpp
@@ -93,6 +93,7 @@
     uint32_t opt_scan_prio = 1;
     uint32_t opt_scan_ordered = 0;
     uint32_t opt_scan4_round = 0;
+    uint32_t opt_scan5_fast = 1;
     uint32_t opt_scan4_chunk = 0;
     gft::SolveOptions opt_solve;
     mutable std::recursive_mutex mu;
diff --git a/gofindthem_amd/csrc/gft_kernels.hip b/gofindthem_amd/csrc/gft_kernels.hip
--- a/gofindthem_amd/csrc/gft_kernels.hip
+++ b/gofindthem_amd/csrc/gft_kernels.hip
@@ -58,6 +58,7 @@
         uint64_t* ctl64 = reinterpret_cast<uint64_t*>(ctl32);
         unit_base[n_docs] = n_docs;
         ctl32[1] = 0; ctl64[1] = 0; ctl64[2] = 0; ctl32[6] = 0;
+        ctl64[8] = 0; ctl64[9] = 0; ctl64[10] = 0;
         ctl64[4] = n_docs; ctl64[5] = doc_off[0]; ctl64[6] = doc_off[n_docs];
     }
     if (d >= n_docs) return;
diff --git a/gofindthem_amd/csrc/gft_kernels.hpp b/gofindthem_amd/csrc/gft_kernels.hpp
--- a/gofindthem_amd/csrc/gft_kernels.hpp
+++ b/gofindthem_amd/csrc/gft_kernels.hpp
@@ -247,7 +247,9 @@
     uint32_t s5_term_bits, s5_pos_bias;
     const uint32_t* s5_bloom;
     uint32_t s5_bloom_lg;
-};
+    uint32_t s5_fast;
+};
+static_assert(sizeof(Scan2Params) == 384, "the kernarg segment of k_scan2 / k_scan4 / k_scan5 keeps its size");
 GFT_HD inline uint32_t scan5_bloom_g(uint32_t x, uint32_t b1n, uint32_t lg) {
     return (scan2_mul24c<0xC2B2AFu>(x ^ (x >> 20)) + scan2_mul24c<0x27D4EBu>(b1n + 1)) >> (32 - lg);
 }
@@ -265,6 +267,18 @@
 constexpr uint32_t kScan5SurvX = 64;
 constexpr uint32_t kScan5SeenWords = 8;
 constexpr uint32_t kScan5CandCapMin = 384;
+enum : uint32_t {
+    kScan5BailEdge = 1,
+    kScan5BailVerdict = 2,
+    kScan5BailShortBig = 3,
+    kScan5BailDeep = 4,
+    kScan5BailFifo = 5,
+};
+constexpr uint32_t kScan5BailReasons = 5;
+constexpr uint32_t kScan5BailBehindTotal = 48;
+GFT_HD inline uint32_t* scan5_bail_counts(uint64_t* n_matches) {
+    return reinterpret_cast<uint32_t*>(reinterpret_cast<uint8_t*>(n_matches) + kScan5BailBehindTotal);
+}
 struct Scan5Plan { uint32_t G, dual_entries, cand_cap, fifo_cap; };
 bool scan5_plan(uint32_t kp, uint32_t short3_bytes, uint32_t shorts_words, uint32_t fpt_lds_bytes, size_t lds_max, uint32_t fifo_cap, Scan5Plan* out);
 hipError_t launch_scan5(const Scan2Params& P, unsigned n_cus, hipStream_t st);
diff --git a/gofindthem_amd/csrc/gft_pipeline.cpp b/gofindthem_amd/csrc/gft_pipeline.cpp
--- a/gofindthem_amd/csrc/gft_pipeline.cpp
+++ b/gofindthem_amd/csrc/gft_pipeline.cpp
@@ -170,6 +170,9 @@
         P.s5_term_bits = e->plan.s5_term_bits; P.s5_pos_bias = e->plan.s5_pos_bias;
         P.s5_bloom = e->plan.s5_bloom_lg ? d.s5.bloom.as<uint32_t>() : nullptr; P.s5_bloom_lg = e->plan.s5_bloom_lg;
     }
+    P.s5_fast = e->opt_scan5_fast;
+    static_assert(kCtlScan5Bail - kCtlTotal == kScan5BailBehindTotal && kScan5BailReasons * 4 <= kCtlScan5BailBytes &&
+                  kCtlScan5Bail + kCtlScan5BailBytes <= kCtlBytes, "k_scan5 finds its bail counts from the match count");
     return P;
 }
 
@@ -189,6 +192,7 @@
         P2 = scan2_params(e, b); slab = P2.slab;
         L.ordered = P2.ordered != 0;
         if (k == ScanKernel::scan4) work = (b.n_units + P2.chunk_units - 1) / P2.chunk_units;
+        if (k == ScanKernel::scan5 && !L.single) HIP_TRY(hipMemsetAsync(ctl_at<uint8_t>(e, kCtlScan5Bail), 0, kCtlScan5BailBytes, st), "memset");
     }
     L.static_slabs = counts_slabs(k) ? grid_waves(e, work) * slab : 0;
     {
diff --git a/gofindthem_amd/csrc/gft_scan5.hip b/gofindthem_amd/csrc/gft_scan5.hip
--- a/gofindthem_amd/csrc/gft_scan5.hip
+++ b/gofindthem_amd/csrc/gft_scan5.hip
@@ -25,16 +25,17 @@
     bool direct;
     uint64_t dbase;
     uint32_t term_bits, pos_base;
+    uint32_t bail;
 };
 typedef __attribute__((address_space(3))) uint32_t lds_w32;
 __device__ __forceinline__ lds_w32* scan5_seen(const Ctx5& o) { return (lds_w32*)(o.fifo + o.fifo_cap + kScan5SurvX); }
 
-template <bool POS>
+template <bool POS, bool FAST>
 __device__ __forceinline__ void out_append(Ctx5& o, bool em, uint32_t term, uint32_t pos) {
     const uint64_t mask = __ballot(em);
     if (em) {
         const uint32_t idx = o.nf + wave_rank(mask);
-        if (!o.direct) {
+        if (FAST || !o.direct) {
             if (idx < o.fifo_cap - o.npend) o.fifo[idx] = POS ? term | (pos - o.pos_base) << o.term_bits : term;
         } else {
             KARG(pool_term)[o.dbase + idx] = term;
@@ -42,10 +43,10 @@
         }
     }
     o.nf += (uint32_t)__popcll(mask);
-    if (!o.direct && o.nf + o.npend > o.fifo_cap) o.lost = true;
-}
-
-template <bool POS>
+    if ((FAST || !o.direct) && o.nf + o.npend > o.fifo_cap) o.lost = true;
+}
+
+template <bool POS, bool FAST>
 __device__ __forceinline__ void short_trip(const Ctx& c, Ctx5& o, uint32_t ubase, uint32_t n) {
     const uint32_t lane = lane_id();
     const bool on = lane < n;
@@ -66,20 +67,21 @@
     for (uint32_t j = 0; j < 3; j++) {
         if (j && !__any(r[j] != 0)) break;
         const uint32_t L = r[j] >> 28;
-        out_append<POS>(o, r[j] != 0 && L <= p + 1, r[j] & 0x0FFFFFFFu, POS ? (c.P.pos_end ? p : p + 1 - L) : 0u);
-    }
-}
-template <bool POS>
+        out_append<POS, FAST>(o, r[j] != 0 && L <= p + 1, r[j] & 0x0FFFFFFFu, POS ? (c.P.pos_end ? p : p + 1 - L) : 0u);
+    }
+}
+template <bool POS, bool FAST>
 __device__ __forceinline__ void park_short(const Ctx& c, Ctx5& o, uint32_t ubase, uint32_t rel, uint32_t sid, uint32_t x3) {
     if (!__any(sid != 0)) return;
     if (__builtin_expect(__any(sid == 255) && KARG(short3_big) != nullptr, 0)) {
+        if constexpr (FAST) { o.bail = kScan5BailShortBig; return; }
         uint32_t r[3] = {0, 0, 0};
         const uint32_t p = ubase + rel;
         if (sid) short_record(c, sid, x3, r);
 #pragma unroll
         for (uint32_t j = 0; j < 3; j++) {
             const uint32_t L = r[j] >> 28;
-            out_append<POS>(o, r[j] != 0 && L <= p + 1, r[j] & 0x0FFFFFFFu, POS ? (c.P.pos_end ? p : p + 1 - L) : 0u);
+            out_append<POS, FAST>(o, r[j] != 0 && L <= p + 1, r[j] & 0x0FFFFFFFu, POS ? (c.P.pos_end ? p : p + 1 - L) : 0u);
         }
         return;
     }
@@ -87,10 +89,10 @@
     const uint32_t n = (uint32_t)__popcll(m);
     if (o.npend + n > o.fifo_cap / 2) {
         wave_lds_fence();
-        while (o.npend) short_trip<POS>(c, o, ubase, o.npend < 64 ? o.npend : 64);
+        while (o.npend) short_trip<POS, FAST>(c, o, ubase, o.npend < 64 ? o.npend : 64);
         wave_lds_fence();
     }
-    if (!o.direct && o.nf + o.npend + n > o.fifo_cap) o.lost = true;
+    if ((FAST || !o.direct) && o.nf + o.npend + n > o.fifo_cap) o.lost = true;
     if (sid) o.fifo[o.fifo_cap - 1 - o.npend - wave_rank(m)] = rel | sid << 16;
     o.npend += n;
 }
@@ -118,7 +120,7 @@
             if (j < cnt) { w0 = g[1 + 2 * j]; w1 = g[2 + 2 * j]; }
             const uint32_t L = w0 >> 28;
             const bool ok = w0 != 0 && L <= p + 1 && ((W ^ w1) >> ((32 - 8 * L) & 31)) == 0;
-            out_append<POS>(o, ok, w0 & 0x0FFFFFFFu, POS ? (P.pos_end ? p : p + 1 - L) : 0u);
+            out_append<POS, false>(o, ok, w0 & 0x0FFFFFFFu, POS ? (P.pos_end ? p : p + 1 - L) : 0u);
         }
         if (b) sid = 0;
     }
@@ -130,7 +132,7 @@
         if (j && !__any(w0 != 0)) break;
         const uint32_t L = w0 >> 28;
         const bool ok = w0 != 0 && L <= p + 1 && ((W ^ r[2 * j + 1]) >> ((32 - 8 * L) & 31)) == 0;
-        out_append<POS>(o, ok, w0 & 0x0FFFFFFFu, POS ? (P.pos_end ? p : p + 1 - L) : 0u);
+        out_append<POS, false>(o, ok, w0 & 0x0FFFFFFFu, POS ? (P.pos_end ? p : p + 1 - L) : 0u);
     }
 }
 template <bool POS>
@@ -148,7 +150,7 @@
     o.npend += n;
 }
 
-template <bool POS>
+template <bool POS, bool FAST>
 __device__ __forceinline__ void finish_long5(const Ctx& c, Ctx5& o, bool on, uint32_t rel, const Cand& k, const Slot& s0, const Slot& s1,
                                              Front t, uint32_t tl, Deferred& d) {
     const Scan2Params& P = c.P;
@@ -162,7 +164,7 @@
         const uint32_t kmax = wave_kmax(act ? e.a.z & kScan2LenMask : 0);
         if (P.fold) front_fold_upto(t, folded, kmax);
         const bool ok = act && entry_ok(c, k.p, t, tl, e, kmax);
-        out_append<POS>(o, ok, e.a.y, POS ? match_pos(P, k.p, e.a.z) : 0u);
+        out_append<POS, FAST>(o, ok, e.a.y, POS ? match_pos(P, k.p, e.a.z) : 0u);
     }
     if (!__any(multi)) return;
     const uint32_t n_ent = multi ? e.a.z : 0, more_at = e.a.y & ~kScan2Multi;
@@ -176,6 +178,7 @@
         }
         return;
     }
+    if constexpr (FAST) { o.bail = kScan5BailDeep; return; }
     Slot cur = e;
     if (multi) cur = slot_load(&KARG(more)[more_at]);
     for (uint32_t j = 0; __any(j < n_ent); j++) {
@@ -185,13 +188,13 @@
         const uint32_t kmax = wave_kmax(act ? cur.a.z & kScan2LenMask : 0);
         if (P.fold) front_fold_upto(t, folded, kmax);
         const bool ok = act && entry_ok(c, k.p, t, tl, cur, kmax);
-        out_append<POS>(o, ok, cur.a.y, POS ? match_pos(P, k.p, cur.a.z) : 0u);
+        out_append<POS, FAST>(o, ok, cur.a.y, POS ? match_pos(P, k.p, cur.a.z) : 0u);
         cur = nxt;
     }
 }
 
 
-template <bool POS>
+template <bool POS, bool FAST>
 __device__ __forceinline__ void drain_deferred5(const Ctx& c, Ctx5& o, uint32_t ubase, Deferred& d) {
     const Scan2Params& P = c.P;
     const uint32_t lane = lane_id();
@@ -209,7 +212,7 @@
         uint32_t folded = 0;
         if (P.fold) front_fold_upto(t, folded, kmax);
         const bool ok = on && entry_ok(c, p, t, tl, e, kmax);
-        out_append<POS>(o, ok, e.a.y, POS ? match_pos(P, p, e.a.z) : 0u);
+        out_append<POS, FAST>(o, ok, e.a.y, POS ? match_pos(P, p, e.a.z) : 0u);
     }
     d.n = 0;
     __builtin_amdgcn_wave_barrier();
@@ -217,6 +220,7 @@
 
 template <bool FPT_LDS, bool DBG, bool SG, bool POS>
 __global__ void __launch_bounds__(kScan2Threads) k_scan5(const Scan2Params P) {
+    constexpr bool FASTK = !SG && !DBG;
     extern __shared__ __align__(16) uint8_t smem[];
     uint8_t* grp = smem;
     uint8_t* cls = smem + 256;
@@ -265,6 +269,8 @@
     uint32_t wave_matches = 0;
     bool told_nonascii = !(P.fold && P.nonascii);
     uint32_t slab_left = KARG(slab);
+    uint32_t bails[kScan5BailReasons] = {};
+    const bool fast_on = P.s5_fast != 0;
 
     constexpr uint32_t wg_waves = kScan5Waves;
     const uint32_t round_units = gridDim.x * wg_waves, wg_first = blockIdx.x * wg_waves;
@@ -286,8 +292,8 @@
         const uint64_t doc_abs = (uint64_t)(uint32_t)__builtin_amdgcn_readfirstlane((uint32_t)(abs_n >> 32)) << 32 |
                                  (uint32_t)__builtin_amdgcn_readfirstlane((uint32_t)abs_n);
         const uint64_t end_v = end_n;
-        const Ctx c{P, cls, nullptr, P.short3_bytes ? short3 : nullptr, fpt, lrec, text_n + doc_abs, doc_abs, kp2,
-                    doc_abs < 7, doc_abs < 23, un.lo, un.hi, doc_abs + un.hi + 4 > KARG(text_bytes), DBG ? P.dbg : 0u};
+        const uint8_t* const dbase = text_n + doc_abs;
+        const bool near_end = doc_abs + un.hi + 4 > KARG(text_bytes);
         const uint32_t nborder = un.lo < kScan2MaxOff ? un.lo : kScan2MaxOff;
         const uint32_t ubase = un.lo - kScan2MaxOff;
         const uint32_t own = un.hi - un.lo;
@@ -295,16 +301,19 @@
         const uint32_t my_lo = un.lo + lane * C;
         const uint32_t my_hi = my_lo + C < un.hi ? my_lo + C : un.hi;
         const uint32_t nvalid = my_lo < un.hi ? my_hi - my_lo : 0;
-        Ctx5 o{fifo, P.s5_fifo_cap, 0, 0, false, false, 0, POS ? P.s5_term_bits : 0u, POS ? un.lo - P.s5_pos_bias : 0u};
-
-        const uint8_t* src = c.dbase + my_lo;
-        uint32_t hist = 0;
-        U128u nxt{0, 0, 0, 0};
-        if (nvalid) {
-            if (doc_abs + my_lo >= 4) hist = load_u32_unaligned(src - 4);
-            else for (uint32_t i = 1; i <= 3 && i <= doc_abs + my_lo; i++) hist |= (uint32_t)src[-(int)i] << (32 - 8 * i);
-            nxt = *reinterpret_cast<const U128u*>(src);
-        }
+
+        const uint8_t* src = dbase + my_lo;
+        uint32_t hist;
+        U128u nxt;
+        auto first_bytes = [&]() {
+            hist = 0; nxt = U128u{0, 0, 0, 0};
+            if (nvalid) {
+                if (doc_abs + my_lo >= 4) hist = load_u32_unaligned(src - 4);
+                else for (uint32_t i = 1; i <= 3 && i <= doc_abs + my_lo; i++) hist |= (uint32_t)src[-(int)i] << (32 - 8 * i);
+                nxt = *reinterpret_cast<const U128u*>(src);
+            }
+        };
+        first_bytes();
         {
             uint32_t item = 0;
             if (lane == 0) item = __hip_atomic_fetch_add(wg_next, 1u, __ATOMIC_RELAXED, __HIP_MEMORY_SCOPE_WORKGROUP);
@@ -313,6 +322,12 @@
         mark(7);
         request_unit(nu);
 
+        auto unit_body = [&](auto fast_c) __attribute__((always_inline)) -> uint32_t {
+        constexpr bool FAST = decltype(fast_c)::value;
+        const Ctx c{P, cls, nullptr, P.short3_bytes ? short3 : nullptr, fpt, lrec, dbase, doc_abs, kp2,
+                    FAST ? false : doc_abs < 7, FAST ? false : doc_abs < 23, un.lo, un.hi, FAST ? false : near_end, DBG ? P.dbg : 0u};
+        Ctx5 o{fifo, P.s5_fifo_cap, 0, 0, false, false, 0, POS ? P.s5_term_bits : 0u, POS ? un.lo - P.s5_pos_bias : 0u, 0};
+        if constexpr (FASTK && !FAST) first_bytes();
         uint32_t m0 = 0, m1 = 0, m2 = 0, m3 = 0;
         if (own) {
             uint32_t h1 = P.s5_pad_g, h2 = P.s5_pad_g, h3 = P.s5_pad_g, pq = 0;
@@ -381,11 +396,12 @@
                 const uint32_t k = ndw >> 3;
                 if (k == 0) m0 = v; else if (k == 1) m1 = v; else if (k == 2) m2 = v; else m3 = v;
             }
-            if (!SG && !told_nonascii && __any((hib & 0x80808080u) != 0)) {
+            if (FAST && !told_nonascii && __any((hib & 0x80808080u) != 0)) return kScan5BailVerdict;
+            if (!FAST && !SG && !told_nonascii && __any((hib & 0x80808080u) != 0)) {
                 for (uint32_t q = 0; q < npieces; q++)
                     fold_job_push((hib & 0x80808080u) != 0 && q * 16 < nvalid, lane * C + q * 16, cand, P.cand_cap, njobs);
             }
-            if (njobs && !told_nonascii) {
+            if (!FAST && njobs && !told_nonascii) {
                 uint32_t bits = 1u;
                 if (njobs <= P.cand_cap) {
                     FOLD_JOB_VARS(fj_);
@@ -413,7 +429,7 @@
         const uint32_t f = __popc(m0) + __popc(m1) + __popc(m2) + __popc(m3) + (lane == 0 ? nborder : 0);
         const uint32_t fincl = wave_incl_scan(f);
         const uint32_t ftotal = lane_value(fincl, 63);
-        for (uint32_t walk = 0; walk < 2 && ftotal; walk++) {
+        for (uint32_t walk = 0; walk < (FAST ? 1u : 2u) && ftotal; walk++) {
             o.nf = 0; o.npend = 0; o.lost = false;
             if (lane < kScan5SeenWords) scan5_seen(o)[lane] = 0;
             for (uint32_t l0 = 0; l0 < 64;) {
@@ -488,7 +504,7 @@
                         if (i0 + 64 * q < ptotal)
                         {
                             const uint32_t sidq = on[q] && rel[q] >= kScan2MaxOff ? k[q].sid : 0;
-                            if (SG) park_short_g<POS>(c, o, lsg, ubase, rel[q], sidq); else park_short<POS>(c, o, ubase, rel[q], sidq, k[q].x3);
+                            if constexpr (SG) park_short_g<POS>(c, o, lsg, ubase, rel[q], sidq); else park_short<POS, FAST>(c, o, ubase, rel[q], sidq, k[q].x3);
                         }
                     const uint64_t below = (1ull << lane) - 1;
 #pragma unroll
@@ -518,7 +534,7 @@
                     b_k.x = survx[b_on ? lane : 0];
                     b_s0 = slot_load(&P.slots[scan2_pair_slot(b_k.x, 0, P.slot_shift, P.slot_seed)]);
                     b_s1 = slot_load(&P.slots[scan2_pair_slot(b_k.x, 1, P.slot_shift, P.slot_seed)]);
-                    if (!c.near24 && !c.near_end) {
+                    if (FAST || (!c.near24 && !c.near_end)) {
                         const U128u v1 = *reinterpret_cast<const U128u*>(c.dbase + (int64_t)b_k.p - 23);
                         const U128u v2 = *reinterpret_cast<const U128u*>(c.dbase + (int64_t)b_k.p - 7);
                         b_fr.f[4] = v1.x; b_fr.f[3] = v1.y; b_fr.f[2] = v1.z; b_fr.f[1] = v1.w;
@@ -530,7 +546,7 @@
                         b_tl = tail_load(c, b_k.p);
                     }
                 }
-                while (o.npend) { if (SG) short_trip_g<POS>(c, o, lsg, ubase, o.npend < 64 ? o.npend : 64); else short_trip<POS>(c, o, ubase, o.npend < 64 ? o.npend : 64); }
+                while (o.npend) { if constexpr (SG) short_trip_g<POS>(c, o, lsg, ubase, o.npend < 64 ? o.npend : 64); else short_trip<POS, FAST>(c, o, ubase, o.npend < 64 ? o.npend : 64); }
                 if (DBG && (P.dbg & 2)) { if (lane == 0) atomicAdd(reinterpret_cast<unsigned long long*>(KARG(dbg_counters) + 2), (unsigned long long)ns); }
                 mark(3);
                 Deferred dfr;
@@ -540,7 +556,7 @@
                 if (ns) {
                     b_k.tw = b_t8.tw;
                     b_fr.f[0] = b_t8.tw;
-                    finish_long5<POS>(c, o, b_on, b_rel, b_k, b_s0, b_s1, b_fr, b_tl, dfr);
+                    finish_long5<POS, FAST>(c, o, b_on, b_rel, b_k, b_s0, b_s1, b_fr, b_tl, dfr);
                 }
                 for (uint32_t i0 = 64; i0 < ns; i0 += 64) {
                     const bool on = i0 + lane < ns;
@@ -556,7 +572,7 @@
                         const Front fr = front_load(c, p, t8.tw);
                         const uint32_t tl5 = tail_load(c, p);
                         k.tw = t8.tw;
-                        finish_long5<POS>(c, o, on, rel, k, s0, s1, fr, tl5, dfr);
+                        finish_long5<POS, FAST>(c, o, on, rel, k, s0, s1, fr, tl5, dfr);
                     } else {
                         const Text8 t8 = cand_load(c, p);
                         const Front fr = front_load(c, p, t8.tw);
@@ -564,15 +580,16 @@
                         cand_keys<false>(c, p, t8, k);
                         const Slot s0 = slot_load(&P.slots[scan2_pair_slot(k.x, 0, P.slot_shift, P.slot_seed)]);
                         const Slot s1 = slot_load(&P.slots[scan2_pair_slot(k.x, 1, P.slot_shift, P.slot_seed)]);
-                        finish_long5<POS>(c, o, on, rel, k, s0, s1, fr, tl5, dfr);
-                    }
-                }
-                if (dfr.n) drain_deferred5<POS>(c, o, ubase, dfr);
+                        finish_long5<POS, FAST>(c, o, on, rel, k, s0, s1, fr, tl5, dfr);
+                    }
+                }
+                if (dfr.n) drain_deferred5<POS, FAST>(c, o, ubase, dfr);
                 wave_lds_fence();
                 l0 = l1;
                 mark(4);
-            }
-            if (o.direct || !o.lost) break;
+                if (FAST && (o.bail || o.lost)) return o.bail ? o.bail : kScan5BailFifo;
+            }
+            if (FAST || o.direct || !o.lost) break;
             {
                 const uint32_t nh = o.nf;
                 if (nh > slab_left) {
@@ -590,7 +607,7 @@
         text_n = KARG(text);
         if (ftotal) {
             const uint32_t nh = o.nf;
-            if (!o.direct && nh > slab_left) {
+            if ((FAST || !o.direct) && nh > slab_left) {
                 const uint32_t want = nh > KARG(slab) ? nh : KARG(slab);
                 uint64_t nb = 0;
                 if (lane == 0) nb = atomicAdd(reinterpret_cast<unsigned long long*>(KARG(cursor)), (unsigned long long)want);
@@ -603,7 +620,7 @@
             wave_matches += nh;
             const bool room = base + nh <= KARG(pool_cap);
             if (lane == 0) { KARG(unit_start)[u] = base; KARG(unit_count)[u] = room ? nh : 0u; }
-            if (room && !o.direct) {
+            if (room && (FAST || !o.direct)) {
                 const uint32_t tmask = POS ? (1u << o.term_bits) - 1u : 0u;
                 for (uint32_t i = lane; i < nh; i += 64) {
                     const uint32_t e = fifo[i];
@@ -620,6 +637,22 @@
         } else if (lane == 0) {
             KARG(unit_start)[u] = slab_next; KARG(unit_count)[u] = 0;
         }
+        return 0u;
+        };
+        uint32_t why = 1;
+        if constexpr (FASTK) {
+            why = (doc_abs < 23 || near_end) ? kScan5BailEdge : 0u;
+            if (!fast_on) why = kScan5BailReasons + 1;
+            else if (!why) why = unit_body(std::true_type{});
+            if (why && fast_on) bails[why - 1]++;
+        }
+        if (why) unit_body(std::false_type{});
+    }
+    if (FASTK && lane < kScan5BailReasons) {
+        uint32_t nb = 0;
+#pragma unroll
+        for (uint32_t r = 0; r < kScan5BailReasons; r++) nb = lane == r ? bails[r] : nb;
+        if (nb) atomicAdd(scan5_bail_counts(KARG(n_matches)) + lane, nb);
     }
     if (lane == 0) {
         if (wave_matches)
diff --git a/include/gft.h b/include/gft.h
--- a/include/gft.h
+++ b/include/gft.h
@@ -519,6 +519,7 @@
                      uint64_t lds_max, const char* forced_kernel, const char** kernel, uint8_t* out, uint64_t cap, uint64_t* needed,
                      char* err, uint64_t err_cap);
 int gft_debug_learned_unit(const gft_engine* e, uint32_t* unit_max, uint32_t* fifo_cap);
+int gft_debug_scan5_bails(const gft_engine* e, uint32_t counts[5]);
 int gft_debug_last_unit_route(const gft_engine* e, const char** name);
 int gft_debug_last_fold_bits(const gft_engine* e, uint32_t* bits);
 int gft_debug_scan_plan(const uint8_t* terms_blob, const uint64_t* term_off, uint32_t n_terms, uint64_t lds_max, const char* forced_kernel,
```
